# ma-compbio/Phylo-HMRF

Measured on AMD Instinct MI355X. Metric: EM-iterations/sec x nodes (bin-pairs), higher is better.
Workload: dtype f32

## Files before the change

### phylo_hmrf_amd/csrc/api.hip

```cpp

#include <algorithm>
#include <cmath>
#include <cstdio>
#include <cstdlib>
#include <cstring>
#include <limits>
#include <numeric>
#include <random>
#include <thread>

#include "common.h"

namespace phmrf {

static thread_local std::string g_error;

void set_error(const std::string& msg) { g_error = msg; }

int fail(int status, const std::string& msg) {
  g_error = msg;
  return status;
}

static hipEvent_t take_event(phmrf_block* b) {
// ... 454 lines not shown
  auto guard = [&](int s) {
    if (s != PHMRF_OK && st == PHMRF_OK) st = s;
  };
  if (hipGetDevice(&b->device) != hipSuccess) guard(fail(PHMRF_ERR_HIP, "hipGetDevice failed"));
  if (st == PHMRF_OK && hipStreamCreateWithFlags(&b->own_stream, hipStreamNonBlocking) != hipSuccess)
    guard(fail(PHMRF_ERR_HIP, "hipStreamCreate failed"));
  b->stream = b->own_stream;
  if (st == PHMRF_OK) guard(dev_alloc(&b->X, (size_t)n * S));
  if (st == PHMRF_OK) guard(dev_alloc(&b->logprob, (size_t)n * K));
  if (st == PHMRF_OK) guard(dev_alloc(&b->labels, (size_t)n));
  if (st == PHMRF_OK) guard(dev_alloc(&b->labels_tmp, (size_t)n));
  if (st == PHMRF_OK) guard(dev_alloc(&b->accum, (size_t)ACCUM_DOUBLES));
  if (st == PHMRF_OK) guard(dev_alloc(&b->counters, (size_t)N_COUNTERS));
  if (st == PHMRF_OK) guard(dev_alloc(&b->work_acc, (size_t)WORK_BANKS * WORK_SLOTS));
  if (st == PHMRF_OK && hipMemsetAsync(b->work_acc, 0, WORK_BANKS * WORK_SLOTS * sizeof(unsigned long long), b->own_stream) != hipSuccess)
    guard(fail(PHMRF_ERR_HIP, "hipMemset failed"));
  if (st == PHMRF_OK && hipHostMalloc(reinterpret_cast<void**>(&b->work_host), WORK_BANKS * WORK_SLOTS * sizeof(unsigned long long)) != hipSuccess)
    guard(fail(PHMRF_ERR_HIP, "hipHostMalloc failed"));
  if (st == PHMRF_OK) guard(dev_alloc(&b->emis_params, (size_t)K * (S + S * (S + 1) / 2 + 1)));
  if (st == PHMRF_OK && hipHostMalloc(reinterpret_cast<void**>(&b->accum_host), ACCUM_DOUBLES * sizeof(double)) != hipSuccess)
    guard(fail(PHMRF_ERR_HIP, "hipHostMalloc failed"));
  if (st == PHMRF_OK && hipHostMalloc(reinterpret_cast<void**>(&b->counters_host), N_COUNTERS * sizeof(unsigned long long)) != hipSuccess)
    guard(fail(PHMRF_ERR_HIP, "hipHostMalloc failed"));
  if (st == PHMRF_OK && (hipEventCreate(&b->ev0) != hipSuccess || hipEventCreate(&b->ev1) != hipSuccess))
    guard(fail(PHMRF_ERR_HIP, "hipEventCreate failed"));
  if (st == PHMRF_OK && hipMemsetAsync(b->labels, 0, (size_t)n, b->stream) != hipSuccess)
    guard(fail(PHMRF_ERR_HIP, "hipMemset failed"));
  if (st != PHMRF_OK) {
    std::string keep = g_error;
    phmrf_block_destroy(b);
    g_error = keep;
    return st;
  }
  *out = b;
  return PHMRF_OK;
}

int phmrf_block_destroy(phmrf_block_t b) {
  if (!b) return PHMRF_OK;
  if (b->stream) (void)hipStreamSynchronize(b->stream);
  coarse_children_destroy(b);
  if (b->c2f) {
    (void)phmrf_block_destroy(b->c2f);
    b->c2f = nullptr;
  }
  dev_free(b->X);
  dev_free(b->logprob);
  dev_free(b->labels);
  dev_free(b->labels_tmp);
  dev_free(b->labels_eval);
  dev_free(b->coarse_flag);
  dev_free(b->coarse_lab);
  if (b->coarse_lab_host) (void)hipHostFree(b->coarse_lab_host);
  b->coarse_lab_host = nullptr;
  dev_free(b->sgain);
  dev_free(b->mf_rev);
  dev_free(b->mf_theta);
  dev_free(b->mf_cap);
  dev_free(b->mf_tcap);
  dev_free(b->mf_exc);
  dev_free(b->mf_hgt);
  dev_free(b->mf_flags);
  if (b->mf_flags_host) (void)hipHostFree(b->mf_flags_host);
  b->mf_flags_host = nullptr;
  for (int s = 0; s < 4; ++s) dev_free(b->saved[s]);
  dev_free(b->nbr);
  dev_free(b->wgt);
  dev_free(b->colour_nodes);
  for (auto& f : b->families) free_family(f);
  dev_free(b->comp);
  dev_free(b->comp_tab);
  dev_free(b->comp_tab64);
  dev_free(b->post_partial);
  dev_free(b->comp_best);
  dev_free(b->comp_gain);
  dev_free(b->cc_seen);
  dev_free(b->cc_stale);
  dev_free(b->stamp);
  dev_free(b->memo);
  dev_free(b->chain_memo);
  dev_free(b->fwd_w);
  if (b->uT_raw) {
    dev_free(b->uT_raw);
    b->uT = nullptr;
  }
  dev_free(b->emis_params);
  dev_free(b->posteriors);
  dev_free(b->summary);
  dev_free(b->anc);
  for (int r = 0; r < 2; ++r) {
    dev_free(b->pin_save[r]);
    dev_free(b->pin_label[r]);
  }
  dev_free(b->xfer);
  if (b->xfer_host) (void)hipHostFree(b->xfer_host);
  if (b->ss) {
    delete b->ss;
    b->ss = nullptr;
  }
  dev_free(b->accum);
  dev_free(b->counters);
  dev_free(b->work_acc);
  if (b->work_host) (void)hipHostFree(b->work_host);
  if (b->accum_host) (void)hipHostFree(b->accum_host);
  if (b->counters_host) (void)hipHostFree(b->counters_host);
  for (auto& p : b->pending) {
    (void)hipEventDestroy(p.a);
    (void)hipEventDestroy(p.b);
  }
  for (auto e : b->free_events) (void)hipEventDestroy(e);
  if (b->cur_start) (void)hipEventDestroy(b->cur_start);
  if (b->ev0) (void)hipEventDestroy(b->ev0);
  if (b->ev1) (void)hipEventDestroy(b->ev1);
  if (b->own_stream) (void)hipStreamDestroy(b->own_stream);
  delete b;
  return PHMRF_OK;
}

int phmrf_block_set_stream(phmrf_block_t b, void* hip_stream) {
  PHMRF_CHECK(b, PHMRF_ERR_INVALID, "block is NULL");
  PHMRF_HIP(hipStreamSynchronize(b->stream));
  b->stream = hip_stream ? reinterpret_cast<hipStream_t>(hip_stream) : b->own_stream;
  for (int lv = 0; lv < N_COARSE_CHILDREN; ++lv)
    if (b->coarse[lv]) b->coarse[lv]->stream = b->stream;
  return PHMRF_OK;
}

int phmrf_block_sync(phmrf_block_t b) {
  PHMRF_CHECK(b, PHMRF_ERR_INVALID, "block is NULL");
  PHMRF_HIP(hipStreamSynchronize(b->stream));
  return PHMRF_OK;
}

int phmrf_block_set_observations(phmrf_block_t b, const double* X) {
  PHMRF_CHECK(b && X, PHMRF_ERR_INVALID, "NULL argument");
  const size_t cnt = (size_t)b->n * b->S;
  std::vector<float> tmp(cnt);
  for (size_t i = 0; i < cnt; ++i) tmp[i] = (float)X[i];
  PHMRF_TRY(upload(b->X, tmp.data(), cnt * sizeof(float), b->stream));
  b->has_X = true;
  return PHMRF_OK;
}

int phmrf_block_set_observations_dev(phmrf_block_t b, const float* X_dev) {
  PHMRF_CHECK(b && X_dev, PHMRF_ERR_INVALID, "NULL argument");
  PHMRF_HIP(hipMemcpyAsync(b->X, X_dev, (size_t)b->n * b->S * sizeof(float), hipMemcpyDeviceToDevice, b->stream));
  b->has_X = true;
  return PHMRF_OK;
}

int phmrf_block_set_graph(phmrf_block_t b, int64_t E, const int64_t* edges, const double* w) {
  PHMRF_CHECK(b, PHMRF_ERR_INVALID, "block is NULL");
  PHMRF_CHECK(E >= 0 && (E == 0 || (edges && w)), PHMRF_ERR_INVALID, "edges / w is NULL");
  const int64_t n = b->n;
  std::vector<int32_t> deg(n, 0);
  for (int64_t e = 0; e < E; ++e) {
    const int64_t a = edges[2 * e], c = edges[2 * e + 1];
    PHMRF_CHECK(a >= 0 && a < n && c >= 0 && c < n, PHMRF_ERR_INVALID, "edge endpoint out of range");
    PHMRF_CHECK(a != c, PHMRF_ERR_INVALID, "self loop in edge list");
    PHMRF_CHECK(w[e] >= 0.0 && std::isfinite(w[e]), PHMRF_ERR_INVALID, "edge weights must be finite and >= 0");
    ++deg[a];
    ++deg[c];
  }
  int maxdeg = 0;
  for (int64_t i = 0; i < n; ++i) maxdeg = std::max(maxdeg, deg[i]);
  PHMRF_CHECK(maxdeg <= 64, PHMRF_ERR_UNSUPPORTED, "node degree > 64 is not supported");
  const int D = std::max(4, (maxdeg + 3) / 4 * 4);
  std::vector<int32_t> nbr((size_t)n * D, -1);
  std::vector<float> wgt((size_t)n * D, 0.f);
  std::fill(deg.begin(), deg.end(), 0);
  for (int64_t e = 0; e < E; ++e) {
    const int64_t a = edges[2 * e], c = edges[2 * e + 1];
    nbr[(size_t)a * D + deg[a]] = (int32_t)c;
    wgt[(size_t)a * D + deg[a]++] = (float)w[e];
    nbr[(size_t)c * D + deg[c]] = (int32_t)a;
    wgt[(size_t)c * D + deg[c]++] = (float)w[e];
  }
  for (int64_t i = 0; i < n; ++i) {
    int32_t* c = &nbr[(size_t)i * D];
    float* ww = &wgt[(size_t)i * D];
    for (int x = 1; x < deg[i]; ++x) {
      const int32_t cv = c[x];
      const float wv = ww[x];
      int y = x - 1;
      while (y >= 0 && c[y] > cv) {
        c[y + 1] = c[y];
        ww[y + 1] = ww[y];
        --y;
      }
      c[y + 1] = cv;
      ww[y + 1] = wv;
    }
    for (int x = 1; x < deg[i]; ++x)
      PHMRF_CHECK(c[x] != c[x - 1], PHMRF_ERR_INVALID, "duplicate edge in edge list");
  }
  std::vector<int32_t> colour(n, -1);
  int ncol = 0;
  {
    std::vector<int> mark(66, -1);
    for (int64_t i = 0; i < n; ++i) {
      const int32_t* c = &nbr[(size_t)i * D];
      for (int x = 0; x < deg[i]; ++x)
        if (colour[c[x]] >= 0) mark[colour[c[x]]] = (int)(i & 0x7fffffff);
      int col = 0;
      while (mark[col] == (int)(i & 0x7fffffff)) ++col;
      colour[i] = col;
      ncol = std::max(ncol, col + 1);
    }
  }
  std::vector<int64_t> cptr(ncol + 1, 0);
  for (int64_t i = 0; i < n; ++i) ++cptr[colour[i] + 1];
  for (int c = 0; c < ncol; ++c) cptr[c + 1] += cptr[c];
  std::vector<int32_t> cnodes(n);
  {
    std::vector<int64_t> pos(cptr.begin(), cptr.end() - 1);
    for (int64_t i = 0; i < n; ++i) cnodes[pos[colour[i]]++] = (int32_t)i;
  }
  dev_free(b->nbr);
  dev_free(b->wgt);
  dev_free(b->colour_nodes);
  PHMRF_TRY(dev_alloc(&b->nbr, (size_t)n * D));
  PHMRF_TRY(dev_alloc(&b->wgt, (size_t)n * D));
  PHMRF_TRY(dev_alloc(&b->colour_nodes, (size_t)n));
  PHMRF_TRY(upload(b->nbr, nbr.data(), nbr.size() * sizeof(int32_t), b->stream));
  PHMRF_TRY(upload(b->wgt, wgt.data(), wgt.size() * sizeof(float), b->stream));
  PHMRF_TRY(upload(b->colour_nodes, cnodes.data(), cnodes.size() * sizeof(int32_t), b->stream));
  b->D = D;
  b->E = E;
  b->n_colours = ncol;
  b->colour_ptr = cptr;
  b->has_graph = true;
  b->has_grid = false;
  for (auto& f : b->families) free_family(f);
  b->families.clear();
  dev_free(b->mf_rev);
  dev_free(b->mf_theta);
  dev_free(b->mf_cap);
  dev_free(b->mf_tcap);
  dev_free(b->mf_exc);
  dev_free(b->mf_hgt);
  return PHMRF_OK;
}

int phmrf_block_set_grid(phmrf_block_t b, int H, int W, int diagonal, int num_neighbor) {
  PHMRF_CHECK(b, PHMRF_ERR_INVALID, "block is NULL");
  PHMRF_CHECK(b->has_graph, PHMRF_ERR_STATE, "set_graph must precede set_grid");
  PHMRF_CHECK(H >= 1 && W >= 1, PHMRF_ERR_INVALID, "H, W must be >= 1");
  PHMRF_CHECK(num_neighbor == 8 || num_neighbor == 4, PHMRF_ERR_INVALID, "num_neighbor must be 8 or 4");
  PHMRF_CHECK(!diagonal || H <= W, PHMRF_ERR_INVALID, "a diagonal block is the first H <= W rows of a W x W upper triangle");
  Geometry g(H, W, diagonal);
  PHMRF_CHECK(g.count() == b->n, PHMRF_ERR_INVALID, "H, W, diagonal do not match the node count");
  const int64_t n = b->n;
  const int D = b->D;
  std::vector<int32_t> nbr((size_t)n * D);
  std::vector<float> wgt((size_t)n * D);
  PHMRF_TRY(download(nbr.data(), b->nbr, nbr.size() * sizeof(int32_t), b->stream));
  PHMRF_TRY(download(wgt.data(), b->wgt, wgt.size() * sizeof(float), b->stream));
  std::vector<int32_t> ci(n), cj(n);
  for (int64_t v = 0; v < n; ++v) {
    int i, j;
    g.coords(v, &i, &j);
    ci[v] = i;
    cj[v] = j;
  }
  int64_t present = 0, expected = 0;
  for (int64_t v = 0; v < n; ++v) {
    for (int x = 0; x < D; ++x) {
      const int32_t u = nbr[(size_t)v * D + x];
      if (u < 0) continue;
      const int di = std::abs(ci[u] - ci[v]), dj = std::abs(cj[u] - cj[v]);
      PHMRF_CHECK(di <= 1 && dj <= 1 && (di + dj) > 0, PHMRF_ERR_INVALID, "edge list joins nodes that are not grid neighbours");
      PHMRF_CHECK(num_neighbor == 8 || (di + dj) == 1, PHMRF_ERR_INVALID, "diagonal edge in a 4-neighbour block");
      ++present;
    }
    for (int di = -1; di <= 1; ++di)
      for (int dj = -1; dj <= 1; ++dj) {
        if ((di == 0 && dj == 0) || (num_neighbor == 4 && di != 0 && dj != 0)) continue;
        const int ni = ci[v] + di, nj = cj[v] + dj;
        if (ni < 0 || ni >= H || nj < 0 || nj >= W || (diagonal && ni > nj)) continue;
        ++expected;
      }
  }
  PHMRF_TRY(setup_grid_tables(b, g, num_neighbor));
  b->grid_complete = present == expected;
  return PHMRF_OK;
}

int phmrf_block_build_grid_graph(phmrf_block_t b, int H, int W, int diagonal, int num_neighbor, double beta1) {
  PHMRF_CHECK(b, PHMRF_ERR_INVALID, "block is NULL");
  PHMRF_CHECK(b->has_X, PHMRF_ERR_STATE, "observations must be set before the graph is built from them");
  PHMRF_CHECK(H >= 1 && W >= 1, PHMRF_ERR_INVALID, "H, W must be >= 1");
  PHMRF_CHECK(num_neighbor == 8 || num_neighbor == 4, PHMRF_ERR_INVALID, "num_neighbor must be 8 or 4");
  PHMRF_CHECK(!diagonal || H <= W, PHMRF_ERR_INVALID, "a diagonal block is the first H <= W rows of a W x W upper triangle");
  PHMRF_CHECK(beta1 >= 0.0 && std::isfinite(beta1), PHMRF_ERR_INVALID, "beta1 must be finite and >= 0");
  Geometry g(H, W, diagonal);
  PHMRF_CHECK(g.count() == b->n, PHMRF_ERR_INVALID, "H, W, diagonal do not match the node count");
  dev_free(b->nbr);
  dev_free(b->wgt);
  PHMRF_TRY(dev_alloc(&b->nbr, (size_t)b->n * 8));
  PHMRF_TRY(dev_alloc(&b->wgt, (size_t)b->n * 8));
  b->D = 8;
  PHMRF_TRY(launch_grid_graph(b, H, W, diagonal, num_neighbor, beta1));
  if (!b->colour_nodes) PHMRF_TRY(dev_alloc(&b->colour_nodes, (size_t)b->n));
  b->has_graph = true;
  b->E = 0;
  PHMRF_TRY(setup_grid_tables(b, g, num_neighbor));
  b->grid_complete = true;
  return PHMRF_OK;
}

int phmrf_block_get_adjacency(phmrf_block_t b, int* D, int32_t* nbr_out, float* wgt_out) {
  PHMRF_CHECK(b && D, PHMRF_ERR_INVALID, "NULL argument");
  PHMRF_CHECK(b->has_graph, PHMRF_ERR_STATE, "graph not set");
  *D = b->D;
  if (nbr_out) PHMRF_TRY(download(nbr_out, b->nbr, (size_t)b->n * b->D * sizeof(int32_t), b->stream));
  if (wgt_out) PHMRF_TRY(download(wgt_out, b->wgt, (size_t)b->n * b->D * sizeof(float), b->stream));
  return PHMRF_OK;
}

int phmrf_block_set_labels(phmrf_block_t b, const int32_t* labels) {
  PHMRF_CHECK(b && labels, PHMRF_ERR_INVALID, "NULL argument");
  std::vector<uint8_t> tmp(b->n);
  for (int64_t i = 0; i < b->n; ++i) {
    PHMRF_CHECK(labels[i] >= 0 && labels[i] < b->K, PHMRF_ERR_INVALID, "label out of range [0,K)");
    tmp[i] = (uint8_t)labels[i];
  }
  PHMRF_TRY(upload(b->labels, tmp.data(), (size_t)b->n, b->stream));
  b->has_labels = true;
  b->labels_are_slot = 0;
  return PHMRF_OK;
}

static int fetch_labels(phmrf_block_t b, const uint8_t* src, int32_t* labels) {
  std::vector<uint8_t> tmp(b->n);
  PHMRF_TRY(download(tmp.data(), src, (size_t)b->n, b->stream));
  for (int64_t i = 0; i < b->n; ++i) labels[i] = tmp[i];
  return PHMRF_OK;
}

int phmrf_block_get_labels(phmrf_block_t b, int32_t* labels) {
  PHMRF_CHECK(b && labels, PHMRF_ERR_INVALID, "NULL argument");
  return fetch_labels(b, b->labels, labels);
}

int phmrf_block_save_labels(phmrf_block_t b, int slot) {
  PHMRF_CHECK(b, PHMRF_ERR_INVALID, "block is NULL");
  PHMRF_CHECK(slot >= 0 && slot < 4, PHMRF_ERR_INVALID, "slot must be in [0,4)");
  if (!b->saved[slot]) PHMRF_TRY(dev_alloc(&b->saved[slot], (size_t)b->n));
  PHMRF_HIP(hipMemcpyAsync(b->saved[slot], b->labels, (size_t)b->n, hipMemcpyDeviceToDevice, b->stream));
  b->labels_are_slot |= 1 << slot;
  return PHMRF_OK;
}

int phmrf_block_restore_labels(phmrf_block_t b, int slot) {
  PHMRF_CHECK(b, PHMRF_ERR_INVALID, "block is NULL");
  PHMRF_CHECK(slot >= 0 && slot < 4 && b->saved[slot], PHMRF_ERR_STATE, "label slot is empty");
  PHMRF_HIP(hipMemcpyAsync(b->labels, b->saved[slot], (size_t)b->n, hipMemcpyDeviceToDevice, b->stream));
  b->has_labels = true;
  b->labels_are_slot = 1 << slot;
  return PHMRF_OK;
}

int phmrf_block_get_saved_labels(phmrf_block_t b, int slot, int32_t* labels) {
  PHMRF_CHECK(b && labels, PHMRF_ERR_INVALID, "NULL argument");
  PHMRF_CHECK(slot >= 0 && slot < 4 && b->saved[slot], PHMRF_ERR_STATE, "label slot is empty");
  return fetch_labels(b, b->saved[slot], labels);
}

int phmrf_emission_pack_size(int S, int K, int64_t* n_floats) {
  PHMRF_CHECK(n_floats && S >= 1 && S <= 16 && K >= 1, PHMRF_ERR_INVALID, "bad S/K");
  *n_floats = (int64_t)K * (S + S * (S + 1) / 2 + 1);
  return PHMRF_OK;
}

int phmrf_emission_pack(int S, int K, const double* means, const double* covars, float* packed) {
  PHMRF_CHECK(means && covars && packed, PHMRF_ERR_INVALID, "NULL argument");
  PHMRF_CHECK(S >= 1 && S <= 16 && K >= 1, PHMRF_ERR_INVALID, "bad S/K");
  const int PS = S + S * (S + 1) / 2 + 1;
  std::vector<double> L(S * S), Li(S * S);
  for (int k = 0; k < K; ++k) {
    const double* cv = covars + (size_t)k * S * S;
    bool ok = false;
    for (int attempt = 0; attempt < 2 && !ok; ++attempt) {
      const double jitter = attempt ? 1e-7 : 0.0;
      ok = true;
      std::fill(L.begin(), L.end(), 0.0);
      for (int i = 0; i < S && ok; ++i)
        for (int j = 0; j <= i; ++j) {
          double s = cv[i * S + j] + (i == j ? jitter : 0.0);
          for (int t = 0; t < j; ++t) s -= L[i * S + t] * L[j * S + t];
          if (i == j) {
            if (!(s > 0.0) || !std::isfinite(s)) { ok = false; break; }
            L[i * S + i] = std::sqrt(s);
          } else {
            L[i * S + j] = s / L[j * S + j];
          }
        }
    }
    if (!ok) return fail(PHMRF_ERR_NOT_PD, "'covars' must be symmetric, positive-definite (state " + std::to_string(k) + ")");
    std::fill(Li.begin(), Li.end(), 0.0);
    double logdet = 0.0;
    for (int i = 0; i < S; ++i) logdet += 2.0 * std::log(L[i * S + i]);
    for (int c = 0; c < S; ++c)
      for (int i = c; i < S; ++i) {
        double s = (i == c) ? 1.0 : 0.0;
        for (int t = c; t < i; ++t) s -= L[i * S + t] * Li[t * S + c];
        Li[i * S + c] = s / L[i * S + i];
      }
    float* p = packed + (size_t)k * PS;
    for (int s = 0; s < S; ++s) p[s] = (float)means[(size_t)k * S + s];
    int idx = S;
    for (int i = 0; i < S; ++i)
      for (int c = 0; c <= i; ++c) p[idx++] = (float)Li[i * S + c];
    p[idx] = (float)(-0.5 * (S * std::log(2.0 * M_PI) + logdet));
  }
  return PHMRF_OK;
}

int phmrf_emission_dev(const float* X_dev, int64_t n, int S, int K, const float* packed_dev, float* logprob_dev,
                       void* hip_stream) {
  PHMRF_CHECK(X_dev && packed_dev && logprob_dev, PHMRF_ERR_INVALID, "NULL argument");
  PHMRF_CHECK(n > 0 && K >= 1 && K <= 64, PHMRF_ERR_INVALID, "bad n/K");
  return launch_emission(X_dev, n, S, K, packed_dev, logprob_dev, nullptr, reinterpret_cast<hipStream_t>(hip_stream));
}

int phmrf_emission(phmrf_block_t b, const double* means, const double* covars) {
  PHMRF_CHECK(b && means && covars, PHMRF_ERR_INVALID, "NULL argument");
  PHMRF_CHECK(b->has_X, PHMRF_ERR_STATE, "observations not set");
  const int PS = b->S + b->S * (b->S + 1) / 2 + 1;
  std::vector<float> packed((size_t)b->K * PS);
  PHMRF_TRY(phmrf_emission_pack(b->S, b->K, means, covars, packed.data()));
  PHMRF_TRY(upload(b->emis_params, packed.data(), packed.size() * sizeof(float), b->stream));
  tic(b, KC_EMISSION);
  PHMRF_TRY(launch_emission(b->X, b->n, b->S, b->K, b->emis_params, b->logprob, b->uT, b->stream));
  toc(b, KC_EMISSION, 1);
  b->has_logprob = true;
  b->uT_valid = b->uT != nullptr;
  b->pin_saved = false;
  b->pin_rows[0] = b->pin_rows[1] = 0;
  return PHMRF_OK;
}

int phmrf_block_get_logprob(phmrf_block_t b, double* logprob) {
  PHMRF_CHECK(b && logprob, PHMRF_ERR_INVALID, "NULL argument");
  PHMRF_CHECK(b->has_logprob, PHMRF_ERR_STATE, "logprob not computed");
  const size_t cnt = (size_t)b->n * b->K;
  std::vector<float> tmp(cnt);
  PHMRF_TRY(download(tmp.data(), b->logprob, cnt * sizeof(float), b->stream));
  for (size_t i = 0; i < cnt; ++i) logprob[i] = tmp[i];
  return PHMRF_OK;
}

int phmrf_block_set_logprob(phmrf_block_t b, const double* logprob) {
  PHMRF_CHECK(b && logprob, PHMRF_ERR_INVALID, "NULL argument");
  const size_t cnt = (size_t)b->n * b->K;
  std::vector<float> tmp(cnt);
  for (size_t i = 0; i < cnt; ++i) tmp[i] = (float)logprob[i];
  PHMRF_TRY(upload(b->logprob, tmp.data(), cnt * sizeof(float), b->stream));
  b->has_logprob = true;
  b->uT_valid = false;
  b->pin_saved = false;
  b->pin_rows[0] = b->pin_rows[1] = 0;
  return PHMRF_OK;
}

static int read_counter(phmrf_block_t b, int64_t* v) {
  PHMRF_HIP(hipMemcpyAsync(b->counters_host + COUNTER_DEFAULT, b->counters + COUNTER_DEFAULT, sizeof(unsigned long long), hipMemcpyDeviceToHost, b->stream));
  PHMRF_HIP(hipStreamSynchronize(b->stream));
  if (v) *v = (int64_t)b->counters_host[COUNTER_DEFAULT];
  return PHMRF_OK;
}

static int zero_counter(phmrf_block_t b) {
  PHMRF_HIP(hipMemsetAsync(b->counters, 0, N_COUNTERS * sizeof(unsigned long long), b->stream));
  b->counter_slot = COUNTER_DEFAULT;
  return PHMRF_OK;
}

int phmrf_mrf_energy(phmrf_block_t b, double beta, double* e_total, double* e_unary, double* e_pair) {
  PHMRF_TRY(check_solvable(b));
  double eu, ep;
  PHMRF_TRY(energy_now(b, beta, &eu, &ep));
  if (e_total) *e_total = eu + ep;
  if (e_unary) *e_unary = eu;
  if (e_pair) *e_pair = ep;
  return PHMRF_OK;
}

int phmrf_block_warm_start(phmrf_block_t b, double beta, int slot, int choose, double* e_current, double* e_saved, int* took_saved) {
  PHMRF_TRY(check_solvable(b));
  PHMRF_CHECK(slot >= 0 && slot < 4 && b->saved[slot], PHMRF_ERR_STATE, "label slot is empty");
  if (took_saved) *took_saved = 1;
  const bool report = e_current || e_saved || took_saved;
  if (!b->has_labels || ((b->labels_are_slot >> slot) & 1)) {
    if (choose && !b->has_labels) PHMRF_TRY(phmrf_block_restore_labels(b, slot));
    if (e_current) *e_current = std::numeric_limits<double>::infinity();
    if (e_saved) *e_saved = 0.0;
    return PHMRF_OK;
  }
  double* const extra = b->accum + (ACCUM_DOUBLES - 4);
  if (choose && !report && b->n >= (1 << 16) && energy_diff_available(b)) {
    PHMRF_TRY(zero_accum(b, 4, 2));
    PHMRF_TRY(zero_accum(b, ACCUM_DOUBLES - 4, 2));
    tic(b, KC_ENERGY);
    PHMRF_TRY(launch_energy_diff(b, b->saved[slot]));
    PHMRF_TRY(launch_choose_labels(b, b->saved[slot], b->accum + 4, extra, beta));
    toc(b, KC_ENERGY, 2);
    b->labels_are_slot = 0;
    return PHMRF_OK;
  }
  PHMRF_TRY(zero_accum(b, 4, 2));
  PHMRF_TRY(zero_accum(b, ACCUM_DOUBLES - 4, 2));
  tic(b, KC_ENERGY);
  PHMRF_TRY(launch_energy(b, (float)beta));
  std::swap(b->labels, b->saved[slot]);
  const int st = launch_energy(b, (float)beta, extra);
  std::swap(b->labels, b->saved[slot]);
  PHMRF_TRY(st);
  if (choose) PHMRF_TRY(launch_choose_labels(b, b->saved[slot], b->accum + 4, extra, beta));
  toc(b, KC_ENERGY, choose ? 3 : 2);
  if (choose) b->labels_are_slot = 0;
  if (!report) return PHMRF_OK;
  PHMRF_HIP(hipMemcpyAsync(b->accum_host + 4, b->accum + 4, 2 * sizeof(double), hipMemcpyDeviceToHost, b->stream));
  PHMRF_HIP(hipMemcpyAsync(b->accum_host + 6, extra, 2 * sizeof(double), hipMemcpyDeviceToHost, b->stream));
  PHMRF_HIP(hipStreamSynchronize(b->stream));
  double ec[2], es[2];
  energy_sums(b, b->accum_host + 4, &ec[0], &ec[1]);
  energy_sums(b, b->accum_host + 6, &es[0], &es[1]);
  const double cur = ec[0] + beta * ec[1], sav = es[0] + beta * es[1];
  if (e_current) *e_current = cur;
  if (e_saved) *e_saved = sav;
  if (took_saved) *took_saved = !(cur < sav) ? 1 : 0;
  return PHMRF_OK;
}

int phmrf_block_energy_diff(phmrf_block_t b, double beta, int slot, double* out) {
  PHMRF_TRY(check_solvable(b));
  PHMRF_CHECK(out, PHMRF_ERR_INVALID, "NULL argument");
  PHMRF_CHECK(slot >= 0 && slot < 4 && b->saved[slot], PHMRF_ERR_STATE, "label slot is empty");
  PHMRF_CHECK(b->has_labels, PHMRF_ERR_STATE, "labels not set");
  PHMRF_CHECK(b->has_grid && b->fwd_w && b->H > 0 && b->W > 0, PHMRF_ERR_UNSUPPORTED,
              "the energy difference from the differing nodes needs a grid block (phmrf_block_set_grid / build_grid_graph)");
  PHMRF_CHECK(energy_diff_available(b), PHMRF_ERR_STATE,
              "the unary planes are not current (a strip pass or a solve builds them after phmrf_block_set_logprob)");
  PHMRF_TRY(zero_accum(b, 4, 2));
  tic(b, KC_ENERGY);
  PHMRF_TRY(launch_energy_diff(b, b->saved[slot]));
  toc(b, KC_ENERGY, 1);
  PHMRF_HIP(hipMemcpyAsync(b->accum_host + 4, b->accum + 4, 2 * sizeof(double), hipMemcpyDeviceToHost, b->stream));
  PHMRF_HIP(hipStreamSynchronize(b->stream));
  energy_sums(b, b->accum_host + 4, &out[0], &out[1]);
  out[1] = beta * out[1];
  return PHMRF_OK;
}

int phmrf_mrf_icm_sweep(phmrf_block_t b, double beta, int64_t* changed) {
  PHMRF_TRY(check_solvable(b));
  b->labels_are_slot = 0;
  PHMRF_TRY(zero_counter(b));
  PHMRF_TRY(icm_sweep_nocount(b, (float)beta));
  return read_counter(b, changed);
}

static int ensure_chain_families(phmrf_block* b) {
  if (!b->has_grid && b->families.empty() && b->nbr && b->n >= 2) PHMRF_TRY(setup_path_families(b));
  return PHMRF_OK;
}

int phmrf_mrf_chain_sweep(phmrf_block_t b, double beta, int family, int64_t* changed) {
  PHMRF_TRY(check_solvable(b));
  b->labels_are_slot = 0;
  PHMRF_TRY(ensure_chain_families(b));
  PHMRF_CHECK(family >= 0 && family < (int)b->families.size(), PHMRF_ERR_INVALID, "no such chain family");
  PHMRF_TRY(zero_counter(b));
  PHMRF_TRY(chain_sweep_nocount(b, (float)beta, family, 0));
  PHMRF_TRY(chain_sweep_nocount(b, (float)beta, family, 1));
  return read_counter(b, changed);
}

int phmrf_block_chain_family_info(phmrf_block_t b, int* n_families, int* n_colours) {
  PHMRF_CHECK(b && n_families, PHMRF_ERR_INVALID, "NULL argument");
  PHMRF_CHECK(b->has_graph, PHMRF_ERR_STATE, "graph not set");
  PHMRF_CHECK(!b->ss, PHMRF_ERR_STATE, "a solve is in progress");
  PHMRF_TRY(ensure_chain_families(b));
  *n_families = (int)b->families.size();
  if (n_colours)
    for (int f = 0; f < MAX_CHAIN_FAMILIES; ++f) n_colours[f] = f < (int)b->families.size() ? b->families[f].n_colours : 0;
  return PHMRF_OK;
}

int phmrf_block_get_chain_segments(phmrf_block_t b, int family, int phase, int colour, int64_t* n_segments, int64_t* n_nodes,
                                   int32_t* seg_start, int32_t* seg_len, int32_t* nodes) {
  PHMRF_CHECK(b && n_segments && n_nodes, PHMRF_ERR_INVALID, "NULL argument");
  PHMRF_CHECK(b->has_graph, PHMRF_ERR_STATE, "graph not set");
  PHMRF_CHECK(!b->ss, PHMRF_ERR_STATE, "a solve is in progress");
  PHMRF_TRY(ensure_chain_families(b));
  PHMRF_CHECK(family >= 0 && family < (int)b->families.size(), PHMRF_ERR_INVALID, "no such chain family");
  const ChainFamily& f = b->families[family];
  PHMRF_CHECK(phase == 0 || phase == 1, PHMRF_ERR_INVALID, "phase must be 0 or 1");
  PHMRF_CHECK(colour >= 0 && colour < f.n_colours, PHMRF_ERR_INVALID, "no such colour in this chain family");
  const int nseg = f.nseg[phase][colour];
  *n_segments = nseg;
  *n_nodes = f.n_nodes;
  if (seg_start && nseg > 0) PHMRF_TRY(download(seg_start, f.seg_start[phase][colour], (size_t)nseg * sizeof(int32_t), b->stream));
  if (seg_len && nseg > 0) PHMRF_TRY(download(seg_len, f.seg_len[phase][colour], (size_t)nseg * sizeof(int32_t), b->stream));
  if (nodes && f.n_nodes > 0) PHMRF_TRY(download(nodes, f.nodes, (size_t)f.n_nodes * sizeof(int32_t), b->stream));
  return PHMRF_OK;
}

int phmrf_block_prepare_components(phmrf_block_t b) {
  PHMRF_CHECK(b, PHMRF_ERR_INVALID, "block is NULL");
  PHMRF_CHECK(!b->ss, PHMRF_ERR_STATE, "a solve is in progress");
  if (!b->has_labels || !b->has_graph) return PHMRF_OK;
  return launch_component_prepare(b);
}

int phmrf_mrf_component_pass(phmrf_block_t b, double beta, int64_t* changed) {
  PHMRF_TRY(check_solvable(b));
  b->labels_are_slot = 0;
  PHMRF_TRY(zero_counter(b));
  tic(b, KC_COMPONENT);
  PHMRF_TRY(launch_component_pass(b, (float)beta));
  toc(b, KC_COMPONENT, 1);
  return read_counter(b, changed);
}

int phmrf_mrf_graph_expansion(phmrf_block_t b, double beta, int alpha, int64_t* changed) {
  PHMRF_TRY(check_solvable(b));
  PHMRF_CHECK(b->has_labels, PHMRF_ERR_STATE, "labels not set");
  PHMRF_CHECK(alpha >= 0 && alpha < b->K, PHMRF_ERR_INVALID, "alpha must be in [0, K)");
  PHMRF_CHECK(b->n >= 2, PHMRF_ERR_INVALID, "the graph has fewer than two nodes");
  b->labels_are_slot = 0;
  PHMRF_TRY(zero_counter(b));
  PHMRF_TRY(launch_graph_expansion(b, (float)beta, alpha));
  return read_counter(b, changed);
}


int phmrf_mrf_strip_pass(phmrf_block_t b, double beta, int orient, int shift_r, int shift_c, int alpha, int64_t* changed) {
  PHMRF_TRY(check_solvable(b));
  b->labels_are_slot = 0;
  PHMRF_CHECK(b->has_grid, PHMRF_ERR_STATE, "strip moves need phmrf_block_set_grid");
  PHMRF_CHECK(b->num_neighbor == 8 || b->num_neighbor == 4, PHMRF_ERR_STATE, "bad grid");
  PHMRF_CHECK(orient == 0 || orient == 1, PHMRF_ERR_INVALID, "orient must be 0 or 1");
  PHMRF_CHECK(shift_r >= 0 && shift_r <= 5 && shift_c >= 0 && shift_c <= 63, PHMRF_ERR_INVALID, "shift out of range");
  PHMRF_CHECK(alpha < b->K, PHMRF_ERR_INVALID, "alpha must be < K");
  PHMRF_TRY(zero_counter(b));
  PHMRF_TRY(strip_pass_nocount(b, (float)beta, orient, shift_r, shift_c, alpha));
  PHMRF_TRY(work_fetch_async(b));
  PHMRF_TRY(read_counter(b, changed));
  work_fold(b);
  return PHMRF_OK;
}

int phmrf_mrf_strip_multi_pass(phmrf_block_t b, double beta, int orient, int shift_r, int shift_c, uint64_t label_mask,
                               int64_t* changed) {
  PHMRF_TRY(check_solvable(b));
  b->labels_are_slot = 0;
  PHMRF_CHECK(b->has_grid, PHMRF_ERR_STATE, "strip moves need phmrf_block_set_grid");
  PHMRF_CHECK(b->num_neighbor == 8 || b->num_neighbor == 4, PHMRF_ERR_STATE, "bad grid");
  PHMRF_CHECK(orient == 0 || orient == 1, PHMRF_ERR_INVALID, "orient must be 0 or 1");
  PHMRF_CHECK(shift_r >= 0 && shift_r <= 5 && shift_c >= 0 && shift_c <= 63, PHMRF_ERR_INVALID, "shift out of range");
  PHMRF_CHECK(b->K >= 64 || (label_mask >> b->K) == 0, PHMRF_ERR_INVALID, "label_mask names a label >= K");
  PHMRF_HIP(hipMemsetAsync(b->counters, 0, N_COUNTERS * sizeof(unsigned long long), b->stream));
  if (!b->uT_valid) PHMRF_TRY(launch_unary_planes(b));
  tic(b, KC_STRIP);
  PHMRF_TRY(launch_strip_multi(b, (float)beta, orient, shift_r, shift_c, label_mask, -1));
  b->work[4] += 1;
  toc(b, KC_STRIP, 1);
  PHMRF_TRY(work_fetch_async(b));
  PHMRF_HIP(hipMemcpyAsync(b->counters_host, b->counters, N_COUNTERS * sizeof(unsigned long long), hipMemcpyDeviceToHost, b->stream));
  PHMRF_HIP(hipStreamSynchronize(b->stream));
  work_fold(b);
  int64_t ch = 0;
  for (int a = 0; a < b->K; ++a) ch += (int64_t)b->counters_host[COUNTER_EXPANSION + a];
  if (changed) *changed = ch;
  return PHMRF_OK;
}

int phmrf_mrf_coarse_pass(phmrf_block_t b, double beta, int scale, int offset, int alpha, int shift_r, int shift_c,
                          int64_t* changed) {
  PHMRF_TRY(check_solvable(b));
  b->labels_are_slot = 0;
  PHMRF_CHECK(b->has_grid, PHMRF_ERR_STATE, "coarse moves need phmrf_block_set_grid");
  PHMRF_CHECK(scale == 2 || scale == 4 || scale == 8, PHMRF_ERR_INVALID, "scale must be 2, 4 or 8");
  PHMRF_CHECK(offset >= 0 && offset < scale, PHMRF_ERR_INVALID, "offset must be in [0, scale)");
  PHMRF_CHECK(alpha >= 0 && alpha < b->K, PHMRF_ERR_INVALID, "alpha must be in [0, K)");
  PHMRF_CHECK(shift_r >= 0 && shift_r <= 5 && shift_c >= 0 && shift_c <= 63, PHMRF_ERR_INVALID, "shift out of range");
  PHMRF_TRY(zero_counter(b));
  PHMRF_TRY(coarse_sweep_nocount(b, (float)beta, scale == 2 ? 0 : (scale == 4 ? 1 : 2), offset, shift_r, shift_c, alpha, alpha + 1));
  return read_counter(b, changed);
}

int phmrf_block_coarse_problem(phmrf_block_t b, double beta, int scale, int offset, int alpha, int64_t* nc, float* D_out,
                               float* lam_out) {
  PHMRF_TRY(check_solvable(b));
  PHMRF_CHECK(nc, PHMRF_ERR_INVALID, "nc is NULL");
  PHMRF_CHECK(b->has_grid, PHMRF_ERR_STATE, "coarse moves need phmrf_block_set_grid");
  PHMRF_CHECK(scale == 2 || scale == 4 || scale == 8, PHMRF_ERR_INVALID, "scale must be 2, 4 or 8");
  PHMRF_CHECK(offset >= 0 && offset < scale, PHMRF_ERR_INVALID, "offset must be in [0, scale)");
  PHMRF_CHECK(alpha >= 0 && alpha < b->K, PHMRF_ERR_INVALID, "alpha must be in [0, K)");
  *nc = coarse_nodes(b, scale, offset);
  if (!D_out && !lam_out) return PHMRF_OK;
  phmrf_block* c = nullptr;
  PHMRF_TRY(coarse_child(b, 4 * (scale == 2 ? 0 : (scale == 4 ? 1 : 2)), &c));
  if (!b->uT_valid) PHMRF_TRY(launch_unary_planes(b));
  PHMRF_TRY(launch_coarsen(b, c, scale, offset, alpha, (float)beta));
  if (D_out) PHMRF_TRY(download(D_out, c->uT + *nc, (size_t)*nc * sizeof(float), b->stream));
  if (lam_out) PHMRF_TRY(download(lam_out, c->fwd_w, (size_t)*nc * sizeof(float4), b->stream));
  return PHMRF_OK;
}

int phmrf_block_coarse_problems(phmrf_block_t b, double beta, int scale, int offset, const int* alphas, int nl, int64_t* nc,
                                float* D_out, float* lam_out) {
  PHMRF_TRY(check_solvable(b));
  PHMRF_CHECK(nc && alphas, PHMRF_ERR_INVALID, "NULL argument");
  PHMRF_CHECK(b->has_grid, PHMRF_ERR_STATE, "coarse moves need phmrf_block_set_grid");
  PHMRF_CHECK(scale == 2 || scale == 4 || scale == 8, PHMRF_ERR_INVALID, "scale must be 2, 4 or 8");
  PHMRF_CHECK(offset >= 0 && offset < scale, PHMRF_ERR_INVALID, "offset must be in [0, scale)");
  PHMRF_CHECK(nl >= 1 && nl <= 4, PHMRF_ERR_INVALID, "nl must be in [1, 4]");
  for (int q = 0; q < nl; ++q) PHMRF_CHECK(alphas[q] >= 0 && alphas[q] < b->K, PHMRF_ERR_INVALID, "alpha must be in [0, K)");
  *nc = coarse_nodes(b, scale, offset);
  if (!D_out && !lam_out) return PHMRF_OK;
  const int level = scale == 2 ? 0 : (scale == 4 ? 1 : 2);
  phmrf_block* ch[4] = {nullptr, nullptr, nullptr, nullptr};
  for (int q = 0; q < nl; ++q) PHMRF_TRY(coarse_child(b, 4 * level + q, &ch[q]));
  if (!b->uT_valid) PHMRF_TRY(launch_unary_planes(b));
  PHMRF_TRY(launch_coarsen_batch(b, ch, alphas, nl, scale, offset, (float)beta, nullptr, -1, false));
  for (int q = 0; q < nl; ++q) {
    if (D_out) PHMRF_TRY(download(D_out + (size_t)q * *nc, ch[q]->uT + *nc, (size_t)*nc * sizeof(float), b->stream));
    if (lam_out) PHMRF_TRY(download(lam_out + (size_t)q * *nc * 4, ch[q]->fwd_w, (size_t)*nc * sizeof(float4), b->stream));
  }
  return PHMRF_OK;
}

int phmrf_mrf_coarse_sweep(phmrf_block_t b, double beta, int scale, int offset, uint64_t label_mask, int shift_r, int shift_c,
                           int stamps, int64_t* changed, int64_t* changed_label) {
  PHMRF_TRY(check_solvable(b));
  PHMRF_CHECK(!b->ss, PHMRF_ERR_STATE, "a solve is in progress");
  PHMRF_CHECK(b->has_grid, PHMRF_ERR_STATE, "coarse moves need phmrf_block_set_grid");
  PHMRF_CHECK(b->has_labels, PHMRF_ERR_STATE, "labels not set");
  PHMRF_CHECK(scale == 2 || scale == 4 || scale == 8, PHMRF_ERR_INVALID, "scale must be 2, 4 or 8");
  PHMRF_CHECK(offset >= 0 && offset < scale, PHMRF_ERR_INVALID, "offset must be in [0, scale)");
  PHMRF_CHECK(shift_r >= 0 && shift_r <= 5 && shift_c >= 0 && shift_c <= 63, PHMRF_ERR_INVALID, "shift out of range");
  PHMRF_CHECK(b->K >= 64 || (label_mask >> b->K) == 0, PHMRF_ERR_INVALID, "label_mask names a label >= K");
  b->labels_are_slot = 0;
  const int level = scale == 2 ? 0 : (scale == 4 ? 1 : 2);
  const size_t lab_bytes = (size_t)N_COARSE * MAX_LABELS * sizeof(unsigned long long);
  if (!b->coarse_lab) {
    PHMRF_TRY(dev_alloc(&b->coarse_lab, (size_t)N_COARSE * MAX_LABELS));
    PHMRF_HIP(hipHostMalloc(reinterpret_cast<void**>(&b->coarse_lab_host), lab_bytes));
  }
  PHMRF_HIP(hipMemsetAsync(b->coarse_lab, 0, lab_bytes, b->stream));
  PHMRF_TRY(zero_counter(b));
  if (stamps) {
    if (!b->stamp) PHMRF_TRY(dev_alloc(&b->stamp, (size_t)b->n));
    PHMRF_HIP(hipMemsetAsync(b->stamp, 0, (size_t)b->n * sizeof(uint16_t), b->stream));
    b->tick = 1;
  }
  int st = coarse_sweep_nocount(b, (float)beta, level, offset, shift_r, shift_c, 0, b->K, label_mask);
  if (st == PHMRF_OK && hipMemcpyAsync(b->coarse_lab_host, b->coarse_lab, lab_bytes, hipMemcpyDeviceToHost, b->stream) != hipSuccess)
    st = PHMRF_ERR_HIP;
  const int st_read = read_counter(b, changed);
  if (stamps) solve_scope_exit(b);
  PHMRF_TRY(st);
  PHMRF_TRY(st_read);
  if (changed_label)
    for (int a = 0; a < b->K; ++a) changed_label[a] = (int64_t)b->coarse_lab_host[(size_t)level * MAX_LABELS + a];
  return PHMRF_OK;
}

static int c2f_ready(phmrf_block_t b) {
  PHMRF_CHECK(b, PHMRF_ERR_INVALID, "block is NULL");
  PHMRF_CHECK(!b->ss, PHMRF_ERR_STATE, "a solve is in progress");
  PHMRF_CHECK(c2f_applies(b), PHMRF_ERR_STATE,
              "the coarse-to-fine start needs a complete 8-neighbour grid block (no row tile) with n >= 1024 and H, W >= 8");
  return c2f_child(b);
}

int phmrf_block_c2f_problem(phmrf_block_t b, int* Hc, int* Wc, int64_t* nc, int32_t* nbr_out, float* wgt_out, float* logprob_out) {
  PHMRF_TRY(check_solvable(b));
  PHMRF_CHECK(Hc && Wc && nc, PHMRF_ERR_INVALID, "NULL argument");
  PHMRF_TRY(c2f_ready(b));
  phmrf_block* c = b->c2f;
  *Hc = b->c2f_Hc;
  *Wc = b->c2f_Wc;
  *nc = c->n;
  if (nbr_out) PHMRF_TRY(download(nbr_out, c->nbr, (size_t)c->n * 8 * sizeof(int32_t), b->stream));
  if (wgt_out) PHMRF_TRY(download(wgt_out, c->wgt, (size_t)c->n * 8 * sizeof(float), b->stream));
  if (logprob_out) {
    PHMRF_TRY(launch_c2f_logprob(b, c, b->c2f_Wc, C2F_SCALE));
    c->has_logprob = true;
    c->uT_valid = false;
    PHMRF_TRY(download(logprob_out, c->logprob, (size_t)c->n * b->K * sizeof(float), b->stream));
  }
  return PHMRF_OK;
}

int phmrf_block_c2f_prolong(phmrf_block_t b, const int32_t* labels_c, int64_t nc) {
  PHMRF_CHECK(b && labels_c, PHMRF_ERR_INVALID, "NULL argument");
  PHMRF_TRY(c2f_ready(b));
  phmrf_block* c = b->c2f;
  PHMRF_CHECK(nc == c->n, PHMRF_ERR_INVALID, "nc is not the number of 4 x 4 super-cells");
  std::vector<uint8_t> tmp((size_t)nc);
  for (int64_t i = 0; i < nc; ++i) {
    PHMRF_CHECK(labels_c[i] >= 0 && labels_c[i] < b->K, PHMRF_ERR_INVALID, "label out of range [0,K)");
    tmp[(size_t)i] = (uint8_t)labels_c[i];
  }
  PHMRF_TRY(upload(c->labels, tmp.data(), (size_t)nc, b->stream));
  c->has_labels = true;
  c->labels_are_slot = 0;
  PHMRF_TRY(launch_c2f_prolong(b, c, b->c2f_Wc, C2F_SCALE));
  PHMRF_HIP(hipStreamSynchronize(b->stream));
  b->has_labels = true;
  b->labels_are_slot = 0;
  return PHMRF_OK;
}


int phmrf_block_set_tile(phmrf_block_t b, int top, int bottom, int64_t sched_n) {
  PHMRF_CHECK(b, PHMRF_ERR_INVALID, "block is NULL");
  PHMRF_CHECK(b->has_grid, PHMRF_ERR_STATE, "row tiles need the grid geometry (phmrf_block_set_grid / build_grid_graph)");
  PHMRF_CHECK(!b->ss, PHMRF_ERR_STATE, "a solve is in progress");
  top = top ? 1 : 0;
  bottom = bottom ? 1 : 0;
  PHMRF_CHECK(b->H >= 2 * (top + bottom) + 2, PHMRF_ERR_INVALID, "a tile needs two rows per cut and two more");
  for (int r = 0; r < 2; ++r) {
    dev_free(b->pin_save[r]);
    dev_free(b->pin_label[r]);
    b->pin_first[r] = b->pin_count[r] = b->pin_split[r] = 0;
    b->pin_rows[r] = 0;
  }
  b->pin_saved = false;
  b->tile_top = top;
  b->tile_bot = bottom;
  b->sched_n = sched_n > 0 ? sched_n : 0;
  if (!top && !bottom) {
    b->own0 = 0;
    b->own1 = -1;
    b->own_r0 = 0;
    b->own_r1 = -1;
    return PHMRF_OK;
  }
  b->own_r0 = top ? 1 : 0;
  b->own_r1 = b->H - (bottom ? 1 : 0);
  b->own0 = row_first(b, b->own_r0);
  b->own1 = row_first(b, b->own_r1);
  if (top) {
    b->pin_first[0] = 0;
    b->pin_count[0] = row_first(b, 2);
    b->pin_split[0] = row_first(b, 1);
  }
  if (bottom) {
    b->pin_first[1] = row_first(b, b->H - 2);
    b->pin_count[1] = b->n - b->pin_first[1];
    b->pin_split[1] = row_first(b, b->H - 1) - b->pin_first[1];
  }
  int64_t cap = 0;
  for (int r = 0; r < 2; ++r)
    if (b->pin_count[r] > 0) {
      PHMRF_TRY(dev_alloc(&b->pin_save[r], (size_t)b->pin_count[r] * b->K));
      PHMRF_TRY(dev_alloc(&b->pin_label[r], (size_t)b->pin_count[r]));
      cap += b->pin_count[r];
    }
  if (cap > b->xfer_cap) {
    dev_free(b->xfer);
    if (b->xfer_host) (void)hipHostFree(b->xfer_host);
    b->xfer_host = nullptr;
    PHMRF_TRY(dev_alloc(&b->xfer, (size_t)cap));
    PHMRF_HIP(hipHostMalloc(reinterpret_cast<void**>(&b->xfer_host), (size_t)2 * cap));
    b->xfer_cap = cap;
  }
  return PHMRF_OK;
}

static void pin_range(const phmrf_block* b, int region, int rows, int64_t* first, int64_t* count) {
  *first = b->pin_first[region];
  *count = 0;
  if (rows <= 0 || b->pin_count[region] == 0) return;
  if (rows >= 2) {
    *count = b->pin_count[region];
  } else if (region == 0) {
    *count = b->pin_split[0];
  } else {
    *first = b->pin_first[1] + b->pin_split[1];
    *count = b->pin_count[1] - b->pin_split[1];
  }
}

int phmrf_block_tile_pins(phmrf_block_t b, int n_top, int n_bottom) {
  PHMRF_CHECK(b, PHMRF_ERR_INVALID, "block is NULL");
  PHMRF_CHECK(is_tile(b), PHMRF_ERR_STATE, "the block is not a tile (phmrf_block_set_tile)");
  PHMRF_CHECK(b->has_logprob, PHMRF_ERR_STATE, "logprob not set");
  PHMRF_CHECK(n_top >= 0 && n_top <= 2 && n_bottom >= 0 && n_bottom <= 2, PHMRF_ERR_INVALID, "0, 1 or 2 rows per cut");
  const int want[2] = {b->tile_top ? n_top : 0, b->tile_bot ? n_bottom : 0};
  if (b->tick) ++b->tick;
  for (int r = 0; r < 2; ++r) {
    if (b->pin_count[r] == 0) continue;
    int64_t pf, pc, wf, wc;
    pin_range(b, r, want[r], &pf, &pc);
    pin_range(b, r, b->pin_saved ? b->pin_rows[r] : 0, &wf, &wc);
    PHMRF_TRY(launch_tile_pins(b, r, b->pin_first[r], b->pin_count[r], pf, pc, wf, wc, !b->pin_saved));
    b->pin_rows[r] = want[r];
  }
  b->pin_saved = true;
  return PHMRF_OK;
}

int phmrf_block_tile_get_boundary(phmrf_block_t b, uint8_t* top_out, uint8_t* bottom_out) {
  PHMRF_CHECK(b, PHMRF_ERR_INVALID, "block is NULL");
  PHMRF_CHECK(is_tile(b), PHMRF_ERR_STATE, "the block is not a tile (phmrf_block_set_tile)");
  const bool have = b->boundary_queued && b->ss && b->ss->collected;
  if (!have) {
    PHMRF_TRY(tile_queue_boundary(b));
    PHMRF_HIP(hipStreamSynchronize(b->stream));
  }
  b->boundary_queued = false;
  int64_t off = 0;
  if (b->tile_top) {
    const int64_t tc = row_first(b, 2) - row_first(b, 1);
    if (top_out) std::memcpy(top_out, b->xfer_host, (size_t)tc);
    off = tc;
  }
  if (b->tile_bot && bottom_out) {
    const int64_t bc = row_first(b, b->H - 1) - row_first(b, b->H - 2);
    std::memcpy(bottom_out, b->xfer_host + off, (size_t)bc);
  }
  return PHMRF_OK;
}

int phmrf_block_tile_put_halo(phmrf_block_t b, const uint8_t* top_in, const uint8_t* bottom_in) {
  PHMRF_CHECK(b, PHMRF_ERR_INVALID, "block is NULL");
  PHMRF_CHECK(is_tile(b), PHMRF_ERR_STATE, "the block is not a tile (phmrf_block_set_tile)");
  if (b->tick) ++b->tick;
  b->labels_are_slot = 0;
  uint8_t* const in_host = b->xfer_host + b->xfer_cap;
  int64_t off = 0;
  if (top_in && b->tile_top) {
    const int64_t c = row_first(b, 1);
    for (int64_t q = 0; q < c; ++q) PHMRF_CHECK(top_in[q] < b->K, PHMRF_ERR_INVALID, "label out of range [0,K)");
    std::memcpy(in_host, top_in, (size_t)c);
    PHMRF_HIP(hipMemcpyAsync(b->xfer, in_host, (size_t)c, hipMemcpyHostToDevice, b->stream));
    PHMRF_TRY(launch_put_labels(b, 0, c, b->xfer));
    off = c;
  }
  if (bottom_in && b->tile_bot) {
    const int64_t f = row_first(b, b->H - 1), c = b->n - f;
    for (int64_t q = 0; q < c; ++q) PHMRF_CHECK(bottom_in[q] < b->K, PHMRF_ERR_INVALID, "label out of range [0,K)");
    std::memcpy(in_host + off, bottom_in, (size_t)c);
    PHMRF_HIP(hipMemcpyAsync(b->xfer + off, in_host + off, (size_t)c, hipMemcpyHostToDevice, b->stream));
    PHMRF_TRY(launch_put_labels(b, f, c, b->xfer + off));
  }
  if (!b->ss) PHMRF_HIP(hipStreamSynchronize(b->stream));
  return PHMRF_OK;
}

static int posterior_launch(phmrf_block_t b, double beta, int estimate_type, bool write_post) {
  PHMRF_TRY(check_solvable(b));
  PHMRF_CHECK(b->has_X, PHMRF_ERR_STATE, "observations not set");
  const int ns = n_stats(b);
  PHMRF_CHECK(8 + ns <= ACCUM_DOUBLES, PHMRF_ERR_UNSUPPORTED, "K*(1+S+S*S) too large");
  if (write_post && !b->posteriors) PHMRF_TRY(dev_alloc(&b->posteriors, (size_t)b->n * b->K));
  if (b->deterministic && !b->post_partial) {
    const int64_t rows = std::min<int64_t>(POST_PARTIAL_ROWS, std::max<int64_t>(1, (b->n + POST_DET_TB - 1) / POST_DET_TB));
    PHMRF_TRY(dev_alloc(&b->post_partial, (size_t)rows * (b->K * (1 + b->S + b->S * (b->S + 1) / 2) + 4)));
  }
  PHMRF_TRY(zero_accum(b, 0, 4));
  PHMRF_TRY(zero_accum(b, 8, ns));
  tic(b, KC_POSTERIOR);
  PHMRF_TRY(launch_posterior_stats(b, (float)beta, estimate_type, write_post));
  toc(b, KC_POSTERIOR, 1);
  return PHMRF_OK;
}

int phmrf_posterior_stats(phmrf_block_t b, double beta, int estimate_type, double* stats_out, double* costs_out,
                          double* posteriors_out) {
  PHMRF_CHECK(b && stats_out && costs_out, PHMRF_ERR_INVALID, "NULL argument");
  PHMRF_TRY(posterior_launch(b, beta, estimate_type, posteriors_out != nullptr));
  const int ns = n_stats(b);
  PHMRF_HIP(hipMemcpyAsync(b->accum_host, b->accum, (8 + ns) * sizeof(double), hipMemcpyDeviceToHost, b->stream));
  PHMRF_HIP(hipStreamSynchronize(b->stream));
  std::memcpy(costs_out, b->accum_host, 4 * sizeof(double));
  std::memcpy(stats_out, b->accum_host + 8, ns * sizeof(double));
  if (posteriors_out) {
    const size_t cnt = (size_t)b->n * b->K;
    std::vector<float> tmp(cnt);
    PHMRF_TRY(download(tmp.data(), b->posteriors, cnt * sizeof(float), b->stream));
    for (size_t i = 0; i < cnt; ++i) posteriors_out[i] = tmp[i];
  }
  return PHMRF_OK;
}

int phmrf_posterior_stats_dev(phmrf_block_t b, double beta, int estimate_type, double* out_dev) {
  PHMRF_CHECK(b && out_dev, PHMRF_ERR_INVALID, "NULL argument");
  PHMRF_TRY(posterior_launch(b, beta, estimate_type, false));
  const int ns = n_stats(b);
  PHMRF_HIP(hipMemcpyAsync(out_dev, b->accum + 8, ns * sizeof(double), hipMemcpyDeviceToDevice, b->stream));
  PHMRF_HIP(hipMemcpyAsync(out_dev + ns, b->accum, 4 * sizeof(double), hipMemcpyDeviceToDevice, b->stream));
  return PHMRF_OK;
}

int phmrf_posterior_summary(phmrf_block_t b, double beta, int estimate_type, float* conf, uint8_t* top, float* entropy_or_null) {
  PHMRF_CHECK(b && conf && top, PHMRF_ERR_INVALID, "NULL argument");
  PHMRF_TRY(check_solvable(b));
  PHMRF_CHECK(b->has_labels, PHMRF_ERR_STATE, "labels not set (phmrf_block_set_labels or a solve)");
  const int64_t n_first = b->own1 >= 0 ? b->own0 : 0, n_last = b->own1 >= 0 ? b->own1 : b->n;
  const int64_t m = n_last - n_first;
  if (m <= 0) return PHMRF_OK;
  if (!b->summary) PHMRF_TRY(dev_alloc(&b->summary, (size_t)b->n * (2 * sizeof(float) + 1)));
  float* d_conf = reinterpret_cast<float*>(b->summary);
  float* d_ent = d_conf + b->n;
  uint8_t* d_top = reinterpret_cast<uint8_t*>(d_ent + b->n);
  tic(b, KC_POSTERIOR);
  PHMRF_TRY(launch_posterior_summary(b, (float)beta, estimate_type, d_conf, d_top, entropy_or_null ? d_ent : nullptr));
  toc(b, KC_POSTERIOR, 1);
  PHMRF_HIP(hipMemcpyAsync(conf, d_conf, (size_t)m * sizeof(float), hipMemcpyDeviceToHost, b->stream));
  PHMRF_HIP(hipMemcpyAsync(top, d_top, (size_t)m, hipMemcpyDeviceToHost, b->stream));
  if (entropy_or_null)
    PHMRF_HIP(hipMemcpyAsync(entropy_or_null, d_ent, (size_t)m * sizeof(float), hipMemcpyDeviceToHost, b->stream));
  PHMRF_HIP(hipStreamSynchronize(b->stream));
  return PHMRF_OK;
}

int phmrf_ancestral(phmrf_block_t b, double beta, int estimate_type, int weighting, int A, const double* affine,
                    const double* cond_var, float* mean_out, float* sd_out_or_null) {
  PHMRF_CHECK(b && affine && cond_var && mean_out, PHMRF_ERR_INVALID, "NULL argument");
  PHMRF_CHECK(weighting == 0 || weighting == 1, PHMRF_ERR_INVALID, "weighting must be 0 (posterior) or 1 (called)");
  PHMRF_CHECK(A >= 1 && A <= 16, PHMRF_ERR_UNSUPPORTED, "ancestral: A must be in [1,16]");
  PHMRF_CHECK(b->S <= 8, PHMRF_ERR_UNSUPPORTED, "ancestral: S must be in [1,8]");
  const int K = b->K, S = b->S, TS = S + 2;
  std::vector<float> tab((size_t)K * A * TS);
  for (int ka = 0; ka < K * A; ++ka) {
    for (int s = 0; s <= S; ++s) tab[(size_t)ka * TS + s] = (float)affine[(size_t)ka * (S + 1) + s];
    tab[(size_t)ka * TS + S + 1] = (float)cond_var[ka];
    PHMRF_CHECK(cond_var[ka] >= 0.0, PHMRF_ERR_INVALID, "cond_var must be finite and >= 0");
  }
  for (float v : tab) PHMRF_CHECK(std::isfinite(v), PHMRF_ERR_INVALID, "the tables must be finite (as float32)");
  PHMRF_CHECK(b->has_X, PHMRF_ERR_STATE, "observations not set");
  PHMRF_CHECK(b->has_labels, PHMRF_ERR_STATE, "labels not set (phmrf_block_set_labels or a solve)");
  if (weighting == 0) PHMRF_TRY(check_solvable(b));
  const int64_t n_first = b->own1 >= 0 ? b->own0 : 0, n_last = b->own1 >= 0 ? b->own1 : b->n;
  const int64_t m = n_last - n_first;
  if (m <= 0) return PHMRF_OK;
  const size_t need = tab.size() + (size_t)2 * A * m;
  if (b->anc_floats < need) {
    dev_free(b->anc);
    b->anc_floats = 0;
    PHMRF_TRY(dev_alloc(&b->anc, need));
    b->anc_floats = need;
  }
  float* d_mean = b->anc + tab.size();
  float* d_sd = d_mean + (size_t)A * m;
  PHMRF_TRY(upload(b->anc, tab.data(), tab.size() * sizeof(float), b->stream));
  tic(b, KC_POSTERIOR);
  PHMRF_TRY(launch_ancestral(b, (float)beta, estimate_type, weighting, A, b->anc, d_mean, sd_out_or_null ? d_sd : nullptr));
  toc(b, KC_POSTERIOR, 1);
  PHMRF_HIP(hipMemcpyAsync(mean_out, d_mean, (size_t)A * m * sizeof(float), hipMemcpyDeviceToHost, b->stream));
  if (sd_out_or_null)
    PHMRF_HIP(hipMemcpyAsync(sd_out_or_null, d_sd, (size_t)A * m * sizeof(float), hipMemcpyDeviceToHost, b->stream));
  PHMRF_HIP(hipStreamSynchronize(b->stream));
  return PHMRF_OK;
}

int phmrf_kmeans_step(phmrf_block_t b, const double* centers, int write_labels, double* out) {
  PHMRF_CHECK(b && centers && out, PHMRF_ERR_INVALID, "NULL argument");
  PHMRF_CHECK(b->has_X, PHMRF_ERR_STATE, "observations not set");
  const int K = b->K, S = b->S, NP = K * S + K + 1;
  PHMRF_CHECK(8 + NP <= ACCUM_DOUBLES, PHMRF_ERR_UNSUPPORTED, "K*S too large");
  std::vector<float> c((size_t)K * S);
  for (int i = 0; i < K * S; ++i) {
    PHMRF_CHECK(std::isfinite(centers[i]), PHMRF_ERR_INVALID, "centres must be finite");
    c[i] = (float)centers[i];
  }
  PHMRF_TRY(upload(b->emis_params, c.data(), c.size() * sizeof(float), b->stream));
  PHMRF_TRY(zero_accum(b, 8, NP));
  PHMRF_TRY(launch_kmeans_step(b, b->emis_params, write_labels != 0, b->accum + 8));
  PHMRF_HIP(hipMemcpyAsync(b->accum_host + 8, b->accum + 8, NP * sizeof(double), hipMemcpyDeviceToHost, b->stream));
  PHMRF_HIP(hipStreamSynchronize(b->stream));
  std::memcpy(out, b->accum_host + 8, NP * sizeof(double));
  if (write_labels) {
    b->has_labels = true;
    b->labels_are_slot = 0;
  }
  return PHMRF_OK;
}

int phmrf_kmeans_moments(phmrf_block_t b, const double* centers, int write_labels, double* out) {
  PHMRF_CHECK(b && centers && out, PHMRF_ERR_INVALID, "NULL argument");
  PHMRF_CHECK(b->has_X, PHMRF_ERR_STATE, "observations not set");
  const int K = b->K, S = b->S, NP = K * S + K + 1 + K * S * S;
  PHMRF_CHECK(S <= 8, PHMRF_ERR_UNSUPPORTED, "second moments: S must be in [1,8]");
  PHMRF_CHECK(8 + NP <= ACCUM_DOUBLES, PHMRF_ERR_UNSUPPORTED, "K*S*S too large");
  std::vector<float> c((size_t)K * S);
  for (int i = 0; i < K * S; ++i) {
    PHMRF_CHECK(std::isfinite(centers[i]), PHMRF_ERR_INVALID, "centres must be finite");
    c[i] = (float)centers[i];
  }
  PHMRF_TRY(upload(b->emis_params, c.data(), c.size() * sizeof(float), b->stream));
  PHMRF_TRY(zero_accum(b, 8, NP));
  PHMRF_TRY(launch_kmeans_step(b, b->emis_params, write_labels != 0, b->accum + 8, true));
  PHMRF_HIP(hipMemcpyAsync(b->accum_host + 8, b->accum + 8, NP * sizeof(double), hipMemcpyDeviceToHost, b->stream));
  PHMRF_HIP(hipStreamSynchronize(b->stream));
  std::memcpy(out, b->accum_host + 8, NP * sizeof(double));
  if (write_labels) {
    b->has_labels = true;
    b->labels_are_slot = 0;
  }
  return PHMRF_OK;
}

int phmrf_block_enable_timing(phmrf_block_t b, int enable) {
  PHMRF_CHECK(b, PHMRF_ERR_INVALID, "block is NULL");
  b->timing = enable != 0;
  return PHMRF_OK;
}

int phmrf_block_set_timing_classes(phmrf_block_t b, uint32_t class_mask) {
  PHMRF_CHECK(b, PHMRF_ERR_INVALID, "block is NULL");
  b->timing_mask = class_mask;
  return PHMRF_OK;
}

static int get_timing(phmrf_block_t b, bool first, int capacity, double* ms, int64_t* launches) {
  PHMRF_CHECK(b, PHMRF_ERR_INVALID, "block is NULL");
  PHMRF_CHECK(capacity >= 0, PHMRF_ERR_INVALID, "capacity < 0");
  resolve_timing(b);
  for (int i = 0; i < PHMRF_NUM_KERNEL_CLASSES && i < capacity; ++i) {
    if (ms) ms[i] = first ? b->ms_first[i] : b->ms[i];
    if (launches) launches[i] = first ? b->launches_first[i] : b->launches[i];
  }
  return PHMRF_OK;
}
int phmrf_block_get_timing(phmrf_block_t b, int capacity, double* ms, int64_t* launches) { return get_timing(b, false, capacity, ms, launches); }
int phmrf_block_get_timing_first(phmrf_block_t b, int capacity, double* ms, int64_t* launches) { return get_timing(b, true, capacity, ms, launches); }

int phmrf_block_reset_timing(phmrf_block_t b) {
  PHMRF_CHECK(b, PHMRF_ERR_INVALID, "block is NULL");
  resolve_timing(b);
  for (int i = 0; i < PHMRF_NUM_KERNEL_CLASSES; ++i) {
    b->ms[i] = b->ms_first[i] = 0;
    b->launches[i] = b->launches_first[i] = 0;
  }
  for (int q = 0; q < N_WORK; ++q) b->work[q] = b->work_first[q] = 0;
  PHMRF_HIP(hipMemsetAsync(b->work_acc, 0, WORK_BANKS * WORK_SLOTS * sizeof(unsigned long long), b->stream));
  b->intervals.clear();
  return PHMRF_OK;
}

int phmrf_time_base_reset(void) {
  int dev = 0;
  PHMRF_HIP(hipGetDevice(&dev));
  PHMRF_CHECK(dev >= 0 && dev < 64, PHMRF_ERR_UNSUPPORTED, "device index >= 64");
  if (!g_time_base[dev]) PHMRF_HIP(hipEventCreate(&g_time_base[dev]));
  PHMRF_HIP(hipDeviceSynchronize());
  PHMRF_HIP(hipEventRecord(g_time_base[dev], nullptr));
  PHMRF_HIP(hipEventSynchronize(g_time_base[dev]));
  return PHMRF_OK;
}

int phmrf_block_get_work(phmrf_block_t b, int64_t* out) {
  PHMRF_CHECK(b && out, PHMRF_ERR_INVALID, "NULL argument");
  for (int q = 0; q < 8; ++q) out[q] = b->work[q];
  return PHMRF_OK;
}

int phmrf_block_get_work_first(phmrf_block_t b, int64_t* out) {
  PHMRF_CHECK(b && out, PHMRF_ERR_INVALID, "NULL argument");
  for (int q = 0; q < 8; ++q) out[q] = b->work_first[q];
  return PHMRF_OK;
}

int phmrf_block_get_work_ex(phmrf_block_t b, int first_round_only, int capacity, int64_t* out) {
  PHMRF_CHECK(b && out, PHMRF_ERR_INVALID, "NULL argument");
  for (int q = 0; q < N_WORK && q < capacity; ++q) out[q] = first_round_only ? b->work_first[q] : b->work[q];
  return PHMRF_OK;
}

int phmrf_block_get_intervals(phmrf_block_t b, int kclass, double* out, int64_t capacity, int64_t* count) {
  PHMRF_CHECK(b && count, PHMRF_ERR_INVALID, "NULL argument");
  PHMRF_CHECK(kclass >= 0 && kclass < PHMRF_NUM_KERNEL_CLASSES, PHMRF_ERR_INVALID, "no such kernel class");
  resolve_timing(b);
  int64_t c = 0;
  for (const auto& iv : b->intervals)
    if (iv.kclass == kclass) {
      if (out && c < capacity) {
        out[2 * c] = iv.t0;
        out[2 * c + 1] = iv.t1;
      }
      ++c;
    }
  *count = c;
  return PHMRF_OK;
}

}
```

### phylo_hmrf_amd/csrc/common.h

```cpp
#pragma once

#include <hip/hip_runtime.h>
#include <stdint.h>

#include <array>
#include <string>
#include <vector>

#include "../../include/phmrf.h"

namespace phmrf {

void set_error(const std::string& msg);
int fail(int status, const std::string& msg);

#define PHMRF_HIP(expr)                                                                     \
  do {                                                                                      \
    hipError_t _e = (expr);                                                                 \
    if (_e != hipSuccess)                                                                   \
      return ::phmrf::fail(PHMRF_ERR_HIP, std::string(#expr) + ": " + hipGetErrorString(_e)); \
  } while (0)

#define PHMRF_CHECK(cond, status, msg) \
  do {                                 \
    if (!(cond)) return ::phmrf::fail((status), (msg)); \
  } while (0)

#define PHMRF_TRY(expr)          \
  do {                           \
    int _s = (expr);             \
    if (_s != PHMRF_OK) return _s; \
  } while (0)

enum KernelClass { KC_EMISSION = 0, KC_ICM = 1, KC_CHAIN = 2, KC_COMPONENT = 3, KC_ENERGY = 4, KC_POSTERIOR = 5, KC_STRIP = 6, KC_PROPOSE = 7, KC_COARSE = 8, KC_FUSION = 9 };

struct ChainFamily {
  int32_t* nodes = nullptr;
  int32_t* seg_start[2][3] = {};
  int32_t* seg_len[2][3] = {};
  uint16_t* memo[2][3] = {};
  int nseg[2][3] = {};
  int64_t n_nodes = 0;
  int n_chains = 0;
  int n_colours = 0;
  int max_len = 0;
};

constexpr int N_COUNTERS = PHMRF_NUM_COUNTERS;
constexpr int MAX_LABELS = 64;
constexpr int MAX_CHAIN_FAMILIES = 4;
constexpr int N_COARSE = 3;
constexpr int N_COARSE_CHILDREN = 4 * N_COARSE;
constexpr int COUNTER_DEFAULT = 0;
constexpr int COUNTER_EXPANSION = PHMRF_COUNTER_EXPANSION;
constexpr int COUNTER_CHAIN = PHMRF_COUNTER_CHAIN;
constexpr int COUNTER_ICM = PHMRF_COUNTER_ICM;
constexpr int COUNTER_COMPONENT = PHMRF_COUNTER_COMPONENT;
constexpr int COUNTER_FUSION = PHMRF_COUNTER_FUSION;
constexpr int COUNTER_COARSE = PHMRF_COUNTER_COARSE;
constexpr int COUNTER_TRACE = 100;
enum TraceCounter { TRACE_SEEN = 0, TRACE_PAST_MEMO = 1, TRACE_INTO_DP = 2, TRACE_DP_STEPS = 3, TRACE_MOVED = 4, N_TRACE = 5 };
constexpr int N_WORK = 11;
constexpr int WORK_INCREMENTAL = 10;
constexpr int COUNTER_ENERGY = 120;
static_assert(COUNTER_DEFAULT < COUNTER_EXPANSION && COUNTER_EXPANSION + MAX_LABELS <= COUNTER_CHAIN, "label slots run into the chain slots");
static_assert(COUNTER_CHAIN + MAX_CHAIN_FAMILIES <= COUNTER_ICM && COUNTER_ICM < COUNTER_COMPONENT && COUNTER_COMPONENT < COUNTER_FUSION,
              "chain / ICM / component slots overlap");
static_assert(COUNTER_FUSION + 2 <= COUNTER_COARSE && COUNTER_COARSE + N_COARSE <= COUNTER_TRACE, "fusion / coarse slots overlap");
static_assert(COUNTER_TRACE + N_TRACE <= COUNTER_ENERGY && COUNTER_ENERGY + 2 <= N_COUNTERS, "trace / energy slots do not fit the bank");

}

struct phmrf_solve_state;
struct phmrf_block {
  int64_t n = 0;
  int S = 0, K = 0;
  int device = 0;
  hipStream_t stream = nullptr;
  hipStream_t own_stream = nullptr;

  float* X = nullptr;
  float* logprob = nullptr;
  uint8_t* labels = nullptr;
  uint8_t* labels_tmp = nullptr;
  uint8_t* labels_eval = nullptr;
  int eval_tick = -1;
  float* sgain = nullptr;
  uint8_t* saved[4] = {nullptr, nullptr, nullptr, nullptr};
  int labels_are_slot = 0;
  bool has_X = false, has_logprob = false, has_labels = false, has_graph = false, has_grid = false;

  int D = 0;
  int64_t E = 0;
  int32_t* nbr = nullptr;
  float* wgt = nullptr;

  int n_colours = 0;
  int32_t* colour_nodes = nullptr;
  std::vector<int64_t> colour_ptr;

  int H = 0, W = 0, diagonal = 0, num_neighbor = 0;
  bool grid_complete = false;
  std::vector<phmrf::ChainFamily> families;

  int32_t* comp = nullptr;
  float* comp_tab = nullptr;
  long long* comp_tab64 = nullptr;
  bool deterministic = false;
  double* post_partial = nullptr;
  int32_t* comp_best = nullptr;
  float* comp_gain = nullptr;
  uint8_t* cc_seen = nullptr;
  int* cc_stale = nullptr;
  bool cc_prepared = false;
  float4* fwd_w = nullptr;
  float* uT = nullptr;
  float* uT_raw = nullptr;
  bool uT_valid = false;
  bool unary_pins = false;
  phmrf_block* coarse[phmrf::N_COARSE_CHILDREN] = {};
  unsigned int* coarse_flag = nullptr;
  phmrf_block* c2f = nullptr;
  int c2f_Hc = 0, c2f_Wc = 0;
  unsigned long long* coarse_lab = nullptr;
  unsigned long long* coarse_lab_host = nullptr;
  char* coarse_arena = nullptr;
  uint8_t* mf_rev = nullptr;
  float* mf_theta = nullptr;
  int32_t* mf_cap = nullptr;
  int32_t* mf_tcap = nullptr;
  long long* mf_exc = nullptr;
  int32_t* mf_hgt = nullptr;
  int32_t* mf_flags = nullptr;
  int32_t* mf_flags_host = nullptr;
  int prop_tick = -1;
  int geom_phase = 0;
  uint16_t* stamp = nullptr;
  uint16_t* memo = nullptr;
  uint16_t* chain_memo = nullptr;
  size_t chain_memo_count = 0;
  int64_t memo_strips = 0;
  int tick = 0;
  int counter_slot = 0;

  float* emis_params = nullptr;
  float* posteriors = nullptr;
  char* summary = nullptr;
  float* anc = nullptr;
  size_t anc_floats = 0;
  double* accum = nullptr;
  double* accum_host = nullptr;
  unsigned long long* counters = nullptr;
  unsigned long long* counters_host = nullptr;
  unsigned long long* work_acc = nullptr;
  unsigned long long* work_host = nullptr;

  bool timing = false;
  unsigned int timing_mask = ~0u;
  hipEvent_t ev0 = nullptr, ev1 = nullptr;
  struct Pending { int kclass; hipEvent_t a, b; bool first; };
  std::vector<Pending> pending;
  std::vector<hipEvent_t> free_events;
  hipEvent_t cur_start = nullptr;
  double ms[PHMRF_NUM_KERNEL_CLASSES] = {};
  int64_t launches[PHMRF_NUM_KERNEL_CLASSES] = {};
  double ms_first[PHMRF_NUM_KERNEL_CLASSES] = {};
  int64_t launches_first[PHMRF_NUM_KERNEL_CLASSES] = {};
  int64_t work_first[phmrf::N_WORK] = {};
  int64_t work[phmrf::N_WORK] = {};
  struct Interval { int kclass; float t0, t1; };
  std::vector<Interval> intervals;

  int tile_top = 0, tile_bot = 0;
  int64_t own0 = 0, own1 = -1;
  int own_r0 = 0, own_r1 = -1;
  int64_t sched_n = 0;
  float* pin_save[2] = {nullptr, nullptr};
  uint8_t* pin_label[2] = {nullptr, nullptr};
  uint8_t* xfer = nullptr;
  uint8_t* xfer_host = nullptr;
  int64_t xfer_cap = 0;
  bool boundary_queued = false;
  int64_t pin_first[2] = {0, 0}, pin_count[2] = {0, 0};
  int64_t pin_split[2] = {0, 0};
  int pin_rows[2] = {0, 0};
  bool pin_saved = false;
  struct phmrf_solve_state* ss = nullptr;
};

struct phmrf_solve_state {
  phmrf_solve_opts o;
  double beta = 0;
  float bf = 0;
  bool have_init_energy = false;
  double eu0 = 0, ep0 = 0;
  int64_t total = 0;
  int rounds = 0, converged = 0;
  bool chains = false, strips = false, expansions = false, coarse = false, graph_expansions = false;
  int n_fam = 0;
  int64_t tol = 0;
  int64_t sched_n = 0;
  std::vector<int> slots;
  int64_t last_changed = 0;
  int64_t coarse_changed[phmrf::N_COARSE] = {0, 0, 0};
  bool coarse_ran[phmrf::N_COARSE] = {false, false, false};
  unsigned long long coarse_lab_mask[phmrf::N_COARSE] = {~0ull, ~0ull, ~0ull};
  bool coarse_all[phmrf::N_COARSE] = {true, true, true};
  bool force_coarse = false;
  bool coarse_checked = false;
  std::array<char, phmrf::N_COUNTERS> active{}, ran{};
  std::array<long long, phmrf::N_COUNTERS> last_count{};
  bool all_active = true, verifying = false;
  double eu_carry = 0, ep_carry = 0;
  double e_prev = 0;
  int geom = 0;
  bool prev_moving = false;
  bool launched = false, collected = false, incremental = false, snapshot = false;
  int status = 0;
};

namespace phmrf {

#ifdef PHMRF_DEV
#define PHMRF_DEV_ENV(name) (getenv(name))
#else
#define PHMRF_DEV_ENV(name) (static_cast<const char*>(nullptr))
#endif
inline bool no_skip() {
  static const bool v = PHMRF_DEV_ENV("PHMRF_NO_SKIP") != nullptr;
  return v;
}
constexpr int C2F_SCALE = 4;
constexpr int UT_PAD = 64;
constexpr int WORK_SLOTS = 7;
constexpr int WORK_BANKS = 256;
constexpr int POST_PARTIAL_ROWS = 2048;
constexpr int POST_DET_TB = 64;
constexpr int ACCUM_DOUBLES = 8192;

void tic(phmrf_block* b, int kclass);
void toc(phmrf_block* b, int kclass, int n_launches);
void resolve_timing(phmrf_block* b);

template <typename T>
int dev_alloc(T** p, size_t count) {
  *p = nullptr;
  if (count == 0) count = 1;
  PHMRF_HIP(hipMalloc(reinterpret_cast<void**>(p), count * sizeof(T)));
  return PHMRF_OK;
}

template <typename T>
void dev_free(T*& p) {
  if (p) (void)hipFree(p);
  p = nullptr;
}

inline bool is_tile(const phmrf_block* b) { return b->tile_top || b->tile_bot; }

struct Geometry;
int setup_grid_tables(phmrf_block* b, const Geometry& g, int num_neighbor);
int setup_path_families(phmrf_block* b);
int zero_accum(phmrf_block* b, size_t first, size_t count);
int check_solvable(phmrf_block* b);
int energy_now(phmrf_block* b, double beta, double* eu, double* ep);
void energy_sums(const phmrf_block* b, const void* slots, double* eu, double* ep);
int work_fetch_async(phmrf_block* b);
void work_fold(phmrf_block* b, bool first_round = false);
int icm_sweep_nocount(phmrf_block* b, float beta);
int chain_sweep_nocount(phmrf_block* b, float beta, int family, int phase, bool timed = true);
int strip_pass_nocount(phmrf_block* b, float beta, int orient, int shift_r, int shift_c, int alpha, int geom = -1, bool timed = true);
int coarse_child(phmrf_block* b, int level_slot, phmrf_block** out);
void coarse_children_destroy(phmrf_block* b);
int coarse_sweep_nocount(phmrf_block* b, float beta, int level, int off, int shift_r, int shift_c, int alpha_lo, int alpha_hi,
                         unsigned long long label_mask = ~0ull);
int tile_queue_boundary(phmrf_block* b);
bool c2f_applies(const phmrf_block* b);
int c2f_child(phmrf_block* b);
void solve_scope_exit(phmrf_block* b);

inline int tile_threads(int K) { return K <= 40 ? 256 : 128; }
inline int padded_k(int K) { return (K % 2 == 0) ? K + 1 : K; }

int launch_emission(const float* X, int64_t n, int S, int K, const float* packed, float* logprob, float* uT, hipStream_t st);
int launch_argmax_labels(const phmrf_block* b);
int launch_icm_colour(const phmrf_block* b, float beta, int colour);
int launch_energy(const phmrf_block* b, float beta, double* accum_at = nullptr);
int launch_choose_labels(const phmrf_block* b, const uint8_t* saved, const double* acc_cur, const double* acc_sav, double beta);
bool energy_delta_available(const phmrf_block* b);
bool energy_diff_available(const phmrf_block* b);
int launch_energy_diff(const phmrf_block* b, const uint8_t* other);
int launch_energy_delta(const phmrf_block* b, double* accum_at = nullptr);
int launch_posterior_stats(const phmrf_block* b, float beta, int estimate_type, bool write_posteriors);
int launch_posterior_summary(const phmrf_block* b, float beta, int estimate_type, float* conf, uint8_t* top,
                             float* entropy);
int launch_ancestral(const phmrf_block* b, float beta, int estimate_type, int weighting, int A, const float* tab, float* mean_out,
                     float* sd_out);
int launch_chain_colour(const phmrf_block* b, float beta, int family, int colour, int phase);
int launch_component_pass(phmrf_block* b, float beta);
int launch_component_prepare(phmrf_block* b);
int launch_grid_components(int32_t* comp, int64_t n, int W, int diagonal, const uint8_t* labels, hipStream_t st);
int launch_grid_graph(const phmrf_block* b, int H, int W, int diagonal, int nn, double beta1);
int launch_propose(phmrf_block* b, float beta);
int launch_strip_pass(const phmrf_block* b, float beta, int orient, int shift_r, int shift_c, int alpha,
                      int geom = -1);
int launch_strip_multi(const phmrf_block* b, float beta, int orient, int shift_r, int shift_c, unsigned long long label_mask,
                       int geom = -1);
int launch_kmeans_step(const phmrf_block* b, const float* centers_dev, bool write_labels, double* acc_dev, bool outer = false);
int launch_fwd_weights(phmrf_block* b);
int64_t coarse_nodes(const phmrf_block* b, int s, int off);
int launch_coarsen(const phmrf_block* b, phmrf_block* child, int s, int off, int alpha, float beta);
int launch_coarsen_batch(const phmrf_block* b, phmrf_block* const* children, const int* alphas, int nl, int s, int off, float beta,
                         const unsigned int* rebuild, int since, bool reset);
int launch_coarse_apply(const phmrf_block* b, const phmrf_block* child, int s, int off, int alpha, const unsigned long long* gate = nullptr,
                        unsigned int* moved_flag = nullptr, unsigned long long* changed_label = nullptr);
int launch_c2f_graph(const phmrf_block* b, phmrf_block* child, int Hc, int Wc, int s);
int launch_c2f_logprob(const phmrf_block* b, phmrf_block* child, int Wc, int s);
int launch_c2f_prolong(const phmrf_block* b, const phmrf_block* child, int Wc, int s);
int launch_graph_expansion(phmrf_block* b, float beta, int alpha);
int launch_unary_planes(phmrf_block* b);
constexpr float PIN_COST = 1.0e9f;
int launch_tile_pins(phmrf_block* b, int region, int64_t first, int64_t count, int64_t pinned_first, int64_t pinned_count,
                     int64_t was_first, int64_t was_count, bool save_first);
int launch_put_labels(phmrf_block* b, int64_t first, int64_t count, const uint8_t* src_dev);

template <class I = int64_t>
__host__ __device__ __forceinline__ I grid_row_first(int i, int W, int diagonal) {
  return diagonal ? (I)i * W - ((I)i * (i - 1)) / 2 : (I)i * W;
}
template <class I = int64_t>
__host__ __device__ __forceinline__ I grid_row_base(int i, int W, int diagonal) {
  return diagonal ? (I)i * W - ((I)i * (i - 1)) / 2 - i : (I)i * W;
}
template <class I = int64_t>
__host__ __device__ __forceinline__ I grid_id(int i, int j, int W, int diagonal) {
  return diagonal ? grid_row_first<I>(i, W, 1) + (j - i) : (I)i * W + j;
}
template <class I = int64_t>
__host__ __device__ __forceinline__ I grid_node(int i, int j, int H, int W, int diagonal) {
  if (i < 0 || i >= H || j < 0 || j >= W || (diagonal && i > j)) return -1;
  return grid_id<I>(i, j, W, diagonal);
}
inline int64_t row_first(const phmrf_block* b, int i) { return grid_row_first(i, b->W, b->diagonal); }
__host__ __device__ __forceinline__ void grid_coords(int64_t v, int W, int diagonal, int* i, int* j) {
  if (!diagonal) {
    *i = (int)(v / W);
    *j = (int)(v - (int64_t)(*i) * W);
    return;
  }
  const double bq = 2.0 * W + 1.0;
  int r = (int)((bq - sqrt(bq * bq - 8.0 * (double)v)) * 0.5);
  r = r < 0 ? 0 : (r > W - 1 ? W - 1 : r);
  while (r > 0 && grid_row_first(r, W, 1) > v) --r;
  while (r + 1 < W && grid_row_first(r + 1, W, 1) <= v) ++r;
  *i = r;
  *j = r + (int)(v - grid_row_first(r, W, 1));
}

struct Geometry {
  int H, W, diagonal;
  explicit Geometry(int H_, int W_, int diag) : H(H_), W(W_), diagonal(diag) {}
  int64_t count() const { return grid_row_first(H, W, diagonal); }
  void coords(int64_t id, int* i, int* j) const { grid_coords(id, W, diagonal, i, j); }
  int64_t id(int i, int j) const { return grid_row_base(i, W, diagonal) + j; }
  bool valid(int i, int j) const { return i >= 0 && i < H && j >= 0 && j < W && (!diagonal || i <= j); }
};

__host__ __device__ __forceinline__ unsigned grid_neighbour_ids(int64_t v, int i, int j, int H, int W, int diagonal,
                                                                int64_t (&c)[8]) {
  const int64_t up = grid_row_base(i - 1, W, diagonal), dn = grid_row_base(i + 1, W, diagonal);
  const int jlo_dn = diagonal ? i + 1 : 0;
  const bool has[8] = {i > 0 && j - 1 >= 0, i > 0, i > 0 && j + 1 < W, j - 1 >= (diagonal ? i : 0), j + 1 < W,
                       i + 1 < H && j - 1 >= jlo_dn, i + 1 < H && j >= jlo_dn, i + 1 < H && j + 1 < W};
  const int64_t id[8] = {up + j - 1, up + j, up + j + 1, v - 1, v + 1, dn + j - 1, dn + j, dn + j + 1};
  unsigned mask = 0;
#pragma unroll
  for (int d = 0; d < 8; ++d) {
    c[d] = has[d] ? id[d] : v;
    mask |= has[d] ? 1u << d : 0u;
  }
  return mask;
}

template <class I>
__host__ __device__ __forceinline__ void grid_forward_ids(I v, int i, int j, int H, int W, int diagonal, bool on, I (&c)[4]) {
  const I dn = grid_row_base<I>(i + 1, W, diagonal);
  const int jlo = diagonal ? i + 1 : 0;
  const bool below = on && i + 1 < H;
  c[0] = (on && j + 1 < W) ? v + 1 : v;
  c[1] = (below && j - 1 >= jlo) ? dn + j - 1 : v;
  c[2] = (below && j >= jlo) ? dn + j : v;
  c[3] = (below && j + 1 < W) ? dn + j + 1 : v;
}

__device__ __forceinline__ void grid_gather_neighbours(int64_t v, int i, int j, int H, int W, int diagonal,
                                                       const float4* __restrict__ fwd_w, int64_t (&c)[8], float (&w)[8]) {
  const unsigned has = grid_neighbour_ids(v, i, j, H, W, diagonal, c);
  const float4 own = fwd_w[v];
  const float4 f0 = fwd_w[c[0]], f1 = fwd_w[c[1]], f2 = fwd_w[c[2]], f3 = fwd_w[c[3]];
  w[0] = (has & 1u) ? f0.w : 0.f;
  w[1] = (has & 2u) ? f1.z : 0.f;
  w[2] = (has & 4u) ? f2.y : 0.f;
  w[3] = (has & 8u) ? f3.x : 0.f;
  w[4] = (has & 16u) ? own.x : 0.f;
  w[5] = (has & 32u) ? own.y : 0.f;
  w[6] = (has & 64u) ? own.z : 0.f;
  w[7] = (has & 128u) ? own.w : 0.f;
}

}
```

### phylo_hmrf_amd/csrc/kernels.hip

```cpp

#include <cstdlib>

#include "common.h"

namespace phmrf {

namespace {

constexpr int ACC_COST = 0;
constexpr int ACC_ENERGY = 4;
constexpr int ACC_STATS = 8;

constexpr double ENERGY_FIX = 1048576.0;
__device__ __forceinline__ void energy_flush(double* accum, double tu, double tp, int det) {
  if (det) {
    atomicAdd(reinterpret_cast<unsigned long long*>(accum + ACC_ENERGY), (unsigned long long)__double2ll_rn(tu * ENERGY_FIX));
    atomicAdd(reinterpret_cast<unsigned long long*>(accum + ACC_ENERGY + 1), (unsigned long long)__double2ll_rn(tp * ENERGY_FIX));
  } else {
    atomicAdd(accum + ACC_ENERGY, tu);
    atomicAdd(accum + ACC_ENERGY + 1, tp);
  }
}

__device__ __forceinline__ double wave_sum(double v) {
#pragma unroll
  for (int off = 32; off > 0; off >>= 1) v += __shfl_down(v, off, 64);
  return v;
}

__device__ __forceinline__ double block_sum(double v, double* red) {
  v = wave_sum(v);
  const int lane = threadIdx.x & 63, wave = threadIdx.x >> 6;
  __syncthreads();
  if (lane == 0) red[wave] = v;
  __syncthreads();
  double t = 0.0;
  if (threadIdx.x == 0) {
    const int nw = (blockDim.x + 63) >> 6;
    for (int i = 0; i < nw; ++i) t += red[i];
  }
  return t;
}

template <int VEC, bool ACCUM>
__device__ __forceinline__ void rows_to_tile(const float* __restrict__ mat, const int32_t* __restrict__ nodes,
                                             int64_t base, int rows, int K, int Kp, float* tile, float scale,
                                             float tile_scale) {
  const int KV = K / VEC;
  const int total = rows * KV;
  auto ld = [&](int q, float (&v)[VEC]) {
    const int r = q / KV;
    const int c = (q - r * KV) * VEC;
    const int64_t node = nodes ? (int64_t)nodes[base + r] : base + r;
    const float* src = mat + node * K + c;
    if (VEC == 4) {
      const float4 t = *reinterpret_cast<const float4*>(src);
      v[0] = t.x; v[1] = t.y; v[2] = t.z; v[3] = t.w;
    } else if (VEC == 2) {
      const float2 t = *reinterpret_cast<const float2*>(src);
      v[0] = t.x; v[1] = t.y;
    } else {
      v[0] = src[0];
    }
  };
  auto st = [&](int q, const float (&v)[VEC]) {
    const int r = q / KV;
    const int c = (q - r * KV) * VEC;
    float* dst = tile + r * Kp + c;
#pragma unroll
    for (int j = 0; j < VEC; ++j) dst[j] = ACCUM ? fmaf(tile_scale, dst[j], scale * v[j]) : scale * v[j];
  };
  const int step = blockDim.x;
  int q = threadIdx.x;
  for (; q + 3 * step < total; q += 4 * step) {
    float v0[VEC], v1[VEC], v2[VEC], v3[VEC];
    ld(q, v0); ld(q + step, v1); ld(q + 2 * step, v2); ld(q + 3 * step, v3);
    st(q, v0); st(q + step, v1); st(q + 2 * step, v2); st(q + 3 * step, v3);
  }
  for (; q < total; q += step) {
    float v[VEC];
    ld(q, v);
    st(q, v);
  }
}

template <int VEC>
__device__ __forceinline__ void tile_to_rows(float* __restrict__ out, int rows, int K, int Kp, const float* tile) {
  const int KV = K / VEC;
  const int total = rows * KV;
  for (int q = threadIdx.x; q < total; q += blockDim.x) {
    const int r = q / KV;
    const int c = (q - r * KV) * VEC;
    const float* s = tile + r * Kp + c;
    float* d = out + (int64_t)r * K + c;
    if (VEC == 4) {
      *reinterpret_cast<float4*>(d) = make_float4(s[0], s[1], s[2], s[3]);
    } else if (VEC == 2) {
      *reinterpret_cast<float2*>(d) = make_float2(s[0], s[1]);
    } else {
      d[0] = s[0];
    }
  }
}

inline int vec_of(int K) { return (K % 4 == 0) ? 4 : (K % 2 == 0 ? 2 : 1); }

inline int grid_for(int64_t work_items, int tb, int max_blocks = 256 * 16) {
  int64_t g = (work_items + tb - 1) / tb;
  if (g > max_blocks) g = max_blocks;
  if (g < 1) g = 1;
  return (int)g;
}

template <int S, int VEC>
__global__ __launch_bounds__(256) void emission_kernel(const float* __restrict__ X, int64_t n, int K, int Kp,
                                                       const float* __restrict__ P, float* __restrict__ out,
                                                       float* __restrict__ uT) {
  extern __shared__ float tile[];
  constexpr int PS = S + S * (S + 1) / 2 + 1;
  const int TB = blockDim.x;
  for (int64_t base = (int64_t)blockIdx.x * TB; base < n; base += (int64_t)gridDim.x * TB) {
    const int64_t i = base + threadIdx.x;
    if (i < n) {
      float x[S];
      if (S % 4 == 0) {
#pragma unroll
        for (int s = 0; s < S; s += 4) {
          const float4 t = *reinterpret_cast<const float4*>(X + i * S + s);
          x[s] = t.x; x[s + 1] = t.y; x[s + 2] = t.z; x[s + 3] = t.w;
        }
      } else {
#pragma unroll
        for (int s = 0; s < S; ++s) x[s] = X[i * S + s];
      }
      float* row = tile + threadIdx.x * Kp;
      for (int k = 0; k < K; ++k) {
        const float* p = P + k * PS;
        float d[S];
#pragma unroll
        for (int s = 0; s < S; ++s) d[s] = x[s] - p[s];
        float q = 0.f;
        int idx = S;
#pragma unroll
        for (int r = 0; r < S; ++r) {
          float y = 0.f;
#pragma unroll
          for (int c = 0; c <= r; ++c) y = fmaf(p[idx++], d[c], y);
          q = fmaf(y, y, q);
        }
        const float lp = fmaf(-0.5f, q, p[idx]);
        row[k] = lp;
        if (uT) uT[(int64_t)k * n + i] = -lp;
      }
    }
    __syncthreads();
    const int64_t rem = n - base;
    const int rows = rem < TB ? (int)rem : TB;
    tile_to_rows<VEC>(out + base * K, rows, K, Kp, tile);
    __syncthreads();
  }
}

template <int S>
int launch_emission_s(const float* X, int64_t n, int K, const float* packed, float* logprob, float* uT, hipStream_t st) {
  const int TB = tile_threads(K), Kp = padded_k(K);
  const size_t lds = (size_t)TB * Kp * sizeof(float);
  const int grid = grid_for(n, TB);
  switch (vec_of(K)) {
    case 4: hipLaunchKernelGGL((emission_kernel<S, 4>), dim3(grid), dim3(TB), lds, st, X, n, K, Kp, packed, logprob, uT); break;
    case 2: hipLaunchKernelGGL((emission_kernel<S, 2>), dim3(grid), dim3(TB), lds, st, X, n, K, Kp, packed, logprob, uT); break;
    default: hipLaunchKernelGGL((emission_kernel<S, 1>), dim3(grid), dim3(TB), lds, st, X, n, K, Kp, packed, logprob, uT); break;
  }
  PHMRF_HIP(hipGetLastError());
  return PHMRF_OK;
}

template <int VEC>
__global__ __launch_bounds__(256) void argmax_kernel(const float* __restrict__ logprob, int64_t n, int K, int Kp,
                                                     uint8_t* __restrict__ labels) {
  extern __shared__ float tile[];
  const int TB = blockDim.x;
  for (int64_t base = (int64_t)blockIdx.x * TB; base < n; base += (int64_t)gridDim.x * TB) {
    const int64_t rem = n - base;
    const int rows = rem < TB ? (int)rem : TB;
    rows_to_tile<VEC, false>(logprob, nullptr, base, rows, K, Kp, tile, 1.f, 0.f);
    __syncthreads();
    if ((int)threadIdx.x < rows) {
      const float* row = tile + threadIdx.x * Kp;
      float best = row[0];
      int bk = 0;
      for (int k = 1; k < K; ++k) {
        const float v = row[k];
        if (v > best) { best = v; bk = k; }
      }
      labels[base + threadIdx.x] = (uint8_t)bk;
    }
    __syncthreads();
  }
}

template <int VEC>
__global__ __launch_bounds__(256) void icm_kernel(const float* __restrict__ logprob, const int32_t* __restrict__ nodes,
                                                  int64_t count, int K, int Kp, int D,
                                                  const int32_t* __restrict__ nbr, const float* __restrict__ wgt,
                                                  uint8_t* __restrict__ labels, float beta,
                                                  unsigned long long* __restrict__ changed,
                                                  uint16_t* __restrict__ stamp, int tick) {
  extern __shared__ float tile[];
  const int TB = blockDim.x;
  unsigned int my_changed = 0;
  for (int64_t base = (int64_t)blockIdx.x * TB; base < count; base += (int64_t)gridDim.x * TB) {
    const int64_t rem = count - base;
    const int rows = rem < TB ? (int)rem : TB;
    rows_to_tile<VEC, false>(logprob, nodes, base, rows, K, Kp, tile, -1.f, 0.f);
    __syncthreads();
    if ((int)threadIdx.x < rows) {
      const int64_t node = nodes ? (int64_t)nodes[base + threadIdx.x] : base + threadIdx.x;
      float* row = tile + threadIdx.x * Kp;
      const int32_t* nb = nbr + node * D;
      const float* wg = wgt + node * D;
      for (int j = 0; j < D; j += 4) {
        const int4 c = *reinterpret_cast<const int4*>(nb + j);
        const float4 w = *reinterpret_cast<const float4*>(wg + j);
        if (c.x >= 0) row[labels[c.x]] -= beta * w.x;
        if (c.y >= 0) row[labels[c.y]] -= beta * w.y;
        if (c.z >= 0) row[labels[c.z]] -= beta * w.z;
        if (c.w >= 0) row[labels[c.w]] -= beta * w.w;
      }
      const int cur = labels[node];
      float best = row[cur];
      int bk = cur;
      for (int k = 0; k < K; ++k) {
        const float v = row[k];
        if (v < best) { best = v; bk = k; }
      }
      if (bk != cur) {
        labels[node] = (uint8_t)bk;
        if (stamp) {
          stamp[node] = (uint16_t)tick;
          for (int j = 0; j < D; ++j)
            if (nb[j] >= 0) stamp[nb[j]] = (uint16_t)tick;
        }
        ++my_changed;
      }
    }
    __syncthreads();
  }
  unsigned int s = my_changed;
#pragma unroll
  for (int off = 32; off > 0; off >>= 1) s += __shfl_down(s, off, 64);
  if ((threadIdx.x & 63) == 0 && s) atomicAdd(changed, (unsigned long long)s);
}

__global__ __launch_bounds__(256) void energy_kernel(const float* __restrict__ logprob, int64_t n, int K, int D,
                                                     const int32_t* __restrict__ nbr, const float* __restrict__ wgt,
                                                     const uint8_t* __restrict__ labels, double* __restrict__ accum, int det) {
  __shared__ double red[8];
  double eu = 0.0, ep = 0.0;
  for (int64_t i = (int64_t)blockIdx.x * blockDim.x + threadIdx.x; i < n; i += (int64_t)gridDim.x * blockDim.x) {
    const int l = labels[i];
    eu -= (double)logprob[i * K + l];
    const int32_t* nb = nbr + i * D;
    const float* wg = wgt + i * D;
    float s = 0.f;
    for (int j = 0; j < D; j += 4) {
      const int4 c = *reinterpret_cast<const int4*>(nb + j);
      const float4 w = *reinterpret_cast<const float4*>(wg + j);
      if (c.x >= 0 && labels[c.x] != l) s += w.x;
      if (c.y >= 0 && labels[c.y] != l) s += w.y;
      if (c.z >= 0 && labels[c.z] != l) s += w.z;
      if (c.w >= 0 && labels[c.w] != l) s += w.w;
    }
    ep += (double)s;
  }
  const double tu = block_sum(eu, red);
  const double tp = block_sum(ep, red);
  if (threadIdx.x == 0) energy_flush(accum, tu, 0.5 * tp, det);
}

__global__ __launch_bounds__(256) void energy_grid_kernel(const float* __restrict__ logprob, const float* __restrict__ uT,
                                                          int64_t n, int K, int H, int W,
                                                          int diagonal, const float4* __restrict__ fwd_w,
                                                          const uint8_t* __restrict__ labels, double* __restrict__ accum, int det,
                                                          int row0, int row1) {
  __shared__ double red[8];
  const int j = blockIdx.x * 64 + (threadIdx.x & 63);
  double eu = 0.0, ep = 0.0;
  constexpr int UR = 4;
  const int stride = gridDim.y * 4;
  const int row_end = (diagonal && blockIdx.x * 64 + 64 < row1) ? blockIdx.x * 64 + 64 : row1;
  for (int i0 = row0 + blockIdx.y * 4 + (threadIdx.x >> 6); i0 < row_end; i0 += stride * UR) {
    int64_t node[UR];
    int lab[UR];
    bool on[UR];
#pragma unroll
    for (int u = 0; u < UR; ++u) {
      const int i = i0 + u * stride;
      on[u] = i < row1 && j < W && !(diagonal && j < i);
      node[u] = on[u] ? grid_row_base(i, W, diagonal) + j : 0;
      lab[u] = labels[node[u]];
    }
    float un[UR];
    float4 w[UR];
#pragma unroll
    for (int u = 0; u < UR; ++u) {
      un[u] = uT ? uT[(int64_t)lab[u] * n + node[u]] : -logprob[node[u] * K + lab[u]];
      w[u] = fwd_w[node[u]];
    }
    int ln[UR][4];
#pragma unroll
    for (int u = 0; u < UR; ++u) {
      int64_t c[4];
      grid_forward_ids(node[u], i0 + u * stride, j, H, W, diagonal, on[u], c);
      ln[u][0] = labels[c[0]]; ln[u][1] = labels[c[1]]; ln[u][2] = labels[c[2]]; ln[u][3] = labels[c[3]];
    }
#pragma unroll
    for (int u = 0; u < UR; ++u) {
      if (!on[u]) continue;
      const int l = lab[u];
      eu += (double)un[u];
      float s = 0.f;
      if (ln[u][0] != l) s += w[u].x;
      if (ln[u][1] != l) s += w[u].y;
      if (ln[u][2] != l) s += w[u].z;
      if (ln[u][3] != l) s += w[u].w;
      ep += (double)s;
    }
  }
  const double tu = block_sum(eu, red);
  const double tp = block_sum(ep, red);
  if (threadIdx.x == 0) energy_flush(accum, tu, tp, det);
}

__global__ __launch_bounds__(256) void energy_delta_grid_kernel(const float* __restrict__ uT, int64_t n, int H, int W, int diagonal,
                                                                const float4* __restrict__ fwd_w,
                                                                const uint8_t* __restrict__ labels,
                                                                const uint8_t* __restrict__ prev,
                                                                const uint16_t* __restrict__ stamp, int since,
                                                                double* __restrict__ accum, int det, int row0, int row1) {
  __shared__ double red[8];
  const int j = blockIdx.x * 64 + (threadIdx.x & 63);
  double eu = 0.0, ep = 0.0;
  constexpr int UR = 4;
  const int stride = gridDim.y * 4;
  const int row_end = (diagonal && blockIdx.x * 64 + 64 < row1) ? blockIdx.x * 64 + 64 : row1;
  for (int i0 = row0 + blockIdx.y * 4 + (threadIdx.x >> 6); i0 < row_end; i0 += stride * UR) {
    int64_t node[UR];
    bool on[UR];
    bool any = false;
#pragma unroll
    for (int u = 0; u < UR; ++u) {
      const int i = i0 + u * stride;
      const bool in = i < row1 && j < W && !(diagonal && j < i);
      node[u] = in ? grid_row_base(i, W, diagonal) + j : 0;
      on[u] = in && (int)stamp[node[u]] > since;
      any = any || on[u];
    }
    if (!__any(any)) continue;
    int lab[UR], labp[UR];
#pragma unroll
    for (int u = 0; u < UR; ++u) {
      lab[u] = labels[node[u]];
      labp[u] = prev[node[u]];
    }
    float un[UR], unp[UR];
    float4 w[UR];
#pragma unroll
    for (int u = 0; u < UR; ++u) {
      un[u] = uT[(int64_t)lab[u] * n + node[u]];
      unp[u] = uT[(int64_t)labp[u] * n + node[u]];
      w[u] = fwd_w[node[u]];
    }
    int ln[UR][4], lp[UR][4];
#pragma unroll
    for (int u = 0; u < UR; ++u) {
      int64_t c[4];
      grid_forward_ids(node[u], i0 + u * stride, j, H, W, diagonal, on[u], c);
      ln[u][0] = labels[c[0]]; ln[u][1] = labels[c[1]]; ln[u][2] = labels[c[2]]; ln[u][3] = labels[c[3]];
      lp[u][0] = prev[c[0]]; lp[u][1] = prev[c[1]]; lp[u][2] = prev[c[2]]; lp[u][3] = prev[c[3]];
    }
#pragma unroll
    for (int u = 0; u < UR; ++u) {
      if (!on[u]) continue;
      const int l = lab[u], q = labp[u];
      eu += (double)un[u] - (double)unp[u];
      float s = 0.f;
      s += (ln[u][0] != l ? w[u].x : 0.f) - (lp[u][0] != q ? w[u].x : 0.f);
      s += (ln[u][1] != l ? w[u].y : 0.f) - (lp[u][1] != q ? w[u].y : 0.f);
      s += (ln[u][2] != l ? w[u].z : 0.f) - (lp[u][2] != q ? w[u].z : 0.f);
      s += (ln[u][3] != l ? w[u].w : 0.f) - (lp[u][3] != q ? w[u].w : 0.f);
      ep += (double)s;
    }
  }
  const double tu = block_sum(eu, red);
  const double tp = block_sum(ep, red);
  if (threadIdx.x == 0 && (tu != 0.0 || tp != 0.0)) energy_flush(accum, tu, tp, det);
}

__global__ __launch_bounds__(256) void energy_diff_grid_kernel(const float* __restrict__ uT, int64_t n, int H, int W, int diagonal,
                                                               const float4* __restrict__ fwd_w,
                                                               const uint8_t* __restrict__ labels,
                                                               const uint8_t* __restrict__ other, double* __restrict__ accum,
                                                               int det, int row0, int row1) {
  __shared__ double red[8];
  const int j = blockIdx.x * 64 + (threadIdx.x & 63);
  double eu = 0.0, ep = 0.0;
  constexpr int UR = 4;
  const int stride = gridDim.y * 4;
  const int row_end = (diagonal && blockIdx.x * 64 + 64 < row1) ? blockIdx.x * 64 + 64 : row1;
  for (int i0 = row0 + blockIdx.y * 4 + (threadIdx.x >> 6); i0 < row_end; i0 += stride * UR) {
    int64_t me[UR], c[UR][4];
    bool in[UR];
#pragma unroll
    for (int u = 0; u < UR; ++u) {
      const int i = i0 + u * stride;
      in[u] = i < row1 && j < W && !(diagonal && j < i);
      me[u] = in[u] ? grid_row_base(i, W, diagonal) + j : 0;
      grid_forward_ids(me[u], i, j, H, W, diagonal, in[u], c[u]);
    }
    int la[UR], lb[UR], na[UR][4], nb[UR][4];
    bool on[UR];
    bool any = false;
#pragma unroll
    for (int u = 0; u < UR; ++u) {
      la[u] = labels[me[u]];
      lb[u] = other[me[u]];
#pragma unroll
      for (int q = 0; q < 4; ++q) {
        na[u][q] = labels[c[u][q]];
        nb[u][q] = other[c[u][q]];
      }
    }
#pragma unroll
    for (int u = 0; u < UR; ++u) {
      on[u] = in[u] && (la[u] != lb[u] || na[u][0] != nb[u][0] || na[u][1] != nb[u][1] || na[u][2] != nb[u][2] || na[u][3] != nb[u][3]);
      any = any || on[u];
    }
    if (!__any(any)) continue;
#pragma unroll
    for (int u = 0; u < UR; ++u) {
      if (!on[u]) continue;
      const float4 w = fwd_w[me[u]];
      if (la[u] != lb[u]) eu += (double)uT[(int64_t)la[u] * n + me[u]] - (double)uT[(int64_t)lb[u] * n + me[u]];
      float s = 0.f;
      s += (na[u][0] != la[u] ? w.x : 0.f) - (nb[u][0] != lb[u] ? w.x : 0.f);
      s += (na[u][1] != la[u] ? w.y : 0.f) - (nb[u][1] != lb[u] ? w.y : 0.f);
      s += (na[u][2] != la[u] ? w.z : 0.f) - (nb[u][2] != lb[u] ? w.z : 0.f);
      s += (na[u][3] != la[u] ? w.w : 0.f) - (nb[u][3] != lb[u] ? w.w : 0.f);
      ep += (double)s;
    }
  }
  const double tu = block_sum(eu, red);
  const double tp = block_sum(ep, red);
  if (threadIdx.x == 0 && (tu != 0.0 || tp != 0.0)) energy_flush(accum, tu, tp, det);
}

typedef float f32x16 __attribute__((ext_vector_type(16)));
typedef float f32x4 __attribute__((ext_vector_type(4)));

template <int S>
__device__ __forceinline__ int stat_slot(int K, int o, int* second) {
  constexpr int M = 1 + S + S * (S + 1) / 2;
  const int k = o / M, m = o - k * M;
  *second = -1;
  if (m == 0) return k;
  if (m <= S) return K + k * S + (m - 1);
  int q = m - 1 - S, ps = 0;
  while (q >= S - ps) { q -= S - ps; ++ps; }
  const int pt = ps + q;
  if (pt != ps) *second = K + K * S + k * S * S + pt * S + ps;
  return K + K * S + k * S * S + ps * S + pt;
}

template <int S, int VEC, bool WRITE_POST, bool GRID>
__global__ __launch_bounds__(256, 5) void posterior_kernel(const float* __restrict__ X, const float* __restrict__ logprob,
                                                        int64_t n, int K, int Kp, int D,
                                                        const int32_t* __restrict__ nbr, const float* __restrict__ wgt,
                                                        const uint8_t* __restrict__ labels, float beta, int use_w,
                                                        float* __restrict__ post_out, double* __restrict__ accum,
                                                        int gH, int gW, int gdiag, const float4* __restrict__ fwd_w,
                                                        int64_t n_first, double* __restrict__ partial) {
  extern __shared__ float lds[];
  constexpr int M = 1 + S + S * (S + 1) / 2;
  constexpr int Mp = ((S + 1) % 2 == 0) ? S + 2 : S + 1;
  constexpr int NMB = (M + 15) / 16;
  const int TB = blockDim.x;
  float* tile = lds;
  float* feat = lds + TB * Kp;
  __shared__ double red[8];

  const int KM = K * M;
  double* sacc = reinterpret_cast<double*>(lds + TB * (Kp + Mp));
  for (int o = threadIdx.x; o < KM; o += TB) sacc[o] = 0.0;
  const int wave = threadIdx.x >> 6, lane = threadIdx.x & 63;
  double c_pair = 0.0, c_pcn = 0.0, c_un = 0.0;
  int fa[NMB], fb[NMB];
#pragma unroll
  for (int q = 0; q < NMB; ++q) {
    const int m = q * 16 + (lane & 15);
    int a = 0, bq = 0;
    if (m >= 1 && m <= S) {
      bq = m;
    } else if (m > S && m < M) {
      int r = m - 1 - S, ps = 0;
      while (r >= S - ps) { r -= S - ps; ++ps; }
      a = ps + 1;
      bq = ps + r + 1;
    }
    fa[q] = a;
    fb[q] = bq;
  }
  __syncthreads();

  for (int64_t base = n_first + (int64_t)blockIdx.x * TB; base < n; base += (int64_t)gridDim.x * TB) {
    const int64_t rem = n - base;
    const int rows = rem < TB ? (int)rem : TB;
    const int64_t i = base + threadIdx.x;
    const bool live = (int)threadIdx.x < rows;
    float* row = tile + threadIdx.x * Kp;
    float wtot = 0.f;
    int li = 0;
    if (live) {
      li = labels[i];
      for (int k = 0; k < K; ++k) row[k] = 0.f;
      const int32_t* nb = nbr + i * D;
      const float* wg = wgt + i * D;
      float diff = 0.f;
      int deg = 0;
      if (GRID) {
        int gi, gj;
        grid_coords(i, gW, gdiag, &gi, &gj);
        int64_t cc[8];
        float ww[8];
        grid_gather_neighbours(i, gi, gj, gH, gW, gdiag, fwd_w, cc, ww);
        int ll[8];
#pragma unroll
        for (int t = 0; t < 8; ++t) ll[t] = labels[cc[t]];
#pragma unroll
        for (int t = 0; t < 8; ++t) {
          if (cc[t] != i) {
            const float w = use_w ? ww[t] : 1.f;
            const int l = ll[t];
            row[l] += w;
            wtot += w;
            if (l != li) diff += w;
            ++deg;
          }
        }
      } else if (D == 8) {
        const int4 c0 = *reinterpret_cast<const int4*>(nb), c1 = *reinterpret_cast<const int4*>(nb + 4);
        const float4 w0 = *reinterpret_cast<const float4*>(wg), w1 = *reinterpret_cast<const float4*>(wg + 4);
        const int cc[8] = {c0.x, c0.y, c0.z, c0.w, c1.x, c1.y, c1.z, c1.w};
        const float ww[8] = {w0.x, w0.y, w0.z, w0.w, w1.x, w1.y, w1.z, w1.w};
        int ll[8];
#pragma unroll
        for (int t = 0; t < 8; ++t) ll[t] = labels[cc[t] >= 0 ? (int64_t)cc[t] : i];
#pragma unroll
        for (int t = 0; t < 8; ++t) {
          if (cc[t] >= 0) {
            const float w = use_w ? ww[t] : 1.f;
            const int l = ll[t];
            row[l] += w;
            wtot += w;
            if (l != li) diff += w;
            ++deg;
          }
        }
      } else
      for (int j = 0; j < D; j += 4) {
        const int4 c = *reinterpret_cast<const int4*>(nb + j);
        const float4 wv = *reinterpret_cast<const float4*>(wg + j);
        const int cc[4] = {c.x, c.y, c.z, c.w};
        const float ww[4] = {wv.x, wv.y, wv.z, wv.w};
        int ll[4];
#pragma unroll
        for (int t = 0; t < 4; ++t) ll[t] = labels[cc[t] >= 0 ? (int64_t)cc[t] : i];
#pragma unroll
        for (int t = 0; t < 4; ++t) {
          if (cc[t] >= 0) {
            const float w = use_w ? ww[t] : 1.f;
            const int l = ll[t];
            row[l] += w;
            wtot += w;
            if (l != li) diff += w;
            ++deg;
          }
        }
      }
      c_pair += (double)(beta * diff);
      if (!deg) {
        row[li] = 1.f;
        wtot = 1.f;
      }
      float mb = -3.0e38f;
      for (int k = 0; k < K; ++k) mb = fmaxf(mb, beta * (row[k] - wtot));
      float s2 = 0.f;
      for (int k = 0; k < K; ++k) s2 += __expf(beta * (row[k] - wtot) - mb);
      const float ppn = __expf(beta * (row[li] - wtot) - mb) / s2;
      c_pcn -= (double)logf(ppn + 1e-16f);
      c_un -= (double)logprob[i * K + li];
    }
    __syncthreads();
// ... 298 lines not shown
      const float4 t = *reinterpret_cast<const float4*>(X + i * S + s);
      x[s] = t.x; x[s + 1] = t.y; x[s + 2] = t.z; x[s + 3] = t.w;
    }
  } else {
#pragma unroll
    for (int s = 0; s < S; ++s) x[s] = X[i * S + s];
  }
}

template <int S>
__device__ __forceinline__ float affine_map(const float* __restrict__ t, const float (&x)[S]) {
  float mu = t[0];
#pragma unroll
  for (int s = 0; s < S; ++s) mu = fmaf(t[1 + s], x[s], mu);
  return mu;
}

template <int S, int VEC, bool GRID>
__global__ __launch_bounds__(256) void ancestral_kernel(const float* __restrict__ X, const float* __restrict__ logprob, int64_t n,
                                                        int K, int Kp, int D, const int32_t* __restrict__ nbr,
                                                        const float* __restrict__ wgt, const uint8_t* __restrict__ labels,
                                                        float beta, int use_w, int gH, int gW, int gdiag,
                                                        const float4* __restrict__ fwd_w, int64_t n_first, int A,
                                                        const float* __restrict__ tab, float* __restrict__ mean_out,
                                                        float* __restrict__ sd_out) {
  extern __shared__ float lds[];
  constexpr int TS = S + 2;
  const int TB = blockDim.x;
  const int64_t m = n - n_first;
  float* tile = lds;
  for (int64_t base = n_first + (int64_t)blockIdx.x * TB; base < n; base += (int64_t)gridDim.x * TB) {
    const int64_t rem = n - base;
    const int rows = rem < TB ? (int)rem : TB;
    const int64_t i = base + threadIdx.x;
    const bool live = (int)threadIdx.x < rows;
    float* row = tile + threadIdx.x * Kp;
    if (live) label_histogram<GRID>(row, i, labels[i], K, D, nbr, wgt, labels, use_w, gH, gW, gdiag, fwd_w);
    __syncthreads();
    rows_to_tile<VEC, true>(logprob, nullptr, base, rows, K, Kp, tile, 1.f, beta);
    __syncthreads();
    if (live) {
      float mx = -3.0e38f;
      for (int k = 0; k < K; ++k) mx = fmaxf(mx, row[k]);
      float s1 = 0.f;
      for (int k = 0; k < K; ++k) {
        const float e = __expf(row[k] - mx);
        row[k] = e;
        s1 += e;
      }
      const float inv = 1.f / s1;
      float x[S];
      load_observation<S>(X, i, x);
      const int64_t o = i - n_first;
      for (int a0 = 0; a0 < A; a0 += ANC_CHUNK) {
        const int ac = A - a0 < ANC_CHUNK ? A - a0 : ANC_CHUNK;
        float mean[ANC_CHUNK], var[ANC_CHUNK];
#pragma unroll
        for (int q = 0; q < ANC_CHUNK; ++q) mean[q] = var[q] = 0.f;
        for (int k = 0; k < K; ++k) {
          const float p = row[k] * inv;
          const float* t = tab + ((size_t)k * A + a0) * TS;
#pragma unroll
          for (int q = 0; q < ANC_CHUNK; ++q)
            if (q < ac) mean[q] = fmaf(p, affine_map<S>(t + q * TS, x), mean[q]);
        }
#pragma unroll
        for (int q = 0; q < ANC_CHUNK; ++q)
          if (q < ac) mean_out[(int64_t)(a0 + q) * m + o] = mean[q];
        if (sd_out) {
          for (int k = 0; k < K; ++k) {
            const float p = row[k] * inv;
            const float* t = tab + ((size_t)k * A + a0) * TS;
#pragma unroll
            for (int q = 0; q < ANC_CHUNK; ++q)
              if (q < ac) {
                const float d = affine_map<S>(t + q * TS, x) - mean[q];
                var[q] = fmaf(p, fmaf(d, d, t[q * TS + S + 1]), var[q]);
              }
          }
#pragma unroll
          for (int q = 0; q < ANC_CHUNK; ++q)
            if (q < ac) sd_out[(int64_t)(a0 + q) * m + o] = sqrtf(var[q]);
        }
      }
    }
    __syncthreads();
  }
}

template <int S>
__global__ __launch_bounds__(256) void ancestral_called_kernel(const float* __restrict__ X, int64_t n,
                                                               const uint8_t* __restrict__ labels, int64_t n_first, int A,
                                                               const float* __restrict__ tab, float* __restrict__ mean_out,
                                                               float* __restrict__ sd_out) {
  constexpr int TS = S + 2;
  const int64_t m = n - n_first;
  for (int64_t i = n_first + (int64_t)blockIdx.x * blockDim.x + threadIdx.x; i < n; i += (int64_t)gridDim.x * blockDim.x) {
    float x[S];
    load_observation<S>(X, i, x);
    const float* t = tab + (size_t)labels[i] * A * TS;
    const int64_t o = i - n_first;
    for (int a = 0; a < A; ++a, t += TS) {
      mean_out[(int64_t)a * m + o] = affine_map<S>(t, x);
      if (sd_out) sd_out[(int64_t)a * m + o] = sqrtf(t[S + 1]);
    }
  }
}

constexpr int ANC_GRID_CAP = 256 * 8;

template <int S>
int launch_ancestral_s(const phmrf_block* b, float beta, int estimate_type, int weighting, int A, const float* tab, float* mean_out,
                       float* sd_out) {
  const int K = b->K, TB = tile_threads(K), Kp = padded_k(K);
  const int64_t n_first = b->own1 >= 0 ? b->own0 : 0, n_last = b->own1 >= 0 ? b->own1 : b->n;
  if (n_last <= n_first) return PHMRF_OK;
  if (weighting == 1) {
    const int grid = grid_for(n_last - n_first, 256, ANC_GRID_CAP);
    hipLaunchKernelGGL((ancestral_called_kernel<S>), dim3(grid), dim3(256), 0, b->stream, b->X, n_last, b->labels, n_first, A, tab,
                       mean_out, sd_out);
    PHMRF_HIP(hipGetLastError());
    return PHMRF_OK;
  }
  const size_t lds = (size_t)TB * Kp * sizeof(float);
  const int grid = grid_for(n_last - n_first, TB, ANC_GRID_CAP * (256 / TB));
  const int use_w = estimate_type == 3 ? 1 : 0;
  const bool grid_form = b->has_grid && b->grid_complete && b->fwd_w && b->D == 8 && b->num_neighbor == 8;
#define PHMRF_LAUNCH_ANC(VEC_, G_)                                                                                          \
  hipLaunchKernelGGL((ancestral_kernel<S, VEC_, G_>), dim3(grid), dim3(TB), lds, b->stream, b->X, b->logprob, n_last, K, Kp, \
                     b->D, b->nbr, b->wgt, b->labels, beta, use_w, b->H, b->W, b->diagonal, b->fwd_w, n_first, A, tab,       \
                     mean_out, sd_out)
  switch (vec_of(K)) {
    case 4: if (grid_form) PHMRF_LAUNCH_ANC(4, true); else PHMRF_LAUNCH_ANC(4, false); break;
    case 2: if (grid_form) PHMRF_LAUNCH_ANC(2, true); else PHMRF_LAUNCH_ANC(2, false); break;
    default: if (grid_form) PHMRF_LAUNCH_ANC(1, true); else PHMRF_LAUNCH_ANC(1, false); break;
  }
#undef PHMRF_LAUNCH_ANC
  PHMRF_HIP(hipGetLastError());
  return PHMRF_OK;
}

}

int launch_ancestral(const phmrf_block* b, float beta, int estimate_type, int weighting, int A, const float* tab, float* mean_out,
                     float* sd_out) {
  switch (b->S) {
#define PHMRF_CASE(S_) case S_: return launch_ancestral_s<S_>(b, beta, estimate_type, weighting, A, tab, mean_out, sd_out);
    PHMRF_CASE(1) PHMRF_CASE(2) PHMRF_CASE(3) PHMRF_CASE(4) PHMRF_CASE(5) PHMRF_CASE(6) PHMRF_CASE(7) PHMRF_CASE(8)
#undef PHMRF_CASE
  }
  return fail(PHMRF_ERR_UNSUPPORTED, "ancestral: S must be in [1,8]");
}

int launch_emission(const float* X, int64_t n, int S, int K, const float* packed, float* logprob, float* uT, hipStream_t st) {
  switch (S) {
#define PHMRF_CASE(S_) case S_: return launch_emission_s<S_>(X, n, K, packed, logprob, uT, st);
    PHMRF_CASE(1) PHMRF_CASE(2) PHMRF_CASE(3) PHMRF_CASE(4) PHMRF_CASE(5) PHMRF_CASE(6) PHMRF_CASE(7) PHMRF_CASE(8)
    PHMRF_CASE(9) PHMRF_CASE(10) PHMRF_CASE(11) PHMRF_CASE(12) PHMRF_CASE(13) PHMRF_CASE(14) PHMRF_CASE(15) PHMRF_CASE(16)
#undef PHMRF_CASE
  }
  return fail(PHMRF_ERR_UNSUPPORTED, "emission: S must be in [1,16]");
}

int launch_argmax_labels(const phmrf_block* b) {
  const int K = b->K, TB = tile_threads(K), Kp = padded_k(K);
  const size_t lds = (size_t)TB * Kp * sizeof(float);
  const int grid = grid_for(b->n, TB);
  switch (vec_of(K)) {
    case 4: hipLaunchKernelGGL((argmax_kernel<4>), dim3(grid), dim3(TB), lds, b->stream, b->logprob, b->n, K, Kp, b->labels); break;
    case 2: hipLaunchKernelGGL((argmax_kernel<2>), dim3(grid), dim3(TB), lds, b->stream, b->logprob, b->n, K, Kp, b->labels); break;
    default: hipLaunchKernelGGL((argmax_kernel<1>), dim3(grid), dim3(TB), lds, b->stream, b->logprob, b->n, K, Kp, b->labels); break;
  }
  PHMRF_HIP(hipGetLastError());
  return PHMRF_OK;
}

int launch_icm_colour(const phmrf_block* b, float beta, int colour) {
  const int K = b->K, TB = tile_threads(K), Kp = padded_k(K);
  const int64_t lo = b->colour_ptr[colour], hi = b->colour_ptr[colour + 1];
  const int64_t count = hi - lo;
  if (count <= 0) return PHMRF_OK;
  const size_t lds = (size_t)TB * Kp * sizeof(float);
  const int grid = grid_for(count, TB);
  const int32_t* nodes = b->colour_nodes + lo;
  switch (vec_of(K)) {
    case 4: hipLaunchKernelGGL((icm_kernel<4>), dim3(grid), dim3(TB), lds, b->stream, b->logprob, nodes, count, K, Kp, b->D, b->nbr, b->wgt, b->labels, beta, b->counters + b->counter_slot, b->tick ? b->stamp : nullptr, b->tick); break;
    case 2: hipLaunchKernelGGL((icm_kernel<2>), dim3(grid), dim3(TB), lds, b->stream, b->logprob, nodes, count, K, Kp, b->D, b->nbr, b->wgt, b->labels, beta, b->counters + b->counter_slot, b->tick ? b->stamp : nullptr, b->tick); break;
    default: hipLaunchKernelGGL((icm_kernel<1>), dim3(grid), dim3(TB), lds, b->stream, b->logprob, nodes, count, K, Kp, b->D, b->nbr, b->wgt, b->labels, beta, b->counters + b->counter_slot, b->tick ? b->stamp : nullptr, b->tick); break;
  }
  PHMRF_HIP(hipGetLastError());
  return PHMRF_OK;
}

__global__ __launch_bounds__(256) void choose_labels_kernel(uint8_t* __restrict__ labels, const uint8_t* __restrict__ saved, int64_t n,
                                                            const double* __restrict__ acc_cur, const double* __restrict__ acc_sav,
                                                            double beta, int det) {
  double cu, cp, su, sp;
  if (det) {
    cu = (double)reinterpret_cast<const long long*>(acc_cur)[0] / ENERGY_FIX;
    cp = (double)reinterpret_cast<const long long*>(acc_cur)[1] / ENERGY_FIX;
    su = (double)reinterpret_cast<const long long*>(acc_sav)[0] / ENERGY_FIX;
    sp = (double)reinterpret_cast<const long long*>(acc_sav)[1] / ENERGY_FIX;
  } else {
    cu = acc_cur[0]; cp = acc_cur[1]; su = acc_sav[0]; sp = acc_sav[1];
  }
  if (cu + beta * cp < su + beta * sp) return;
  for (int64_t i = ((int64_t)blockIdx.x * blockDim.x + threadIdx.x) * 16; i < n; i += (int64_t)gridDim.x * blockDim.x * 16) {
    if (i + 16 <= n && ((reinterpret_cast<uintptr_t>(labels + i) | reinterpret_cast<uintptr_t>(saved + i)) & 15) == 0) {
      *reinterpret_cast<uint4*>(labels + i) = *reinterpret_cast<const uint4*>(saved + i);
    } else {
      for (int64_t q = i; q < n && q < i + 16; ++q) labels[q] = saved[q];
    }
  }
}

int launch_choose_labels(const phmrf_block* b, const uint8_t* saved, const double* acc_cur, const double* acc_sav, double beta) {
  int64_t g64 = (b->n / 16 + 255) / 256 + 1;
  const int grid = (int)(g64 > 4096 ? 4096 : g64);
  hipLaunchKernelGGL(choose_labels_kernel, dim3(grid), dim3(256), 0, b->stream, b->labels, saved, b->n, acc_cur, acc_sav, beta,
                     b->deterministic ? 1 : 0);
  PHMRF_HIP(hipGetLastError());
  return PHMRF_OK;
}

bool energy_diff_available(const phmrf_block* b) {
  return b->has_grid && b->fwd_w && b->H > 0 && b->W > 0 && b->uT && b->uT_valid;
}

int launch_energy_diff(const phmrf_block* b, const uint8_t* other) {
  const int gx = (b->W + 63) / 64;
  int gy = (b->H + 3) / 4;
  const int cap = 2048 / gx + 1;
  if (gy > cap) gy = cap;
  const int row0 = b->own_r1 >= 0 ? b->own_r0 : 0, row1 = b->own_r1 >= 0 ? b->own_r1 : b->H;
  hipLaunchKernelGGL(energy_diff_grid_kernel, dim3(gx, gy), dim3(256), 0, b->stream, b->uT, b->n, b->H, b->W, b->diagonal, b->fwd_w,
                     b->labels, other, b->accum, b->deterministic ? 1 : 0, row0, row1);
  PHMRF_HIP(hipGetLastError());
  return PHMRF_OK;
}

int launch_energy(const phmrf_block* b, float beta, double* accum_at) {
  (void)beta;
  double* const acc = accum_at ? accum_at - ACC_ENERGY : b->accum;
  if (b->has_grid && b->fwd_w && b->H > 0 && b->W > 0) {
    const int gx = (b->W + 63) / 64;
    int gy = (b->H + 3) / 4;
    const int cap = 2048 / gx + 1;
    if (gy > cap) gy = cap;
    const int row0 = b->own_r1 >= 0 ? b->own_r0 : 0, row1 = b->own_r1 >= 0 ? b->own_r1 : b->H;
    hipLaunchKernelGGL(energy_grid_kernel, dim3(gx, gy), dim3(256), 0, b->stream, b->logprob,
                       (b->uT && b->uT_valid) ? b->uT : nullptr, b->n, b->K, b->H, b->W, b->diagonal, b->fwd_w, b->labels, acc,
                       b->deterministic ? 1 : 0, row0, row1);
    PHMRF_HIP(hipGetLastError());
    return PHMRF_OK;
  }
  const int grid = grid_for(b->n, 256, 256 * 8);
  hipLaunchKernelGGL(energy_kernel, dim3(grid), dim3(256), 0, b->stream, b->logprob, b->n, b->K, b->D, b->nbr, b->wgt,
                     b->labels, acc, b->deterministic ? 1 : 0);
  PHMRF_HIP(hipGetLastError());
  return PHMRF_OK;
}

bool energy_delta_available(const phmrf_block* b) {
  return b->has_grid && b->fwd_w && b->H > 0 && b->W > 0 && b->uT && b->uT_valid && b->stamp && b->tick > 0 && b->labels_eval &&
         b->eval_tick >= 0;
}

int launch_energy_delta(const phmrf_block* b, double* accum_at) {
  double* const acc = accum_at ? accum_at - ACC_ENERGY : b->accum;
  const int gx = (b->W + 63) / 64;
  int gy = (b->H + 3) / 4;
  const int cap = 2048 / gx + 1;
  if (gy > cap) gy = cap;
  const int row0 = b->own_r1 >= 0 ? b->own_r0 : 0, row1 = b->own_r1 >= 0 ? b->own_r1 : b->H;
  hipLaunchKernelGGL(energy_delta_grid_kernel, dim3(gx, gy), dim3(256), 0, b->stream, b->uT, b->n, b->H, b->W, b->diagonal,
                     b->fwd_w, b->labels, b->labels_eval, b->stamp, b->eval_tick, acc, b->deterministic ? 1 : 0, row0, row1);
  PHMRF_HIP(hipGetLastError());
  return PHMRF_OK;
}

int launch_posterior_stats(const phmrf_block* b, float beta, int estimate_type, bool write_posteriors) {
  switch (b->S) {
#define PHMRF_CASE(S_) case S_: return launch_posterior_s<S_>(b, beta, estimate_type, write_posteriors);
    PHMRF_CASE(1) PHMRF_CASE(2) PHMRF_CASE(3) PHMRF_CASE(4) PHMRF_CASE(5) PHMRF_CASE(6) PHMRF_CASE(7) PHMRF_CASE(8)
#undef PHMRF_CASE
  }
  return fail(PHMRF_ERR_UNSUPPORTED, "posterior_stats: S must be in [1,8]");
}

}
```

### phylo_hmrf_amd/csrc/solve.hip

```cpp

#include <algorithm>
#include <cmath>
#include <cstdio>
#include <cstdlib>
#include <cstring>
#include <limits>
#include <thread>

#include "common.h"

namespace phmrf {

static const int COARSE_SCALE[N_COARSE] = {2, 4, 8};
static const int COARSE_CHILD_SLOT = COUNTER_EXPANSION + 1;
static const int GEOM_R[3] = {0, 2, 4}, GEOM_C[3] = {0, 21, 42};
static const int64_t COARSE_ON_DIV = 8;
static const int64_t COARSE_ROUND_DIV = 4;
static const int64_t MOVING_DIV_AT_LARGE = 64;
static const int64_t MOVING_DIV = 16;
static const int TICK_BUDGET = 60000;

static int coarse_children_create(phmrf_block_t b) {
  auto up = [](size_t x) { return (x + 255) & ~(size_t)255; };
  constexpr int NC = N_COARSE_CHILDREN;
  size_t off_lab[NC], off_uT[NC], off_fwd[NC], total = up((size_t)NC * N_COUNTERS * sizeof(unsigned long long));
  int64_t nm[NC];
  for (int ls = 0; ls < N_COARSE_CHILDREN; ++ls) {
    const int s = COARSE_SCALE[ls / 4];
    nm[ls] = coarse_nodes(b, s, s - 1);
    off_lab[ls] = total;
    total += up((size_t)nm[ls]);
    off_uT[ls] = total;
    total += up((size_t)2 * nm[ls] * sizeof(float));
    off_fwd[ls] = total;
    total += up((size_t)nm[ls] * sizeof(float4));
  }
  PHMRF_HIP(hipMalloc(reinterpret_cast<void**>(&b->coarse_arena), total));
  PHMRF_HIP(hipMemsetAsync(b->coarse_arena, 0, (size_t)NC * N_COUNTERS * sizeof(unsigned long long), b->stream));
  for (int ls = 0; ls < N_COARSE_CHILDREN; ++ls) {
    phmrf_block* c = new phmrf_block();
    c->n = nm[ls];
    c->S = 1;
    c->K = 2;
    c->device = b->device;
    c->deterministic = b->deterministic;
    c->counters = reinterpret_cast<unsigned long long*>(b->coarse_arena) + (size_t)ls * N_COUNTERS;
    c->labels = reinterpret_cast<uint8_t*>(b->coarse_arena + off_lab[ls]);
    c->uT = reinterpret_cast<float*>(b->coarse_arena + off_uT[ls]);
    c->fwd_w = reinterpret_cast<float4*>(b->coarse_arena + off_fwd[ls]);
    c->uT_valid = true;
    c->has_grid = true;
    c->has_graph = true;
    c->has_logprob = true;
    c->D = 0;
    c->unary_pins = true;
    c->stream = b->stream;
    b->coarse[ls] = c;
  }
  return PHMRF_OK;
}

void coarse_children_destroy(phmrf_block* b) {
  for (int ls = 0; ls < N_COARSE_CHILDREN; ++ls) {
    delete b->coarse[ls];
    b->coarse[ls] = nullptr;
  }
  if (b->coarse_arena) (void)hipFree(b->coarse_arena);
  b->coarse_arena = nullptr;
}

int coarse_child(phmrf_block* b, int level_slot, phmrf_block** out) {
  if (!b->coarse_arena) PHMRF_TRY(coarse_children_create(b));
  b->coarse[level_slot]->stream = b->stream;
  b->coarse[level_slot]->num_neighbor = b->num_neighbor;
  *out = b->coarse[level_slot];
  return PHMRF_OK;
}

int coarse_sweep_nocount(phmrf_block* b, float beta, int level, int off, int shift_r, int shift_c, int alpha_lo, int alpha_hi,
                         unsigned long long label_mask) {
  const int s = COARSE_SCALE[level];
  if (!b->uT_valid) PHMRF_TRY(launch_unary_planes(b));
  static const int batch_env = PHMRF_DEV_ENV("PHMRF_COARSE_BATCH") ? atoi(PHMRF_DEV_ENV("PHMRF_COARSE_BATCH")) : 4;
  const int batch = (batch_env == 1 || batch_env == 2) ? batch_env : 4;
  static const bool no_gate = PHMRF_DEV_ENV("PHMRF_COARSE_NO_GATE") != nullptr;
  static const bool no_stamp_gate = PHMRF_DEV_ENV("PHMRF_COARSE_NO_STAMP_GATE") != nullptr;
  phmrf_block* ch[4] = {nullptr, nullptr, nullptr, nullptr};
  for (int q = 0; q < batch; ++q) PHMRF_TRY(coarse_child(b, level * 4 + q, &ch[q]));
  if (!b->coarse_flag) PHMRF_TRY(dev_alloc(&b->coarse_flag, (size_t)1));
  tic(b, KC_COARSE);
  int n_launch = 0;
  std::vector<int> todo;
  for (int a = alpha_lo; a < alpha_hi; ++a)
    if ((label_mask >> a) & 1ull) todo.push_back(a);
  for (size_t t0 = 0; t0 < todo.size(); t0 += (size_t)batch) {
    const int nl = (int)std::min<size_t>((size_t)batch, todo.size() - t0);
    int alphas[4] = {0, 0, 0, 0};
    for (int q = 0; q < nl; ++q) alphas[q] = todo[t0 + q];
    for (int q = 0; q < nl; ++q) ch[q]->counter_slot = COARSE_CHILD_SLOT;
    PHMRF_TRY(launch_coarsen_batch(b, ch, alphas, nl == 3 ? 3 : nl, s, off, beta, nullptr, -1, true));
    const int since = (b->tick && !no_stamp_gate) ? b->tick : -1;
    ++n_launch;
    for (int q = 0; q < nl; ++q) {
      phmrf_block* c = ch[q];
      if (q > 0) {
        phmrf_block* one[1] = {c};
        PHMRF_TRY(launch_coarsen_batch(b, one, &alphas[q], 1, s, off, beta, b->coarse_flag, since, false));
        ++n_launch;
      }
      PHMRF_TRY(launch_strip_pass(c, beta, 0, shift_r % 6, shift_c % 64, 1, -1));
      PHMRF_TRY(launch_strip_pass(c, beta, 1, (shift_r + 3) % 6, (shift_c + 31) % 64, 1, -1));
      if (b->tick) ++b->tick;
      PHMRF_TRY(launch_coarse_apply(b, c, s, off, alphas[q], no_gate ? nullptr : c->counters + COARSE_CHILD_SLOT, b->coarse_flag,
                                    b->coarse_lab ? b->coarse_lab + level * MAX_LABELS + alphas[q] : nullptr));
      n_launch += 3;
    }
  }
  toc(b, KC_COARSE, n_launch);
  return PHMRF_OK;
}

static int energy_round_launch(phmrf_block* b, bool* incremental_out, bool* snapshot_out) {
  static const bool always_full = PHMRF_DEV_ENV("PHMRF_ENERGY_FULL") != nullptr;
  static const char* const min_n_env = PHMRF_DEV_ENV("PHMRF_ENERGY_MIN_N");
  static const int64_t min_n = min_n_env ? std::max<int64_t>(1, std::atoll(min_n_env)) : (int64_t)1 << 18;
  const bool grid = b->has_grid && b->fwd_w && b->uT && b->uT_valid && b->stamp && b->tick > 0 && b->n >= min_n;
  const bool snapshot = grid && !always_full;
  const bool incremental = snapshot && energy_delta_available(b);
  tic(b, KC_ENERGY);
  double* const at = reinterpret_cast<double*>(b->counters + COUNTER_ENERGY);
  if (incremental) {
    PHMRF_TRY(launch_energy_delta(b, at));
    b->work[WORK_INCREMENTAL] += 1;
  } else {
    PHMRF_TRY(launch_energy(b, 0.f, at));
  }
  toc(b, KC_ENERGY, 1);
  if (is_tile(b))
    PHMRF_HIP(hipMemcpyAsync(b->accum_host + 6, b->accum + 6, sizeof(double), hipMemcpyDeviceToHost, b->stream));
  if (snapshot) {
    if (!b->labels_eval) PHMRF_TRY(dev_alloc(&b->labels_eval, (size_t)b->n));
    PHMRF_HIP(hipMemcpyAsync(b->labels_eval, b->labels, (size_t)b->n, hipMemcpyDeviceToDevice, b->stream));
    b->eval_tick = b->tick;
    ++b->tick;
  }
  *incremental_out = incremental;
  *snapshot_out = snapshot;
  return PHMRF_OK;
}

static int energy_round_collect(phmrf_block* b, double beta, bool incremental, double* eu_carry, double* ep_carry) {
  static const bool check = PHMRF_DEV_ENV("PHMRF_ENERGY_CHECK") != nullptr;
  double du, dp;
  energy_sums(b, b->counters_host + COUNTER_ENERGY, &du, &dp);
  if (incremental) {
    *eu_carry += du;
    *ep_carry += dp;
  } else {
    *eu_carry = du;
    *ep_carry = dp;
  }
  if (check && incremental) {
    double fu, fp;
    PHMRF_TRY(energy_now(b, beta, &fu, &fp));
    const double eu = *eu_carry, ep = beta * *ep_carry;
    const double tol = 1e-9 * std::fabs(fu + fp) + 1e-3;
    if (std::fabs(fu - eu) > tol || std::fabs(fp - ep) > tol)
      fprintf(stderr, "[phmrf energy check] incremental %.6f + %.6f, full %.6f + %.6f (diff %.3e, %.3e)\n", eu, ep, fu, fp,
              eu - fu, ep - fp);
  }
  return PHMRF_OK;
}

void solve_scope_exit(phmrf_block* b) {
  phmrf_solve_state* s = b->ss;
  if (s) b->geom_phase = (s->geom + 1) % 3;
  b->tick = 0;
  b->eval_tick = -1;
  b->counter_slot = COUNTER_DEFAULT;
  b->prop_tick = -1;
  delete s;
  b->ss = nullptr;
}

int tile_queue_boundary(phmrf_block* b) {
  int64_t off = 0;
  if (b->tile_top) {
    const int64_t tf = row_first(b, 1), tc = row_first(b, 2) - tf;
    PHMRF_HIP(hipMemcpyAsync(b->xfer_host, b->labels + tf, (size_t)tc, hipMemcpyDeviceToHost, b->stream));
    off = tc;
  }
  if (b->tile_bot) {
    const int64_t bf = row_first(b, b->H - 2), bc = row_first(b, b->H - 1) - bf;
    PHMRF_HIP(hipMemcpyAsync(b->xfer_host + off, b->labels + bf, (size_t)bc, hipMemcpyDeviceToHost, b->stream));
  }
  b->boundary_queued = true;
  return PHMRF_OK;
}

}

using namespace phmrf;

struct EndSolves {
  phmrf_block_t* bl;
  int n;
  ~EndSolves() {
    for (int i = 0; i < n; ++i)
      if (bl[i]->ss) {
        (void)hipStreamSynchronize(bl[i]->stream);
        solve_scope_exit(bl[i]);
      }
  }
};

namespace phmrf {
bool c2f_applies(const phmrf_block* b) {
  if (!b->has_grid || !b->fwd_w || b->num_neighbor != 8 || !b->grid_complete || is_tile(b)) return false;
  return b->n >= 1024 && b->H >= 2 * C2F_SCALE && b->W >= 2 * C2F_SCALE;
}

int c2f_child(phmrf_block* b) {
  const int s = C2F_SCALE;
  if (!b->c2f) {
    const int Hc = (b->H + s - 1) / s, Wc = (b->W + s - 1) / s;
    Geometry gc(Hc, Wc, b->diagonal);
    phmrf_block_t c = nullptr;
    PHMRF_TRY(phmrf_block_create(gc.count(), 1, b->K, &c));
    auto build = [&]() -> int {
      c->stream = b->stream;
      PHMRF_TRY(dev_alloc(&c->nbr, (size_t)c->n * 8));
      PHMRF_TRY(dev_alloc(&c->wgt, (size_t)c->n * 8));
      c->D = 8;
      PHMRF_TRY(launch_c2f_graph(b, c, Hc, Wc, s));
      if (!c->colour_nodes) PHMRF_TRY(dev_alloc(&c->colour_nodes, (size_t)c->n));
      c->has_graph = true;
      PHMRF_TRY(setup_grid_tables(c, gc, 8));
      c->grid_complete = true;
      return PHMRF_OK;
    };
    const int st = build();
    if (st != PHMRF_OK) {
      (void)hipStreamSynchronize(b->stream);
      c->stream = c->own_stream;
      (void)phmrf_block_destroy(c);
      return st;
    }
    b->c2f = c;
    b->c2f_Hc = Hc;
    b->c2f_Wc = Wc;
  }
  b->c2f->stream = b->stream;
  return PHMRF_OK;
}
}

static int c2f_start(phmrf_block* b, double beta, const phmrf_solve_opts& o, bool* started) {
  *started = false;
  if (o.coarse_start <= 0 || !o.use_strips || !c2f_applies(b)) return PHMRF_OK;
  const int s = C2F_SCALE;
  PHMRF_TRY(c2f_child(b));
  phmrf_block* c = b->c2f;
  PHMRF_TRY(launch_c2f_logprob(b, c, b->c2f_Wc, s));
  c->has_logprob = true;
  c->uT_valid = false;
  phmrf_solve_opts oc = o;
  oc.init_mode = 1;
  PHMRF_TRY(phmrf_mrf_solve(c, beta, &oc, nullptr));
  PHMRF_TRY(launch_c2f_prolong(b, c, b->c2f_Wc, s));
  *started = true;
  return PHMRF_OK;
}

static void count_into(phmrf_block* b, int slot) {
  b->counter_slot = slot;
  b->ss->ran[slot] = 1;
}
static void activate_all(phmrf_solve_state* s) {
  for (int sl : s->slots) s->active[sl] = 1;
}
static bool out_of_budget(const phmrf_block* b) { return b->ss->rounds >= b->ss->o.max_rounds || b->tick >= TICK_BUDGET; }
static bool moved_at_large(const phmrf_solve_state* s) { return s->total * COARSE_ON_DIV >= s->sched_n; }
static bool last_round_moved_at_large(const phmrf_solve_state* s) { return s->last_changed * COARSE_ROUND_DIV >= s->sched_n; }
static bool rests_coarse_labels(const phmrf_block* b) { return !is_tile(b) && b->ss->o.energy_tol_ppb > 0; }
static bool verifies_coarse(const phmrf_solve_state* s) { return s->verifying && (s->o.energy_tol_ppb == 0 || moved_at_large(s)); }
static bool coarse_scale_on(const phmrf_solve_state* s, int lv) {
  return verifies_coarse(s) || s->force_coarse ||
         (s->active[COUNTER_COARSE + lv] && (last_round_moved_at_large(s) || s->coarse_changed[lv] > 0));
}
static bool coarse_runs_all_labels(const phmrf_block* b) {
  const phmrf_solve_state* s = b->ss;
  return !rests_coarse_labels(b) || verifies_coarse(s) || s->force_coarse || last_round_moved_at_large(s);
}

static int solve_begin(phmrf_block* b, double beta, const phmrf_solve_opts* opts, bool want_init_energy) {
  PHMRF_TRY(check_solvable(b));
  if (b->ss) solve_scope_exit(b);
  phmrf_solve_state* s = new phmrf_solve_state();
  b->ss = s;
  phmrf_solve_opts& o = s->o;
  std::memset(&o, 0, sizeof(o));
  o.max_rounds = 64;
  o.use_chains = 1;
  o.use_components = 1;
  o.use_strips = 1;
  o.use_expansion = 1;
  o.use_coarse = 1;
  if (opts) {
    o = *opts;
    if (o.max_rounds <= 0) o.max_rounds = 64;
  }
  s->beta = beta;
  s->bf = (float)beta;
  s->sched_n = b->sched_n > 0 ? b->sched_n : b->n;
  b->labels_are_slot = 0;
  EndSolves abort_guard{&b, 1};
  if (o.init_mode == 1) {
    bool started = false;
    PHMRF_TRY(c2f_start(b, beta, o, &started));
    if (!started) PHMRF_TRY(launch_argmax_labels(b));
    b->has_labels = true;
  }
  if (want_init_energy) {
    PHMRF_TRY(energy_now(b, beta, &s->eu0, &s->ep0));
    s->have_init_energy = true;
  }
  if (o.use_chains && !b->has_grid && b->families.empty() && b->nbr && b->n >= 2) PHMRF_TRY(setup_path_families(b));
  s->chains = o.use_chains && (b->has_grid || !b->families.empty());
  s->strips = o.use_strips && b->has_grid;
  s->tol = o.min_changed > 0 ? o.min_changed : 0;
  const int K = b->K;
  s->expansions = s->strips && o.use_expansion;
  s->graph_expansions = !b->has_grid && o.use_expansion && b->nbr != nullptr && b->n >= 2;
  s->n_fam = s->chains ? (int)b->families.size() : 0;
  PHMRF_CHECK(s->n_fam <= MAX_CHAIN_FAMILIES, PHMRF_ERR_INVALID, "internal: more chain families than counter slots");
  for (int f = 0; f < s->n_fam; ++f) s->slots.push_back(COUNTER_CHAIN + f);
  s->slots.push_back(COUNTER_ICM);
  if (o.use_components) s->slots.push_back(COUNTER_COMPONENT);
  if (s->strips) {
    s->slots.push_back(COUNTER_FUSION);
    s->slots.push_back(COUNTER_FUSION + 1);
  }
  if (s->expansions || s->graph_expansions)
    for (int a = 0; a < K; ++a) s->slots.push_back(COUNTER_EXPANSION + a);
  s->coarse = s->strips && o.use_coarse && b->H >= 4 && b->W >= 4;
  if (s->coarse)
    for (int lv = 0; lv < N_COARSE; ++lv) s->slots.push_back(COUNTER_COARSE + lv);
  activate_all(s);
  s->last_count.fill(-1);
  if (!b->stamp) PHMRF_TRY(dev_alloc(&b->stamp, (size_t)b->n));
  PHMRF_HIP(hipMemsetAsync(b->stamp, 0, (size_t)b->n * sizeof(uint16_t), b->stream));
  b->tick = 1;
  b->eval_tick = -1;
  b->prop_tick = -1;
  if (s->chains) {
    size_t total = 0;
    for (auto& f : b->families)
      for (int p = 0; p < 2; ++p)
        for (int c = 0; c < f.n_colours; ++c) total += (size_t)f.nseg[p][c];
    if (!b->chain_memo || b->chain_memo_count != total) {
      dev_free(b->chain_memo);
      PHMRF_TRY(dev_alloc(&b->chain_memo, total));
      b->chain_memo_count = total;
    }
    size_t off = 0;
    for (auto& f : b->families)
      for (int p = 0; p < 2; ++p)
        for (int c = 0; c < f.n_colours; ++c) {
          f.memo[p][c] = f.nseg[p][c] > 0 ? b->chain_memo + off : nullptr;
          off += (size_t)f.nseg[p][c];
        }
    PHMRF_HIP(hipMemsetAsync(b->chain_memo, 0, (total ? total : 1) * sizeof(uint16_t), b->stream));
  }
  if (s->strips) {
    int64_t max_strips = 0;
    for (int orient = 0; orient < 2; ++orient) {
      const int Hs = orient ? b->W : b->H, Ws = orient ? b->H : b->W;
      const int64_t ns = (int64_t)((Hs + 5 + 5) / 6) * ((Ws + 63 + 63) / 64);
      max_strips = std::max(max_strips, ns);
    }
    if (!b->memo || b->memo_strips < max_strips) {
      dev_free(b->memo);
      PHMRF_TRY(dev_alloc(&b->memo, (size_t)6 * max_strips * (K + 1)));
      b->memo_strips = max_strips;
    }
    PHMRF_HIP(hipMemsetAsync(b->memo, 0, (size_t)6 * b->memo_strips * (K + 1) * sizeof(uint16_t), b->stream));
  }
  s->e_prev = (s->have_init_energy && !is_tile(b)) ? s->eu0 + s->ep0 : std::numeric_limits<double>::infinity();
  s->geom = b->geom_phase % 3;
  if (is_tile(b)) PHMRF_TRY(zero_accum(b, 6, 1));
  abort_guard.n = 0;
  return PHMRF_OK;
}

static int round_chains(phmrf_block* b) {
  phmrf_solve_state* s = b->ss;
  const int n_ord_fams = s->expansions ? 0 : (b->has_grid ? 2 : s->n_fam);
  auto runs = [&](int f) { return s->active[COUNTER_CHAIN + f] && (f < n_ord_fams || s->verifying); };
  int n_chain = 0;
  for (int f = 0; f < s->n_fam; ++f)
    if (runs(f)) n_chain += b->families[f].n_colours;
  if (n_chain == 0) return PHMRF_OK;
  tic(b, KC_CHAIN);
  for (int f = 0; f < s->n_fam; ++f)
    if (runs(f)) {
      count_into(b, COUNTER_CHAIN + f);
      PHMRF_TRY(chain_sweep_nocount(b, s->bf, f, b->has_grid ? (s->verifying ? 1 : 0) : (s->rounds & 1), false));
    }
  toc(b, KC_CHAIN, n_chain);
  return PHMRF_OK;
}

static int round_icm(phmrf_block* b) {
  phmrf_solve_state* s = b->ss;
  if (!(s->active[COUNTER_ICM] && (s->verifying || !(s->chains || s->strips) || !b->has_grid))) return PHMRF_OK;
  count_into(b, COUNTER_ICM);
  return icm_sweep_nocount(b, s->bf);
}

static int round_components(phmrf_block* b) {
  phmrf_solve_state* s = b->ss;
  const bool comp_round = s->rounds == 0 || s->verifying || s->prev_moving || !(s->chains || s->strips) || !b->has_grid;
  if (!(s->o.use_components && (s->active[COUNTER_COMPONENT] || s->prev_moving) && comp_round)) return PHMRF_OK;
  count_into(b, COUNTER_COMPONENT);
  if (b->tick) ++b->tick;
  tic(b, KC_COMPONENT);
  PHMRF_TRY(launch_component_pass(b, s->bf));
  toc(b, KC_COMPONENT, 1);
  return PHMRF_OK;
}

static int round_graph_expansions(phmrf_block* b) {
  phmrf_solve_state* s = b->ss;
  if (!s->graph_expansions) return PHMRF_OK;
  for (int a = 0; a < b->K; ++a)
    if (s->active[COUNTER_EXPANSION + a]) {
      count_into(b, COUNTER_EXPANSION + a);
      ++b->tick;
      tic(b, KC_STRIP);
      PHMRF_TRY(launch_graph_expansion(b, s->bf, a));
      toc(b, KC_STRIP, 1);
    }
  return PHMRF_OK;
}

static int round_strips(phmrf_block* b) {
  phmrf_solve_state* s = b->ss;
  if (!s->strips) return PHMRF_OK;
  const int K = b->K, geom = s->geom;
  for (int orient = 0; orient < 2; ++orient) {
    if (s->active[COUNTER_FUSION + orient]) {
      count_into(b, COUNTER_FUSION + orient);
      PHMRF_TRY(strip_pass_nocount(b, s->bf, orient, (GEOM_R[geom] + 3) % 6, (GEOM_C[geom] + 31) % 64, -1, geom));
    }
    if (!s->expansions) continue;
    unsigned long long lmask = 0ull;
    for (int a = 0; a < K; ++a)
      if (s->active[COUNTER_EXPANSION + a]) {
        lmask |= 1ull << a;
        s->ran[COUNTER_EXPANSION + a] = 1;
      }
    if (!lmask) continue;
    if (!b->uT_valid) {
      tic(b, KC_PROPOSE);
      PHMRF_TRY(launch_unary_planes(b));
      toc(b, KC_PROPOSE, 1);
    }
    tic(b, KC_STRIP);
    ++b->tick;
    PHMRF_TRY(launch_strip_multi(b, s->bf, orient, GEOM_R[geom], GEOM_C[geom], lmask, geom));
    b->tick += K;
    b->work[4] += 1;
    toc(b, KC_STRIP, 1);
  }
  return PHMRF_OK;
}

static int round_coarse(phmrf_block* b) {
  phmrf_solve_state* s = b->ss;
  if (!s->coarse) return PHMRF_OK;
  const int K = b->K, r = s->rounds;
  const size_t lab_bytes = (size_t)N_COARSE * MAX_LABELS * sizeof(unsigned long long);
  bool any_on = false;
  for (int lv = 0; lv < N_COARSE; ++lv) any_on = any_on || coarse_scale_on(s, lv);
  const bool count_labels = any_on && rests_coarse_labels(b);
  if (count_labels) {
    if (!b->coarse_lab) {
      PHMRF_TRY(dev_alloc(&b->coarse_lab, (size_t)N_COARSE * MAX_LABELS));
      PHMRF_HIP(hipHostMalloc(reinterpret_cast<void**>(&b->coarse_lab_host), lab_bytes));
    }
    PHMRF_HIP(hipMemsetAsync(b->coarse_lab, 0, lab_bytes, b->stream));
  }
  const bool verify_coarse = verifies_coarse(s), all_labels = coarse_runs_all_labels(b);
  const unsigned long long kmask = K >= MAX_LABELS ? ~0ull : ((1ull << K) - 1ull);
  for (int lv = 0; lv < N_COARSE; ++lv) {
    const int sc = COARSE_SCALE[lv];
    s->coarse_ran[lv] = coarse_scale_on(s, lv);
    if (!s->coarse_ran[lv]) continue;
    if (all_labels) s->coarse_lab_mask[lv] = kmask;
    s->coarse_all[lv] = all_labels;
    count_into(b, COUNTER_COARSE + lv);
    for (int off = 0; off < sc; ++off)
      if (verify_coarse || off == r % sc)
        PHMRF_TRY(coarse_sweep_nocount(b, s->bf, lv, off, (2 * r + lv + off) % 6, (17 * r + 5 * lv + 13 * off) % 64, 0, K,
                                       s->coarse_lab_mask[lv] & kmask));
  }
  if (count_labels)
    PHMRF_HIP(hipMemcpyAsync(b->coarse_lab_host, b->coarse_lab, lab_bytes, hipMemcpyDeviceToHost, b->stream));
  return PHMRF_OK;
}

int phmrf_mrf_solve_round_launch(phmrf_block_t b) {
  PHMRF_CHECK(b, PHMRF_ERR_INVALID, "block is NULL");
  phmrf_solve_state* s = b->ss;
  PHMRF_CHECK(s, PHMRF_ERR_STATE, "no solve in progress (phmrf_mrf_solve_begin)");
  PHMRF_CHECK(!s->launched, PHMRF_ERR_STATE, "the previous round has not been decided");
  if (s->status != 0) return PHMRF_OK;
  PHMRF_HIP(hipMemsetAsync(b->counters, 0, N_COUNTERS * sizeof(unsigned long long), b->stream));
  s->ran.fill(0);
  PHMRF_TRY(round_chains(b));
  PHMRF_TRY(round_icm(b));
  PHMRF_TRY(round_components(b));
  PHMRF_TRY(round_graph_expansions(b));
  PHMRF_TRY(round_strips(b));
  PHMRF_TRY(round_coarse(b));
  b->counter_slot = COUNTER_DEFAULT;
  if (b->timing) PHMRF_TRY(work_fetch_async(b));
  PHMRF_TRY(energy_round_launch(b, &s->incremental, &s->snapshot));
  PHMRF_HIP(hipMemcpyAsync(b->counters_host, b->counters, N_COUNTERS * sizeof(unsigned long long), hipMemcpyDeviceToHost,
                           b->stream));
  if (is_tile(b)) PHMRF_TRY(tile_queue_boundary(b));
  s->launched = true;
  s->collected = false;
  return PHMRF_OK;
}

int phmrf_mrf_solve_round_collect(phmrf_block_t b, uint64_t* counters, double* energy) {
  PHMRF_CHECK(b, PHMRF_ERR_INVALID, "block is NULL");
  phmrf_solve_state* s = b->ss;
  PHMRF_CHECK(s, PHMRF_ERR_STATE, "no solve in progress (phmrf_mrf_solve_begin)");
  if (s->status != 0 && !s->launched) {
    if (counters) std::memset(counters, 0, N_COUNTERS * sizeof(unsigned long long));
    if (energy) { energy[0] = s->eu_carry; energy[1] = s->ep_carry; }
    return PHMRF_OK;
  }
  PHMRF_CHECK(s->launched, PHMRF_ERR_STATE, "no round has been launched");
  if (!s->collected) {
    PHMRF_HIP(hipStreamSynchronize(b->stream));
    PHMRF_TRY(energy_round_collect(b, s->beta, s->incremental, &s->eu_carry, &s->ep_carry));
    if (b->timing) work_fold(b, s->rounds == 0);
    s->collected = true;
    if (is_tile(b)) {
      unsigned long long viol = 0;
      std::memcpy(&viol, b->accum_host + 6, sizeof(viol));
      PHMRF_CHECK(viol == 0, PHMRF_ERR_STATE, "internal: a pinned row of a tile has moved");
    }
  }
  if (counters) {
    std::memcpy(counters, b->counters_host, N_COUNTERS * sizeof(unsigned long long));
    counters[COUNTER_ENERGY] = counters[COUNTER_ENERGY + 1] = 0ull;
  }
  if (energy) { energy[0] = s->eu_carry; energy[1] = s->ep_carry; }
  return PHMRF_OK;
}

static int finish(phmrf_solve_state* s, int st, int* status) {
  s->status = st;
  s->converged = st == 1;
  if (status) *status = st;
  return PHMRF_OK;
}
static int next_round(phmrf_block* b, int* status) {
  if (out_of_budget(b)) return finish(b->ss, 2, status);
  if (status) *status = 0;
  return PHMRF_OK;
}

static int64_t fold_counters(phmrf_block* b, const uint64_t* counters) {
  phmrf_solve_state* s = b->ss;
  int64_t ch = 0;
  for (int sl : s->slots) {
    ch += (int64_t)counters[sl];
    if (s->ran[sl]) s->last_count[sl] = (long long)counters[sl];
  }
  s->total += ch;
  s->last_changed = ch;
  s->prev_moving = ch * (moved_at_large(s) ? MOVING_DIV_AT_LARGE : MOVING_DIV) >= s->sched_n;
  if (s->prev_moving) s->geom = (s->geom + 1) % 3;
  for (int lv = 0; lv < N_COARSE; ++lv)
    if (s->coarse_ran[lv]) {
      s->coarse_changed[lv] = (int64_t)counters[COUNTER_COARSE + lv];
      if (b->coarse_lab_host && rests_coarse_labels(b)) {
        unsigned long long keep = 0ull;
        for (int a = 0; a < b->K; ++a)
          if (b->coarse_lab_host[lv * MAX_LABELS + a] > 0ull) keep |= 1ull << a;
        s->coarse_lab_mask[lv] = keep;
      }
    }
  ++s->rounds;
  return ch;
}

static void trace_round(phmrf_block* b, const uint64_t* counters, int64_t ch, double e_now) {
  static const bool trace = getenv("PHMRF_SOLVE_TRACE") != nullptr;
  if (!trace) return;
  const phmrf_solve_state* s = b->ss;
  int n_active = 0;
  for (int sl : s->slots) n_active += s->active[sl];
  fprintf(stderr, "[phmrf solve] round %d active %d/%d changed %lld energy %.6f delta %.3e\n", s->rounds - 1, n_active,
          (int)s->slots.size(), (long long)ch, e_now, e_now - s->e_prev);
  if (!b->timing) return;
  static double seen[PHMRF_NUM_KERNEL_CLASSES] = {};
  resolve_timing(b);
  fprintf(stderr, "[phmrf solve]   ms:");
  static const char* NM[PHMRF_NUM_KERNEL_CLASSES] = {"emis", "icm", "chain", "comp", "energy", "post", "strip", "prop", "coarse", "fusion"};
  for (int kc = 0; kc < PHMRF_NUM_KERNEL_CLASSES; ++kc) {
    fprintf(stderr, " %s %.2f", NM[kc], b->ms[kc] - seen[kc]);
    seen[kc] = b->ms[kc];
  }
  fprintf(stderr, "  changed by slot:");
  for (int sl : s->slots)
    if (counters[sl]) fprintf(stderr, " %d:%llu", sl, (unsigned long long)counters[sl]);
  fprintf(stderr, "\n");
  const unsigned long long* t = b->counters_host + COUNTER_TRACE;
  if (t[TRACE_SEEN])
    fprintf(stderr, "[phmrf solve]   expansion strips: launched %llu, past memo+mask %llu, into DP %llu, DP steps %llu, with a move %llu\n",
            t[TRACE_SEEN], t[TRACE_PAST_MEMO], t[TRACE_INTO_DP], t[TRACE_DP_STEPS], t[TRACE_MOVED]);
}

static bool tolerance_decides(phmrf_block* b, double gain, bool coarse_moved, int* status) {
  phmrf_solve_state* s = b->ss;
  const phmrf_solve_opts& o = s->o;
  bool coarse_just_ran = s->coarse;
  for (int lv = 0; lv < N_COARSE; ++lv) coarse_just_ran = coarse_just_ran && s->coarse_ran[lv];
  if (coarse_moved && (o.energy_tol_ppb == 0 || is_tile(b))) s->coarse_checked = false;
  s->force_coarse = false;
  if (!(o.energy_tol_ppb > 0 && std::fabs(gain) < 1e-9 * o.energy_tol_ppb * std::fabs(s->e_prev))) return false;
  if (s->coarse && !s->coarse_checked && !coarse_just_ran && moved_at_large(s)) {
    s->coarse_checked = true;
    s->force_coarse = true;
    activate_all(s);
    next_round(b, status);
    return true;
  }
  finish(s, 1, status);
  return true;
}

static bool quiet_decides(phmrf_block* b, int64_t ch, bool improved, int* status) {
  phmrf_solve_state* s = b->ss;
  if (!(ch <= s->tol || !improved)) return false;
  if (s->all_active && s->verifying) {
    finish(s, 1, status);
    return true;
  }
  activate_all(s);
  s->all_active = true;
  s->verifying = true;
  if (!s->prev_moving) s->geom = (s->geom + 1) % 3;
  next_round(b, status);
  return true;
}

static void rest_move_types(phmrf_block* b, int64_t ch, double gain, bool coarse_moved) {
  phmrf_solve_state* s = b->ss;
  const phmrf_solve_opts& o = s->o;
  auto& active = s->active;
  activate_all(s);
  if (o.energy_tol_ppb > 0 && ch > 0 && gain > 0) {
    const double budget_labels = 1e-9 * o.energy_tol_ppb * std::fabs(s->e_prev) / 4.0 / (gain / (double)ch);
    std::vector<int> by_count;
    for (int sl : s->slots)
      if (s->last_count[sl] >= 0) by_count.push_back(sl);
    std::sort(by_count.begin(), by_count.end(), [&](int a, int c) { return s->last_count[a] < s->last_count[c]; });
    double used = 0.0;
    for (int sl : by_count) {
      used += (double)s->last_count[sl];
      if (used > budget_labels) break;
      active[sl] = 0;
    }
  } else {
    for (int sl : s->slots) active[sl] = s->last_count[sl] != 0 ? 1 : 0;
  }
  if (coarse_moved && s->strips && rests_coarse_labels(b)) {
    active[COUNTER_FUSION] = active[COUNTER_FUSION + 1] = 1;
    if (s->expansions)
      for (int a = 0; a < b->K; ++a) active[COUNTER_EXPANSION + a] = 1;
  }
  int n_act = 0;
  for (int sl : s->slots) n_act += active[sl];
  s->all_active = n_act == (int)s->slots.size();
  if (n_act == 0) {
    activate_all(s);
    s->all_active = true;
  }
}

int phmrf_mrf_solve_round_decide(phmrf_block_t b, const uint64_t* counters, const double* energy, int* status) {
  PHMRF_CHECK(b && counters && energy, PHMRF_ERR_INVALID, "NULL argument");
  phmrf_solve_state* s = b->ss;
  PHMRF_CHECK(s, PHMRF_ERR_STATE, "no solve in progress (phmrf_mrf_solve_begin)");
  if (s->status != 0) {
    if (status) *status = s->status;
    return PHMRF_OK;
  }
  PHMRF_CHECK(s->launched && s->collected, PHMRF_ERR_STATE, "round_decide needs a launched and collected round");
  s->launched = false;
  const double e_now = energy[0] + s->beta * energy[1];
  const int64_t ch = fold_counters(b, counters);
  const bool improved = std::isinf(s->e_prev) ? ch > 0 : e_now < s->e_prev - 1e-11 * std::fabs(s->e_prev);
  trace_round(b, counters, ch, e_now);
  const double gain = s->e_prev - e_now;
  if (e_now < s->e_prev) s->e_prev = e_now;
  bool coarse_moved = false;
  for (int lv = 0; lv < N_COARSE; ++lv) coarse_moved = coarse_moved || (s->coarse && s->coarse_ran[lv] && s->coarse_changed[lv] > 0);
  if (tolerance_decides(b, gain, coarse_moved, status)) return PHMRF_OK;
  if (quiet_decides(b, ch, improved, status)) return PHMRF_OK;
  s->verifying = false;
  rest_move_types(b, ch, gain, coarse_moved);
  return next_round(b, status);
}

int phmrf_mrf_solve_end(phmrf_block_t b, phmrf_solve_result* res) {
  PHMRF_CHECK(b, PHMRF_ERR_INVALID, "block is NULL");
  phmrf_solve_state* s = b->ss;
  PHMRF_CHECK(s, PHMRF_ERR_STATE, "no solve in progress (phmrf_mrf_solve_begin)");
  if (s->launched && !s->collected) (void)hipStreamSynchronize(b->stream);
  b->has_labels = true;
  int st = PHMRF_OK;
  if (res) {
    double eu = 0, ep = 0;
    st = energy_now(b, s->beta, &eu, &ep);
    res->energy = eu + ep;
    res->energy_unary = eu;
    res->energy_pair = ep;
    res->energy_init = s->have_init_energy ? s->eu0 + s->ep0 : std::numeric_limits<double>::quiet_NaN();
    res->rounds = s->rounds;
    res->converged = s->converged;
    res->changed = s->total;
  }
  static const bool child_count = PHMRF_DEV_ENV("PHMRF_CHILD_COUNT") != nullptr;
  if (child_count) {
    (void)hipStreamSynchronize(b->stream);
    for (int lv = 0; lv < N_COARSE; ++lv) {
      unsigned long long tot[N_TRACE] = {};
      for (int q = 0; q < 4; ++q) {
        if (!b->coarse[lv * 4 + q]) continue;
        unsigned long long c[N_TRACE];
        if (hipMemcpy(c, b->coarse[lv * 4 + q]->counters + COUNTER_TRACE, sizeof(c), hipMemcpyDeviceToHost) != hipSuccess) continue;
        for (int x = 0; x < N_TRACE; ++x) tot[x] += c[x];
      }
      fprintf(stderr, "[phmrf solve] coarse scale %d child strips: seen %llu, past the memo and the pin look %llu, into the DP %llu, DP steps %llu, with a move %llu\n",
              COARSE_SCALE[lv], tot[TRACE_SEEN], tot[TRACE_PAST_MEMO], tot[TRACE_INTO_DP], tot[TRACE_DP_STEPS], tot[TRACE_MOVED]);
    }
  }
  solve_scope_exit(b);
  return st;
}

int phmrf_mrf_solve_begin(phmrf_block_t b, double beta, const phmrf_solve_opts* opts, int want_init_energy) {
  return solve_begin(b, beta, opts, want_init_energy != 0);
}

int phmrf_mrf_solve(phmrf_block_t b, double beta, const phmrf_solve_opts* opts, phmrf_solve_result* res) {
  PHMRF_TRY(solve_begin(b, beta, opts, res != nullptr));
  EndSolves scope{&b, 1};
  int status = 0;
  uint64_t counters[N_COUNTERS];
  double energy[2];
  while (status == 0) {
    if (out_of_budget(b)) break;
    PHMRF_TRY(phmrf_mrf_solve_round_launch(b));
    PHMRF_TRY(phmrf_mrf_solve_round_collect(b, counters, energy));
    PHMRF_TRY(phmrf_mrf_solve_round_decide(b, counters, energy, &status));
  }
  return phmrf_mrf_solve_end(b, res);
}

int phmrf_mrf_solve_group(phmrf_block_t* blocks, int n_blocks, double beta, const phmrf_solve_opts* opts) {
  PHMRF_CHECK(blocks && n_blocks >= 0, PHMRF_ERR_INVALID, "NULL argument");
  for (int i = 0; i < n_blocks; ++i) PHMRF_CHECK(blocks[i], PHMRF_ERR_INVALID, "block is NULL");
  EndSolves scope{blocks, 0};
  for (int i = 0; i < n_blocks; ++i) {
    PHMRF_TRY(solve_begin(blocks[i], beta, opts, false));
    scope.n = i + 1;
  }
  std::vector<int> status(n_blocks, 0);
  std::vector<char> in_flight(n_blocks, 0);
  uint64_t counters[N_COUNTERS];
  double energy[2];
  auto launch = [&](int i) -> int {
    phmrf_block* b = blocks[i];
    if (status[i] != 0) return PHMRF_OK;
    if (out_of_budget(b)) {
      status[i] = 2;
      return PHMRF_OK;
    }
    PHMRF_TRY(phmrf_mrf_solve_round_launch(b));
    in_flight[i] = 1;
    return PHMRF_OK;
  };
  int n_in_flight = 0;
  for (int i = 0; i < n_blocks; ++i) {
    PHMRF_TRY(launch(i));
    n_in_flight += in_flight[i];
  }
  while (n_in_flight > 0) {
    bool progressed = false;
    for (int i = 0; i < n_blocks; ++i) {
      if (!in_flight[i]) continue;
      const hipError_t q = hipStreamQuery(blocks[i]->stream);
      if (q == hipErrorNotReady) continue;
      PHMRF_HIP(q);
      PHMRF_TRY(phmrf_mrf_solve_round_collect(blocks[i], counters, energy));
      PHMRF_TRY(phmrf_mrf_solve_round_decide(blocks[i], counters, energy, &status[i]));
      in_flight[i] = 0;
      --n_in_flight;
      PHMRF_TRY(launch(i));
      n_in_flight += in_flight[i];
      progressed = true;
    }
    if (!progressed) std::this_thread::yield();
  }
  int st = PHMRF_OK;
  for (int i = 0; i < n_blocks; ++i) {
    const int s1 = phmrf_mrf_solve_end(blocks[i], nullptr);
    if (s1 != PHMRF_OK) st = s1;
  }
  scope.n = 0;
  return st;
}
```

Baseline: 1.490 billion.

## Fuse unary energy sums into emission and reuse cached pair energies at warm start

The emission kernel now also accumulates the unary energy of the current and warm-slot labellings. Pair energies from the previous solve are cached per label slot. With these, choosing between the current and saved labellings and computing the initial solve energy no longer needs full energy kernels or a host sync. The start energy is carried into the incremental energy tracking. This adds validity bookkeeping across many label-writing paths, with a risk of stale sums if any path is missed.

```diff
diff --git a/phylo_hmrf_amd/csrc/api.hip b/phylo_hmrf_amd/csrc/api.hip
--- a/phylo_hmrf_amd/csrc/api.hip
+++ b/phylo_hmrf_amd/csrc/api.hip
@@ -630,6 +630,7 @@
 int phmrf_block_set_graph(phmrf_block_t b, int64_t E, const int64_t* edges, const double* w) {
   PHMRF_CHECK(b, PHMRF_ERR_INVALID, "block is NULL");
   PHMRF_CHECK(E >= 0 && (E == 0 || (edges && w)), PHMRF_ERR_INVALID, "edges / w is NULL");
+  graph_written(b);
   const int64_t n = b->n;
   std::vector<int32_t> deg(n, 0);
   for (int64_t e = 0; e < E; ++e) {
@@ -726,6 +727,7 @@
   PHMRF_CHECK(H >= 1 && W >= 1, PHMRF_ERR_INVALID, "H, W must be >= 1");
   PHMRF_CHECK(num_neighbor == 8 || num_neighbor == 4, PHMRF_ERR_INVALID, "num_neighbor must be 8 or 4");
   PHMRF_CHECK(!diagonal || H <= W, PHMRF_ERR_INVALID, "a diagonal block is the first H <= W rows of a W x W upper triangle");
+  graph_written(b);
   Geometry g(H, W, diagonal);
   PHMRF_CHECK(g.count() == b->n, PHMRF_ERR_INVALID, "H, W, diagonal do not match the node count");
   const int64_t n = b->n;
@@ -771,6 +773,7 @@
   PHMRF_CHECK(num_neighbor == 8 || num_neighbor == 4, PHMRF_ERR_INVALID, "num_neighbor must be 8 or 4");
   PHMRF_CHECK(!diagonal || H <= W, PHMRF_ERR_INVALID, "a diagonal block is the first H <= W rows of a W x W upper triangle");
   PHMRF_CHECK(beta1 >= 0.0 && std::isfinite(beta1), PHMRF_ERR_INVALID, "beta1 must be finite and >= 0");
+  graph_written(b);
   Geometry g(H, W, diagonal);
   PHMRF_CHECK(g.count() == b->n, PHMRF_ERR_INVALID, "H, W, diagonal do not match the node count");
   dev_free(b->nbr);
@@ -805,7 +808,7 @@
   }
   PHMRF_TRY(upload(b->labels, tmp.data(), (size_t)b->n, b->stream));
   b->has_labels = true;
-  b->labels_are_slot = 0;
+  labels_written(b);
   return PHMRF_OK;
 }
 
@@ -827,6 +830,9 @@
   if (!b->saved[slot]) PHMRF_TRY(dev_alloc(&b->saved[slot], (size_t)b->n));
   PHMRF_HIP(hipMemcpyAsync(b->saved[slot], b->labels, (size_t)b->n, hipMemcpyDeviceToDevice, b->stream));
   b->labels_are_slot |= 1 << slot;
+  b->pair_sum[slot] = b->pair_sum[LAB_CURRENT];
+  b->pair_valid[slot] = b->pair_valid[LAB_CURRENT];
+  if (slot == WARM_SLOT) b->usum_valid &= ~2;
   return PHMRF_OK;
 }
 
@@ -835,7 +841,10 @@
   PHMRF_CHECK(slot >= 0 && slot < 4 && b->saved[slot], PHMRF_ERR_STATE, "label slot is empty");
   PHMRF_HIP(hipMemcpyAsync(b->labels, b->saved[slot], (size_t)b->n, hipMemcpyDeviceToDevice, b->stream));
   b->has_labels = true;
+  labels_written(b);
   b->labels_are_slot = 1 << slot;
+  b->pair_sum[LAB_CURRENT] = b->pair_sum[slot];
+  b->pair_valid[LAB_CURRENT] = b->pair_valid[slot];
   return PHMRF_OK;
 }
 
@@ -909,9 +918,24 @@
   std::vector<float> packed((size_t)b->K * PS);
   PHMRF_TRY(phmrf_emission_pack(b->S, b->K, means, covars, packed.data()));
   PHMRF_TRY(upload(b->emis_params, packed.data(), packed.size() * sizeof(float), b->stream));
+  b->usum_valid = 0;
+  b->start_valid = false;
+  const uint8_t *lab_a = nullptr, *lab_b = nullptr;
+  if (b->uT && b->has_labels) {
+    const bool planes_were_valid = b->uT_valid;
+    b->uT_valid = true;
+    if (setup_applies(b) && b->pair_valid[LAB_CURRENT]) {
+      lab_a = b->labels;
+      if (b->saved[WARM_SLOT] && b->pair_valid[WARM_SLOT] && !((b->labels_are_slot >> WARM_SLOT) & 1)) lab_b = b->saved[WARM_SLOT];
+    }
+    b->uT_valid = planes_were_valid;
+  }
+  if (lab_a) PHMRF_TRY(zero_accum(b, ACC_USUM_CUR, 2));
   tic(b, KC_EMISSION);
-  PHMRF_TRY(launch_emission(b->X, b->n, b->S, b->K, b->emis_params, b->logprob, b->uT, b->stream));
+  PHMRF_TRY(launch_emission(b->X, b->n, b->S, b->K, b->emis_params, b->logprob, b->uT, b->stream, lab_a, lab_b,
+                            b->accum + ACC_USUM_CUR, b->deterministic ? 1 : 0));
   toc(b, KC_EMISSION, 1);
+  b->usum_valid = (lab_a ? 1 : 0) | (lab_b ? 2 : 0);
   b->has_logprob = true;
   b->uT_valid = b->uT != nullptr;
   b->pin_saved = false;
@@ -937,6 +961,8 @@
   PHMRF_TRY(upload(b->logprob, tmp.data(), cnt * sizeof(float), b->stream));
   b->has_logprob = true;
   b->uT_valid = false;
+  b->usum_valid = 0;
+  b->start_valid = false;
   b->pin_saved = false;
   b->pin_rows[0] = b->pin_rows[1] = 0;
   return PHMRF_OK;
@@ -972,11 +998,27 @@
   const bool report = e_current || e_saved || took_saved;
   if (!b->has_labels || ((b->labels_are_slot >> slot) & 1)) {
     if (choose && !b->has_labels) PHMRF_TRY(phmrf_block_restore_labels(b, slot));
+    if (choose && !report && setup_applies(b) && (b->usum_valid & 1) && b->pair_valid[LAB_CURRENT]) {
+      tic(b, KC_ENERGY);
+      PHMRF_TRY(launch_choose_labels_sums(b, nullptr, b->accum + ACC_USUM_CUR, b->pair_sum[LAB_CURRENT], 0.0, beta, b->accum + ACC_START));
+      toc(b, KC_ENERGY, 1);
+      b->start_valid = true;
+    }
     if (e_current) *e_current = std::numeric_limits<double>::infinity();
     if (e_saved) *e_saved = 0.0;
     return PHMRF_OK;
   }
   double* const extra = b->accum + (ACCUM_DOUBLES - 4);
+  if (choose && !report && slot == WARM_SLOT && setup_applies(b) && b->usum_valid == 3 && b->pair_valid[LAB_CURRENT] &&
+      b->pair_valid[slot]) {
+    tic(b, KC_ENERGY);
+    PHMRF_TRY(launch_choose_labels_sums(b, b->saved[slot], b->accum + ACC_USUM_CUR, b->pair_sum[LAB_CURRENT], b->pair_sum[slot], beta,
+                                        b->accum + ACC_START));
+    toc(b, KC_ENERGY, 1);
+    labels_written(b);
+    b->start_valid = true;
+    return PHMRF_OK;
+  }
   if (choose && !report && b->n >= (1 << 16) && energy_diff_available(b)) {
     PHMRF_TRY(zero_accum(b, 4, 2));
     PHMRF_TRY(zero_accum(b, ACCUM_DOUBLES - 4, 2));
@@ -984,7 +1026,7 @@
     PHMRF_TRY(launch_energy_diff(b, b->saved[slot]));
     PHMRF_TRY(launch_choose_labels(b, b->saved[slot], b->accum + 4, extra, beta));
     toc(b, KC_ENERGY, 2);
-    b->labels_are_slot = 0;
+    labels_written(b);
     return PHMRF_OK;
   }
   PHMRF_TRY(zero_accum(b, 4, 2));
@@ -997,7 +1039,7 @@
   PHMRF_TRY(st);
   if (choose) PHMRF_TRY(launch_choose_labels(b, b->saved[slot], b->accum + 4, extra, beta));
   toc(b, KC_ENERGY, choose ? 3 : 2);
-  if (choose) b->labels_are_slot = 0;
+  if (choose) labels_written(b);
   if (!report) return PHMRF_OK;
   PHMRF_HIP(hipMemcpyAsync(b->accum_host + 4, b->accum + 4, 2 * sizeof(double), hipMemcpyDeviceToHost, b->stream));
   PHMRF_HIP(hipMemcpyAsync(b->accum_host + 6, extra, 2 * sizeof(double), hipMemcpyDeviceToHost, b->stream));
@@ -1034,7 +1076,7 @@
 
 int phmrf_mrf_icm_sweep(phmrf_block_t b, double beta, int64_t* changed) {
   PHMRF_TRY(check_solvable(b));
-  b->labels_are_slot = 0;
+  labels_written(b);
   PHMRF_TRY(zero_counter(b));
   PHMRF_TRY(icm_sweep_nocount(b, (float)beta));
   return read_counter(b, changed);
@@ -1047,7 +1089,7 @@
 
 int phmrf_mrf_chain_sweep(phmrf_block_t b, double beta, int family, int64_t* changed) {
   PHMRF_TRY(check_solvable(b));
-  b->labels_are_slot = 0;
+  labels_written(b);
   PHMRF_TRY(ensure_chain_families(b));
   PHMRF_CHECK(family >= 0 && family < (int)b->families.size(), PHMRF_ERR_INVALID, "no such chain family");
   PHMRF_TRY(zero_counter(b));
@@ -1095,7 +1137,7 @@
 
 int phmrf_mrf_component_pass(phmrf_block_t b, double beta, int64_t* changed) {
   PHMRF_TRY(check_solvable(b));
-  b->labels_are_slot = 0;
+  labels_written(b);
   PHMRF_TRY(zero_counter(b));
   tic(b, KC_COMPONENT);
   PHMRF_TRY(launch_component_pass(b, (float)beta));
@@ -1108,7 +1150,7 @@
   PHMRF_CHECK(b->has_labels, PHMRF_ERR_STATE, "labels not set");
   PHMRF_CHECK(alpha >= 0 && alpha < b->K, PHMRF_ERR_INVALID, "alpha must be in [0, K)");
   PHMRF_CHECK(b->n >= 2, PHMRF_ERR_INVALID, "the graph has fewer than two nodes");
-  b->labels_are_slot = 0;
+  labels_written(b);
   PHMRF_TRY(zero_counter(b));
   PHMRF_TRY(launch_graph_expansion(b, (float)beta, alpha));
   return read_counter(b, changed);
@@ -1117,7 +1159,7 @@
 
 int phmrf_mrf_strip_pass(phmrf_block_t b, double beta, int orient, int shift_r, int shift_c, int alpha, int64_t* changed) {
   PHMRF_TRY(check_solvable(b));
-  b->labels_are_slot = 0;
+  labels_written(b);
   PHMRF_CHECK(b->has_grid, PHMRF_ERR_STATE, "strip moves need phmrf_block_set_grid");
   PHMRF_CHECK(b->num_neighbor == 8 || b->num_neighbor == 4, PHMRF_ERR_STATE, "bad grid");
   PHMRF_CHECK(orient == 0 || orient == 1, PHMRF_ERR_INVALID, "orient must be 0 or 1");
@@ -1134,7 +1176,7 @@
 int phmrf_mrf_strip_multi_pass(phmrf_block_t b, double beta, int orient, int shift_r, int shift_c, uint64_t label_mask,
                                int64_t* changed) {
   PHMRF_TRY(check_solvable(b));
-  b->labels_are_slot = 0;
+  labels_written(b);
   PHMRF_CHECK(b->has_grid, PHMRF_ERR_STATE, "strip moves need phmrf_block_set_grid");
   PHMRF_CHECK(b->num_neighbor == 8 || b->num_neighbor == 4, PHMRF_ERR_STATE, "bad grid");
   PHMRF_CHECK(orient == 0 || orient == 1, PHMRF_ERR_INVALID, "orient must be 0 or 1");
@@ -1159,7 +1201,7 @@
 int phmrf_mrf_coarse_pass(phmrf_block_t b, double beta, int scale, int offset, int alpha, int shift_r, int shift_c,
                           int64_t* changed) {
   PHMRF_TRY(check_solvable(b));
-  b->labels_are_slot = 0;
+  labels_written(b);
   PHMRF_CHECK(b->has_grid, PHMRF_ERR_STATE, "coarse moves need phmrf_block_set_grid");
   PHMRF_CHECK(scale == 2 || scale == 4 || scale == 8, PHMRF_ERR_INVALID, "scale must be 2, 4 or 8");
   PHMRF_CHECK(offset >= 0 && offset < scale, PHMRF_ERR_INVALID, "offset must be in [0, scale)");
@@ -1222,7 +1264,7 @@
   PHMRF_CHECK(offset >= 0 && offset < scale, PHMRF_ERR_INVALID, "offset must be in [0, scale)");
   PHMRF_CHECK(shift_r >= 0 && shift_r <= 5 && shift_c >= 0 && shift_c <= 63, PHMRF_ERR_INVALID, "shift out of range");
   PHMRF_CHECK(b->K >= 64 || (label_mask >> b->K) == 0, PHMRF_ERR_INVALID, "label_mask names a label >= K");
-  b->labels_are_slot = 0;
+  labels_written(b);
   const int level = scale == 2 ? 0 : (scale == 4 ? 1 : 2);
   const size_t lab_bytes = (size_t)N_COARSE * MAX_LABELS * sizeof(unsigned long long);
   if (!b->coarse_lab) {
@@ -1287,11 +1329,11 @@
   }
   PHMRF_TRY(upload(c->labels, tmp.data(), (size_t)nc, b->stream));
   c->has_labels = true;
-  c->labels_are_slot = 0;
+  labels_written(c);
   PHMRF_TRY(launch_c2f_prolong(b, c, b->c2f_Wc, C2F_SCALE));
   PHMRF_HIP(hipStreamSynchronize(b->stream));
   b->has_labels = true;
-  b->labels_are_slot = 0;
+  labels_written(b);
   return PHMRF_OK;
 }
 
@@ -1303,6 +1345,7 @@
   top = top ? 1 : 0;
   bottom = bottom ? 1 : 0;
   PHMRF_CHECK(b->H >= 2 * (top + bottom) + 2, PHMRF_ERR_INVALID, "a tile needs two rows per cut and two more");
+  graph_written(b);
   for (int r = 0; r < 2; ++r) {
     dev_free(b->pin_save[r]);
     dev_free(b->pin_label[r]);
@@ -1411,7 +1454,7 @@
   PHMRF_CHECK(b, PHMRF_ERR_INVALID, "block is NULL");
   PHMRF_CHECK(is_tile(b), PHMRF_ERR_STATE, "the block is not a tile (phmrf_block_set_tile)");
   if (b->tick) ++b->tick;
-  b->labels_are_slot = 0;
+  labels_written(b);
   uint8_t* const in_host = b->xfer_host + b->xfer_cap;
   int64_t off = 0;
   if (top_in && b->tile_top) {
@@ -1558,7 +1601,7 @@
   std::memcpy(out, b->accum_host + 8, NP * sizeof(double));
   if (write_labels) {
     b->has_labels = true;
-    b->labels_are_slot = 0;
+    labels_written(b);
   }
   return PHMRF_OK;
 }
@@ -1582,7 +1625,7 @@
   std::memcpy(out, b->accum_host + 8, NP * sizeof(double));
   if (write_labels) {
     b->has_labels = true;
-    b->labels_are_slot = 0;
+    labels_written(b);
   }
   return PHMRF_OK;
 }
diff --git a/phylo_hmrf_amd/csrc/common.h b/phylo_hmrf_amd/csrc/common.h
--- a/phylo_hmrf_amd/csrc/common.h
+++ b/phylo_hmrf_amd/csrc/common.h
@@ -88,6 +88,10 @@
   float* sgain = nullptr;
   uint8_t* saved[4] = {nullptr, nullptr, nullptr, nullptr};
   int labels_are_slot = 0;
+  double pair_sum[5] = {0, 0, 0, 0, 0};
+  bool pair_valid[5] = {false, false, false, false, false};
+  int usum_valid = 0;
+  bool start_valid = false;
   bool has_X = false, has_logprob = false, has_labels = false, has_graph = false, has_grid = false;
 
   int D = 0;
@@ -216,6 +220,8 @@
   int geom = 0;
   bool prev_moving = false;
   bool launched = false, collected = false, incremental = false, snapshot = false;
+  bool carry_from_start = false;
+  bool carry_valid = false;
   int status = 0;
 };
 
@@ -257,6 +263,27 @@
 }
 
 inline bool is_tile(const phmrf_block* b) { return b->tile_top || b->tile_bot; }
+
+constexpr int LAB_CURRENT = 4;
+constexpr int WARM_SLOT = 0;
+constexpr int ACC_USUM_CUR = ACCUM_DOUBLES - 8;
+constexpr int ACC_USUM_SLOT = ACCUM_DOUBLES - 7;
+constexpr int ACC_START = ACCUM_DOUBLES - 6;
+inline bool setup_applies(const phmrf_block* b) {
+  static const char* const legacy_env = PHMRF_DEV_ENV("PHMRF_SETUP_LEGACY");
+  static const bool legacy = legacy_env && legacy_env[0] && legacy_env[0] != '0';
+  return !legacy && b->has_grid && b->fwd_w && b->uT && b->uT_valid && b->D == 8 && b->H > 0 && b->W > 0 && !is_tile(b);
+}
+inline void labels_written(phmrf_block* b) {
+  b->labels_are_slot = 0;
+  b->pair_valid[LAB_CURRENT] = false;
+  b->usum_valid &= ~1;
+  b->start_valid = false;
+}
+inline void graph_written(phmrf_block* b) {
+  for (bool& v : b->pair_valid) v = false;
+  b->start_valid = false;
+}
 
 struct Geometry;
 int setup_grid_tables(phmrf_block* b, const Geometry& g, int num_neighbor);
@@ -282,11 +309,15 @@
 inline int tile_threads(int K) { return K <= 40 ? 256 : 128; }
 inline int padded_k(int K) { return (K % 2 == 0) ? K + 1 : K; }
 
-int launch_emission(const float* X, int64_t n, int S, int K, const float* packed, float* logprob, float* uT, hipStream_t st);
+int launch_emission(const float* X, int64_t n, int S, int K, const float* packed, float* logprob, float* uT, hipStream_t st,
+                    const uint8_t* lab_a = nullptr, const uint8_t* lab_b = nullptr, double* usum = nullptr, int det = 0);
 int launch_argmax_labels(const phmrf_block* b);
 int launch_icm_colour(const phmrf_block* b, float beta, int colour);
 int launch_energy(const phmrf_block* b, float beta, double* accum_at = nullptr);
 int launch_choose_labels(const phmrf_block* b, const uint8_t* saved, const double* acc_cur, const double* acc_sav, double beta);
+int launch_choose_labels_sums(const phmrf_block* b, const uint8_t* saved, const double* usum, double pair_cur, double pair_sav,
+                              double beta, double* start);
+bool energy_snapshot_applies(const phmrf_block* b);
 bool energy_delta_available(const phmrf_block* b);
 bool energy_diff_available(const phmrf_block* b);
 int launch_energy_diff(const phmrf_block* b, const uint8_t* other);
diff --git a/phylo_hmrf_amd/csrc/kernels.hip b/phylo_hmrf_amd/csrc/kernels.hip
--- a/phylo_hmrf_amd/csrc/kernels.hip
+++ b/phylo_hmrf_amd/csrc/kernels.hip
@@ -12,10 +12,11 @@
 constexpr int ACC_STATS = 8;
 
 constexpr double ENERGY_FIX = 1048576.0;
+__device__ __forceinline__ double energy_term(float v, int det) { return det ? rint((double)v * ENERGY_FIX) : (double)v; }
 __device__ __forceinline__ void energy_flush(double* accum, double tu, double tp, int det) {
   if (det) {
-    atomicAdd(reinterpret_cast<unsigned long long*>(accum + ACC_ENERGY), (unsigned long long)__double2ll_rn(tu * ENERGY_FIX));
-    atomicAdd(reinterpret_cast<unsigned long long*>(accum + ACC_ENERGY + 1), (unsigned long long)__double2ll_rn(tp * ENERGY_FIX));
+    atomicAdd(reinterpret_cast<unsigned long long*>(accum + ACC_ENERGY), (unsigned long long)__double2ll_rn(tu));
+    atomicAdd(reinterpret_cast<unsigned long long*>(accum + ACC_ENERGY + 1), (unsigned long long)__double2ll_rn(tp));
   } else {
     atomicAdd(accum + ACC_ENERGY, tu);
     atomicAdd(accum + ACC_ENERGY + 1, tp);
@@ -112,13 +113,15 @@
   return (int)g;
 }
 
-template <int S, int VEC>
+template <int S, int VEC, bool SUMS>
 __global__ __launch_bounds__(256) void emission_kernel(const float* __restrict__ X, int64_t n, int K, int Kp,
                                                        const float* __restrict__ P, float* __restrict__ out,
-                                                       float* __restrict__ uT) {
+                                                       float* __restrict__ uT, const uint8_t* __restrict__ lab_a,
+                                                       const uint8_t* __restrict__ lab_b, double* __restrict__ usum, int det) {
   extern __shared__ float tile[];
   constexpr int PS = S + S * (S + 1) / 2 + 1;
   const int TB = blockDim.x;
+  double ua = 0.0, ub = 0.0;
   for (int64_t base = (int64_t)blockIdx.x * TB; base < n; base += (int64_t)gridDim.x * TB) {
     const int64_t i = base + threadIdx.x;
     if (i < n) {
@@ -152,6 +155,10 @@
         row[k] = lp;
         if (uT) uT[(int64_t)k * n + i] = -lp;
       }
+      if (SUMS) {
+        if (lab_a) ua += energy_term(-row[lab_a[i]], det);
+        if (lab_b) ub += energy_term(-row[lab_b[i]], det);
+      }
     }
     __syncthreads();
     const int64_t rem = n - base;
@@ -159,17 +166,24 @@
     tile_to_rows<VEC>(out + base * K, rows, K, Kp, tile);
     __syncthreads();
   }
-}
-
-template <int S>
-int launch_emission_s(const float* X, int64_t n, int K, const float* packed, float* logprob, float* uT, hipStream_t st) {
+  if (SUMS) {
+    __shared__ double red[8];
+    const double ta = block_sum(ua, red);
+    const double tb = block_sum(ub, red);
+    if (threadIdx.x == 0) energy_flush(usum - ACC_ENERGY, ta, tb, det);
+  }
+}
+
+template <int S, bool SUMS>
+int launch_emission_s(const float* X, int64_t n, int K, const float* packed, float* logprob, float* uT, hipStream_t st,
+                      const uint8_t* lab_a, const uint8_t* lab_b, double* usum, int det) {
   const int TB = tile_threads(K), Kp = padded_k(K);
   const size_t lds = (size_t)TB * Kp * sizeof(float);
   const int grid = grid_for(n, TB);
   switch (vec_of(K)) {
-    case 4: hipLaunchKernelGGL((emission_kernel<S, 4>), dim3(grid), dim3(TB), lds, st, X, n, K, Kp, packed, logprob, uT); break;
-    case 2: hipLaunchKernelGGL((emission_kernel<S, 2>), dim3(grid), dim3(TB), lds, st, X, n, K, Kp, packed, logprob, uT); break;
-    default: hipLaunchKernelGGL((emission_kernel<S, 1>), dim3(grid), dim3(TB), lds, st, X, n, K, Kp, packed, logprob, uT); break;
+    case 4: hipLaunchKernelGGL((emission_kernel<S, 4, SUMS>), dim3(grid), dim3(TB), lds, st, X, n, K, Kp, packed, logprob, uT, lab_a, lab_b, usum, det); break;
+    case 2: hipLaunchKernelGGL((emission_kernel<S, 2, SUMS>), dim3(grid), dim3(TB), lds, st, X, n, K, Kp, packed, logprob, uT, lab_a, lab_b, usum, det); break;
+    default: hipLaunchKernelGGL((emission_kernel<S, 1, SUMS>), dim3(grid), dim3(TB), lds, st, X, n, K, Kp, packed, logprob, uT, lab_a, lab_b, usum, det); break;
   }
   PHMRF_HIP(hipGetLastError());
   return PHMRF_OK;
@@ -259,19 +273,27 @@
   double eu = 0.0, ep = 0.0;
   for (int64_t i = (int64_t)blockIdx.x * blockDim.x + threadIdx.x; i < n; i += (int64_t)gridDim.x * blockDim.x) {
     const int l = labels[i];
-    eu -= (double)logprob[i * K + l];
+    eu += energy_term(-logprob[i * K + l], det);
     const int32_t* nb = nbr + i * D;
     const float* wg = wgt + i * D;
     float s = 0.f;
+    double sq = 0.0;
     for (int j = 0; j < D; j += 4) {
       const int4 c = *reinterpret_cast<const int4*>(nb + j);
       const float4 w = *reinterpret_cast<const float4*>(wg + j);
-      if (c.x >= 0 && labels[c.x] != l) s += w.x;
-      if (c.y >= 0 && labels[c.y] != l) s += w.y;
-      if (c.z >= 0 && labels[c.z] != l) s += w.z;
-      if (c.w >= 0 && labels[c.w] != l) s += w.w;
-    }
-    ep += (double)s;
+      const bool cx = c.x >= 0 && labels[c.x] != l, cy = c.y >= 0 && labels[c.y] != l;
+      const bool cz = c.z >= 0 && labels[c.z] != l, cw = c.w >= 0 && labels[c.w] != l;
+      if (det) {
+        sq += (cx ? energy_term(w.x, 1) : 0.0) + (cy ? energy_term(w.y, 1) : 0.0) + (cz ? energy_term(w.z, 1) : 0.0) +
+              (cw ? energy_term(w.w, 1) : 0.0);
+      } else {
+        if (cx) s += w.x;
+        if (cy) s += w.y;
+        if (cz) s += w.z;
+        if (cw) s += w.w;
+      }
+    }
+    ep += det ? sq : (double)s;
   }
   const double tu = block_sum(eu, red);
   const double tp = block_sum(ep, red);
@@ -318,7 +340,12 @@
     for (int u = 0; u < UR; ++u) {
       if (!on[u]) continue;
       const int l = lab[u];
-      eu += (double)un[u];
+      eu += energy_term(un[u], det);
+      if (det) {
+        ep += (ln[u][0] != l ? energy_term(w[u].x, 1) : 0.0) + (ln[u][1] != l ? energy_term(w[u].y, 1) : 0.0) +
+              (ln[u][2] != l ? energy_term(w[u].z, 1) : 0.0) + (ln[u][3] != l ? energy_term(w[u].w, 1) : 0.0);
+        continue;
+      }
       float s = 0.f;
       if (ln[u][0] != l) s += w[u].x;
       if (ln[u][1] != l) s += w[u].y;
@@ -383,13 +410,24 @@
     for (int u = 0; u < UR; ++u) {
       if (!on[u]) continue;
       const int l = lab[u], q = labp[u];
-      eu += (double)un[u] - (double)unp[u];
-      float s = 0.f;
-      s += (ln[u][0] != l ? w[u].x : 0.f) - (lp[u][0] != q ? w[u].x : 0.f);
-      s += (ln[u][1] != l ? w[u].y : 0.f) - (lp[u][1] != q ? w[u].y : 0.f);
-      s += (ln[u][2] != l ? w[u].z : 0.f) - (lp[u][2] != q ? w[u].z : 0.f);
-      s += (ln[u][3] != l ? w[u].w : 0.f) - (lp[u][3] != q ? w[u].w : 0.f);
-      ep += (double)s;
+      eu += energy_term(un[u], det) - energy_term(unp[u], det);
+      if (det) {
+        ep += energy_term(w[u].x, 1) * (double)((int)(ln[u][0] != l) - (int)(lp[u][0] != q)) +
+              energy_term(w[u].y, 1) * (double)((int)(ln[u][1] != l) - (int)(lp[u][1] != q)) +
+              energy_term(w[u].z, 1) * (double)((int)(ln[u][2] != l) - (int)(lp[u][2] != q)) +
+              energy_term(w[u].w, 1) * (double)((int)(ln[u][3] != l) - (int)(lp[u][3] != q));
+        continue;
+      }
+      float sn = 0.f, so = 0.f;
+      if (ln[u][0] != l) sn += w[u].x;
+      if (ln[u][1] != l) sn += w[u].y;
+      if (ln[u][2] != l) sn += w[u].z;
+      if (ln[u][3] != l) sn += w[u].w;
+      if (lp[u][0] != q) so += w[u].x;
+      if (lp[u][1] != q) so += w[u].y;
+      if (lp[u][2] != q) so += w[u].z;
+      if (lp[u][3] != q) so += w[u].w;
+      ep += (double)sn - (double)so;
     }
   }
   const double tu = block_sum(eu, red);
@@ -441,13 +479,24 @@
     for (int u = 0; u < UR; ++u) {
       if (!on[u]) continue;
       const float4 w = fwd_w[me[u]];
-      if (la[u] != lb[u]) eu += (double)uT[(int64_t)la[u] * n + me[u]] - (double)uT[(int64_t)lb[u] * n + me[u]];
-      float s = 0.f;
-      s += (na[u][0] != la[u] ? w.x : 0.f) - (nb[u][0] != lb[u] ? w.x : 0.f);
-      s += (na[u][1] != la[u] ? w.y : 0.f) - (nb[u][1] != lb[u] ? w.y : 0.f);
-      s += (na[u][2] != la[u] ? w.z : 0.f) - (nb[u][2] != lb[u] ? w.z : 0.f);
-      s += (na[u][3] != la[u] ? w.w : 0.f) - (nb[u][3] != lb[u] ? w.w : 0.f);
-      ep += (double)s;
+      if (la[u] != lb[u]) eu += energy_term(uT[(int64_t)la[u] * n + me[u]], det) - energy_term(uT[(int64_t)lb[u] * n + me[u]], det);
+      if (det) {
+        ep += energy_term(w.x, 1) * (double)((int)(na[u][0] != la[u]) - (int)(nb[u][0] != lb[u])) +
+              energy_term(w.y, 1) * (double)((int)(na[u][1] != la[u]) - (int)(nb[u][1] != lb[u])) +
+              energy_term(w.z, 1) * (double)((int)(na[u][2] != la[u]) - (int)(nb[u][2] != lb[u])) +
+              energy_term(w.w, 1) * (double)((int)(na[u][3] != la[u]) - (int)(nb[u][3] != lb[u]));
+        continue;
+      }
+      float sa = 0.f, sb = 0.f;
+      if (na[u][0] != la[u]) sa += w.x;
+      if (na[u][1] != la[u]) sa += w.y;
+      if (na[u][2] != la[u]) sa += w.z;
+      if (na[u][3] != la[u]) sa += w.w;
+      if (nb[u][0] != lb[u]) sb += w.x;
+      if (nb[u][1] != lb[u]) sb += w.y;
+      if (nb[u][2] != lb[u]) sb += w.z;
+      if (nb[u][3] != lb[u]) sb += w.w;
+      ep += (double)sa - (double)sb;
     }
   }
   const double tu = block_sum(eu, red);
@@ -1052,9 +1101,14 @@
   return fail(PHMRF_ERR_UNSUPPORTED, "ancestral: S must be in [1,8]");
 }
 
-int launch_emission(const float* X, int64_t n, int S, int K, const float* packed, float* logprob, float* uT, hipStream_t st) {
+int launch_emission(const float* X, int64_t n, int S, int K, const float* packed, float* logprob, float* uT, hipStream_t st,
+                    const uint8_t* lab_a, const uint8_t* lab_b, double* usum, int det) {
+  const bool sums = usum && (lab_a || lab_b);
   switch (S) {
-#define PHMRF_CASE(S_) case S_: return launch_emission_s<S_>(X, n, K, packed, logprob, uT, st);
+#define PHMRF_CASE(S_)                                                                                                     \
+  case S_:                                                                                                                 \
+    return sums ? launch_emission_s<S_, true>(X, n, K, packed, logprob, uT, st, lab_a, lab_b, usum, det)                   \
+                : launch_emission_s<S_, false>(X, n, K, packed, logprob, uT, st, nullptr, nullptr, nullptr, 0);
     PHMRF_CASE(1) PHMRF_CASE(2) PHMRF_CASE(3) PHMRF_CASE(4) PHMRF_CASE(5) PHMRF_CASE(6) PHMRF_CASE(7) PHMRF_CASE(8)
     PHMRF_CASE(9) PHMRF_CASE(10) PHMRF_CASE(11) PHMRF_CASE(12) PHMRF_CASE(13) PHMRF_CASE(14) PHMRF_CASE(15) PHMRF_CASE(16)
 #undef PHMRF_CASE
@@ -1112,6 +1166,51 @@
       for (int64_t q = i; q < n && q < i + 16; ++q) labels[q] = saved[q];
     }
   }
+}
+
+__global__ __launch_bounds__(256) void choose_labels_sums_kernel(uint8_t* __restrict__ labels, const uint8_t* __restrict__ saved,
+                                                                 int64_t n, const double* __restrict__ usum, double pair_cur,
+                                                                 double pair_sav, double beta, int det, double* __restrict__ start,
+                                                                 int force_keep) {
+  double du, dp;
+  bool keep;
+  if (det) {
+    const long long cu = reinterpret_cast<const long long*>(usum)[0], su = reinterpret_cast<const long long*>(usum)[1];
+    const long long cp = __double2ll_rn(pair_cur * ENERGY_FIX), sp = __double2ll_rn(pair_sav * ENERGY_FIX);
+    du = (double)(cu - su) / ENERGY_FIX;
+    dp = (double)(cp - sp) / ENERGY_FIX;
+    keep = force_keep || du + beta * dp < 0.0;
+    if (blockIdx.x == 0 && threadIdx.x == 0) {
+      reinterpret_cast<long long*>(start)[0] = keep ? cu : su;
+      reinterpret_cast<long long*>(start)[1] = keep ? cp : sp;
+    }
+  } else {
+    du = usum[0] - usum[1];
+    dp = pair_cur - pair_sav;
+    keep = force_keep || du + beta * dp < 0.0;
+    if (blockIdx.x == 0 && threadIdx.x == 0) {
+      start[0] = keep ? usum[0] : usum[1];
+      start[1] = keep ? pair_cur : pair_sav;
+    }
+  }
+  if (keep) return;
+  for (int64_t i = ((int64_t)blockIdx.x * blockDim.x + threadIdx.x) * 16; i < n; i += (int64_t)gridDim.x * blockDim.x * 16) {
+    if (i + 16 <= n && ((reinterpret_cast<uintptr_t>(labels + i) | reinterpret_cast<uintptr_t>(saved + i)) & 15) == 0) {
+      *reinterpret_cast<uint4*>(labels + i) = *reinterpret_cast<const uint4*>(saved + i);
+    } else {
+      for (int64_t q = i; q < n && q < i + 16; ++q) labels[q] = saved[q];
+    }
+  }
+}
+
+int launch_choose_labels_sums(const phmrf_block* b, const uint8_t* saved, const double* usum, double pair_cur, double pair_sav,
+                              double beta, double* start) {
+  int64_t g64 = (b->n / 16 + 255) / 256 + 1;
+  const int grid = !saved ? 1 : (int)(g64 > 4096 ? 4096 : g64);
+  hipLaunchKernelGGL(choose_labels_sums_kernel, dim3(grid), dim3(saved ? 256 : 64), 0, b->stream, b->labels, saved, b->n, usum, pair_cur,
+                     pair_sav, beta, b->deterministic ? 1 : 0, start, saved ? 0 : 1);
+  PHMRF_HIP(hipGetLastError());
+  return PHMRF_OK;
 }
 
 int launch_choose_labels(const phmrf_block* b, const uint8_t* saved, const double* acc_cur, const double* acc_sav, double beta) {
diff --git a/phylo_hmrf_amd/csrc/solve.hip b/phylo_hmrf_amd/csrc/solve.hip
--- a/phylo_hmrf_amd/csrc/solve.hip
+++ b/phylo_hmrf_amd/csrc/solve.hip
@@ -120,12 +120,24 @@
   return PHMRF_OK;
 }
 
-static int energy_round_launch(phmrf_block* b, bool* incremental_out, bool* snapshot_out) {
+bool energy_snapshot_applies(const phmrf_block* b) {
   static const bool always_full = PHMRF_DEV_ENV("PHMRF_ENERGY_FULL") != nullptr;
   static const char* const min_n_env = PHMRF_DEV_ENV("PHMRF_ENERGY_MIN_N");
   static const int64_t min_n = min_n_env ? std::max<int64_t>(1, std::atoll(min_n_env)) : (int64_t)1 << 18;
   const bool grid = b->has_grid && b->fwd_w && b->uT && b->uT_valid && b->stamp && b->tick > 0 && b->n >= min_n;
-  const bool snapshot = grid && !always_full;
+  return grid && !always_full;
+}
+
+static int energy_snapshot(phmrf_block* b) {
+  if (!b->labels_eval) PHMRF_TRY(dev_alloc(&b->labels_eval, (size_t)b->n));
+  PHMRF_HIP(hipMemcpyAsync(b->labels_eval, b->labels, (size_t)b->n, hipMemcpyDeviceToDevice, b->stream));
+  b->eval_tick = b->tick;
+  ++b->tick;
+  return PHMRF_OK;
+}
+
+static int energy_round_launch(phmrf_block* b, bool* incremental_out, bool* snapshot_out) {
+  const bool snapshot = energy_snapshot_applies(b);
   const bool incremental = snapshot && energy_delta_available(b);
   tic(b, KC_ENERGY);
   double* const at = reinterpret_cast<double*>(b->counters + COUNTER_ENERGY);
@@ -138,12 +150,7 @@
   toc(b, KC_ENERGY, 1);
   if (is_tile(b))
     PHMRF_HIP(hipMemcpyAsync(b->accum_host + 6, b->accum + 6, sizeof(double), hipMemcpyDeviceToHost, b->stream));
-  if (snapshot) {
-    if (!b->labels_eval) PHMRF_TRY(dev_alloc(&b->labels_eval, (size_t)b->n));
-    PHMRF_HIP(hipMemcpyAsync(b->labels_eval, b->labels, (size_t)b->n, hipMemcpyDeviceToDevice, b->stream));
-    b->eval_tick = b->tick;
-    ++b->tick;
-  }
+  if (snapshot) PHMRF_TRY(energy_snapshot(b));
   *incremental_out = incremental;
   *snapshot_out = snapshot;
   return PHMRF_OK;
@@ -153,6 +160,10 @@
   static const bool check = PHMRF_DEV_ENV("PHMRF_ENERGY_CHECK") != nullptr;
   double du, dp;
   energy_sums(b, b->counters_host + COUNTER_ENERGY, &du, &dp);
+  if (b->ss && b->ss->carry_from_start) {
+    energy_sums(b, b->accum_host + ACC_START, eu_carry, ep_carry);
+    b->ss->carry_from_start = false;
+  }
   if (incremental) {
     *eu_carry += du;
     *ep_carry += dp;
@@ -313,7 +324,8 @@
   s->beta = beta;
   s->bf = (float)beta;
   s->sched_n = b->sched_n > 0 ? b->sched_n : b->n;
-  b->labels_are_slot = 0;
+  const bool start_sums = b->start_valid && setup_applies(b) && o.init_mode != 1 && o.use_components;
+  labels_written(b);
   EndSolves abort_guard{&b, 1};
   if (o.init_mode == 1) {
     bool started = false;
@@ -321,8 +333,16 @@
     if (!started) PHMRF_TRY(launch_argmax_labels(b));
     b->has_labels = true;
   }
+  if (start_sums)
+    PHMRF_HIP(hipMemcpyAsync(b->accum_host + ACC_START, b->accum + ACC_START, 2 * sizeof(double), hipMemcpyDeviceToHost, b->stream));
   if (want_init_energy) {
-    PHMRF_TRY(energy_now(b, beta, &s->eu0, &s->ep0));
+    if (start_sums) {
+      PHMRF_HIP(hipStreamSynchronize(b->stream));
+      energy_sums(b, b->accum_host + ACC_START, &s->eu0, &s->ep0);
+      s->ep0 = beta * s->ep0;
+    } else {
+      PHMRF_TRY(energy_now(b, beta, &s->eu0, &s->ep0));
+    }
     s->have_init_energy = true;
   }
   if (o.use_chains && !b->has_grid && b->families.empty() && b->nbr && b->n >= 2) PHMRF_TRY(setup_path_families(b));
@@ -353,6 +373,10 @@
   b->tick = 1;
   b->eval_tick = -1;
   b->prop_tick = -1;
+  if (start_sums && energy_snapshot_applies(b)) {
+    PHMRF_TRY(energy_snapshot(b));
+    s->carry_from_start = true;
+  }
   if (s->chains) {
     size_t total = 0;
     for (auto& f : b->families)
@@ -532,6 +556,7 @@
   if (is_tile(b)) PHMRF_TRY(tile_queue_boundary(b));
   s->launched = true;
   s->collected = false;
+  s->carry_valid = false;
   return PHMRF_OK;
 }
 
@@ -548,6 +573,7 @@
   if (!s->collected) {
     PHMRF_HIP(hipStreamSynchronize(b->stream));
     PHMRF_TRY(energy_round_collect(b, s->beta, s->incremental, &s->eu_carry, &s->ep_carry));
+    s->carry_valid = true;
     if (b->timing) work_fold(b, s->rounds == 0);
     s->collected = true;
     if (is_tile(b)) {
@@ -727,6 +753,8 @@
   PHMRF_CHECK(s, PHMRF_ERR_STATE, "no solve in progress (phmrf_mrf_solve_begin)");
   if (s->launched && !s->collected) (void)hipStreamSynchronize(b->stream);
   b->has_labels = true;
+  b->pair_valid[LAB_CURRENT] = s->carry_valid && !is_tile(b);
+  b->pair_sum[LAB_CURRENT] = s->ep_carry;
   int st = PHMRF_OK;
   if (res) {
     double eu = 0, ep = 0;
diff --git a/profiles/warm_setup_aggregate.py b/profiles/warm_setup_aggregate.py
--- /dev/null
+++ b/profiles/warm_setup_aggregate.py
@@ -0,0 +1,29 @@
+#!/usr/bin/env python3
+import csv
+import glob
+import json
+import os
+import sys
+
+sys.path.insert(0, os.path.dirname(os.path.abspath(__file__)))
+from aggregate_pmc import short
+
+kt = []
+for f in glob.glob(os.path.join(sys.argv[1], "**", "*kernel_trace.csv"), recursive=True):
+    with open(f) as fh:
+        kt += list(csv.DictReader(fh))
+kt.sort(key=lambda r: int(r["Start_Timestamp"]))
+names = [short(r["Kernel_Name"]) for r in kt]
+em = [i for i, k in enumerate(names) if k.startswith("emission_kernel")]
+seq, per = [], {}
+for r, k in list(zip(kt, names))[em[-1] if em else 0:]:
+    us = (int(r["End_Timestamp"]) - int(r["Start_Timestamp"])) / 1e3
+    seq.append([k, round(us, 1)])
+    e = per.setdefault(k, [0, 0.0])
+    e[0] += 1
+    e[1] += us
+out = {"kernels_us": {k: {"launches": v[0], "total_us": round(v[1], 1)} for k, v in sorted(per.items(), key=lambda x: -x[1][1])},
+       "total_us": round(sum(v[1] for v in per.values()), 1), "launch_order_us": seq}
+json.dump(out, open(sys.argv[2], "w"), indent=1)
+print(json.dumps(out["kernels_us"], indent=1))
+print("total_us", out["total_us"])
```

Result: no change. 1.497 billion, median of 5 (+0.4%).
